# fudan-zvg/NeRF-LiDAR

Measured on AMD Instinct MI355X. Metric: LiDAR rays/sec @128 samples/ray, 8x256 MLP; depth L1 vs reference, higher is better.
Workload: dtype f32 (sampling, hash grid) + split-bf16 x3 MFMA (density/semantic/intensity) + bf16 MFMA (view MLP); 1 GPU; C2: nuScenes 32-beam sweep, 32x1024 rays per sweep, samples (64,64,128), 8x256 NerfMLP + semantic + intensity heads, full-size fp32 hash tables; azimuth_columns_total=1024, parallelism=azimuth-sector x1, hip_graph_replay=False, weights=seeded synthetic (white-noise tables, x1500 density gain), sweep_origins=moving: step i renders sweep i mod 64 (pre-uploaded ray batches), gather_bytes_per_ray=1347584

## Files before the change

### include/nerflidar_hip.h

```cpp
#ifndef NERFLIDAR_HIP_H
#define NERFLIDAR_HIP_H

#include <stddef.h>
#include <stdint.h>

#ifdef __cplusplus
extern "C" {
#endif

#define NLR_MAX_LEVELS 4
#define NLR_MAX_GRID_LEVELS 16
#define NLR_MAX_VIEW_DEPTH 16

enum {
    NLR_OK = 0,
    NLR_ERR_INVALID = -1,
    NLR_ERR_UNSUPPORTED = -2,
    NLR_ERR_HIP = -3,
    NLR_ERR_WORKSPACE = -4
};

enum {
    NLR_PREC_F32 = 0,
    NLR_PREC_MIXED = 1,
    NLR_PREC_FAST = 2
};

const char *nlr_last_error(void);
int nlr_version(void);

int nlr_grid_encode_forward(const float *inputs, const void *embeddings, int table_dtype,
                            const int32_t *offsets_host, float *outputs, uint32_t B, uint32_t D,
                            uint32_t C, uint32_t L, float S, uint32_t H, float *dy_dx,
                            uint32_t gridtype, int align_corners, uint32_t interp, int out_layout,
                            void *stream);

int nlr_grid_encode_backward(const float *grad, const float *inputs, const int32_t *offsets_host,
                             float *grad_embeddings, uint32_t B, uint32_t D, uint32_t C, uint32_t L,
                             float S, uint32_t H, const float *dy_dx, float *grad_inputs,
                             uint32_t gridtype, int align_corners, uint32_t interp, int grad_layout,
                             void *stream);

size_t nlr_grid_backward_workspace_bytes(uint32_t B, uint32_t C, uint32_t L, float S, uint32_t H, const int32_t *offsets_host,
                                         uint32_t gridtype, int align_corners);
int nlr_grid_encode_backward_ws(const float *grad, const float *inputs, const int32_t *offsets_host, float *grad_embeddings, uint32_t B,
                                uint32_t D, uint32_t C, uint32_t L, float S, uint32_t H, const float *dy_dx, float *grad_inputs,
                                uint32_t gridtype, int align_corners, uint32_t interp, int grad_layout, void *workspace,
                                size_t workspace_bytes, void *stream);

int nlr_grad_total_variation(const float *inputs, const float *embeddings, float *grad, const int32_t *offsets_host, float weight,
                             uint32_t B, uint32_t D, uint32_t C, uint32_t L, float S, uint32_t H, uint32_t gridtype,
                             int align_corners, void *stream);

void nlr_level_scale(uint32_t L, float S, uint32_t H, float *scale, uint32_t *resolution);

void nlr_sample_u(uint32_t n, int rand, float *u_host, float *max_jitter);

typedef struct NlrLinear {
    const float *weight;
    const float *bias;
    uint32_t out_features, in_features;
} NlrLinear;

typedef struct NlrGridDesc {
    const void *table;
    int32_t table_dtype;
    uint32_t num_levels, level_dim;
    uint32_t base_resolution;
    float log2_per_level_scale;
    const int32_t *offsets;
    uint32_t gridtype;
    uint32_t align_corners;
    uint32_t interp;
} NlrGridDesc;

typedef struct NlrMlpDesc {
    NlrGridDesc grid;
    NlrLinear density0, density2;
    uint32_t disable_rgb;
    uint32_t bottleneck_width;
    uint32_t net_depth_viewdirs, net_width_viewdirs, skip_layer_dir, deg_view;
    NlrLinear view[NLR_MAX_VIEW_DEPTH];
    NlrLinear rgb_layer;
    uint32_t use_semantic, no_sem_layer, class_num;
    NlrLinear sem0, sem2;
    uint32_t use_intensity;
    NlrLinear int0, int2;
    float density_bias, rgb_premultiplier, rgb_bias, rgb_padding;
    uint32_t re_weights;
} NlrMlpDesc;

typedef struct NlrModelDesc {
    uint32_t num_levels;
    uint32_t num_samples[NLR_MAX_LEVELS];
    const NlrMlpDesc *mlps[NLR_MAX_LEVELS];
    float dilation_multiplier, dilation_bias;
    float anneal_slope, resample_padding;
    float power_lambda, std_scale;
    float bg_intensity;
    uint32_t opaque_background;
    uint32_t mlp_precision;
} NlrModelDesc;

typedef struct NlrModel NlrModel;
int nlr_model_create(const NlrModelDesc *desc, NlrModel **out, void *stream);
void nlr_model_destroy(NlrModel *m);
int nlr_model_set_table(NlrModel *m, uint32_t level, const void *table_dev, int table_dtype);

typedef struct NlrRays {
    const float *origins, *directions, *viewdirs;
    const float *radii, *near, *far;
    const float *base_x, *base_y;
} NlrRays;

typedef struct NlrRenderCfg {
    float train_frac;
    uint32_t compute_extras;
    uint32_t sample_n, sample_m;
    const float *rand_jitter[NLR_MAX_LEVELS];
    const float *rand_deg[NLR_MAX_LEVELS];
    float scale_factor;
    uint32_t shuffled_rays;
} NlrRenderCfg;

typedef struct NlrLevelOut {
    float *sdist, *tdist;
    float *weights, *density;
    float *rgb;
    float *semantic;
    float *intensity;
    float *depth;
    float *r_rgb;
    float *r_acc, *r_distance_mean, *r_distance_median, *r_distance_percentile_5, *r_distance_percentile_95;
} NlrLevelOut;

typedef struct NlrOut {
    float *rgb;
    float *depth;
    float *semantic;
    float *intensity;
    float *acc, *distance_mean, *distance_median, *distance_percentile_5, *distance_percentile_95;
    int32_t *labels;
    float *points;
    float *packed;
    uint32_t packed_h, packed_w;
    NlrLevelOut history[NLR_MAX_LEVELS];
} NlrOut;

size_t nlr_workspace_bytes(const NlrModel *m, uint32_t N);
int nlr_render_rays(const NlrModel *m, const NlrRays *rays, uint32_t N, const NlrRenderCfg *cfg,
                    const NlrOut *out, void *workspace, size_t workspace_bytes, void *stream);
int nlr_render_lidar(const NlrModel *m, const NlrRays *rays, uint32_t N, const NlrRenderCfg *cfg,
                     const NlrOut *out, void *workspace, size_t workspace_bytes, void *stream);

const char *nlr_kernel_names(void);

const char *nlr_build_sha(void);

#define NLR_DBG_FORCE_GENERIC 0
#define NLR_DBG_MLP_WORKGROUPS 1
#define NLR_DBG_BINNED_C4 2
#define NLR_DBG_NO_XPAIR_SCATTER 3
#define NLR_DBG_SCATTER_LEVELS 4
#define NLR_DBG_NO_SCATTER_CACHE 5
#define NLR_DBG_RAY_GROUPS 6
#define NLR_DBG_LAST_ROUTE 7
#define NLR_DBG_TRAIN_ROUTE 8
#define NLR_DBG_TRAIN_TRUNK_ROW0 9
#define NLR_DBG_TRAIN_TRUNK_ROWS 10
int nlr_debug_set(uint32_t key, int value);
int nlr_debug_get(uint32_t key);
int nlr_grid_fast_path(const int32_t *offsets_host, uint32_t L, uint32_t C, float S, uint32_t H, int table_dtype, uint32_t gridtype,
                       int align_corners, uint32_t interp);

enum { NLR_K_RESAMPLE = 0, NLR_K_PROP = 1, NLR_K_ENCODE = 2, NLR_K_DIRBIAS = 3, NLR_K_MLP = 4, NLR_K_COMPOSITE = 5, NLR_K_COUNT = 6 };
int nlr_profile_begin(NlrModel *m);
int nlr_profile_begin_kinds(NlrModel *m, uint32_t kind_mask);
int nlr_profile_end(NlrModel *m, void *stream, float *total_ms, uint32_t *launches);

int nlr_resample_level(const float *prev_sdist, const float *prev_weights, uint32_t n_prev,
                       float dilation, float anneal, float resample_padding, uint32_t num_samples,
                       const float *rand_jitter, const float *near, const float *far,
                       float power_lambda, uint32_t N, float *sdist, float *tdist, void *stream);

int nlr_mlp_level(const NlrModel *m, uint32_t level, const NlrRays *rays, const float *tdist,
                  uint32_t N, uint32_t sample_n, uint32_t sample_m, const float *rand_deg,
                  float *features , float *density, float *rgb,
                  float *semantic, float *intensity, void *workspace, size_t workspace_bytes,
                  void *stream);

int nlr_composite_level(const float *density, const float *tdist, const float *directions,
                        const float *rgb, const float *semantic, const float *intensity,
                        const float *far, const float *origins, uint32_t N, uint32_t S,
                        uint32_t class_num, int opaque_background, float bg, int compute_extras,
                        float scale_factor, float *weights, const NlrOut *out, float *level_depth,
                        void *stream);

size_t nlr_range_workspace_bytes(uint32_t H, uint32_t W);
int nlr_range_project(const double *points, const float *semantic, const float *rgb, uint32_t N, uint32_t H, uint32_t W,
                      float fov_up_deg, float fov_down_deg, void *workspace, size_t workspace_bytes, float *proj_range,
                      float *proj_xyz, float *proj_semantic, float *proj_rgb, int32_t *proj_idx, float *proj_mask,
                      void *stream);

int nlr_composite_backward(const float *density, const float *tdist, const float *directions, const float *rgb,
                           const float *semantic, const float *intensity, uint32_t N, uint32_t S, uint32_t class_num,
                           int opaque_background, float bg, const float *g_rgb, const float *g_depth,
                           const float *g_semantic, const float *g_intensity, const float *g_acc, const float *g_weights,
                           float *d_density, float *d_rgb, float *d_semantic, float *d_intensity, void *stream);
int nlr_cast_contract(const NlrRays *rays, const float *tdist, uint32_t N, uint32_t S, uint32_t sample_n, uint32_t sample_m,
                      float std_scale, const float *rand_deg, float *means, float *stds, void *stream);
int nlr_hash_decay_forward(const float *embeddings, const int32_t *offsets_host, uint32_t L, uint32_t C, double *level_sumsq,
                           void *stream);
int nlr_hash_decay_backward(const float *embeddings, const int32_t *offsets_host, uint32_t L, uint32_t C, float upstream,
                            float *grad_embeddings, void *stream);

typedef struct NlrTrainPlan NlrTrainPlan;
int nlr_train_plan_create(uint32_t F, uint32_t W, uint32_t WB, uint32_t D, uint32_t deg_view, uint32_t class_num,
                          int use_semantic, int use_intensity, float density_bias, float rgb_premultiplier, float rgb_bias,
                          float rgb_padding, NlrTrainPlan **out, uint32_t *n_params);
void nlr_train_plan_destroy(NlrTrainPlan *p);
uint32_t nlr_train_act_width(const NlrTrainPlan *p);
int nlr_train_param_layout(const NlrTrainPlan *p, uint32_t *offsets, uint32_t capacity);
int nlr_train_linear_table(const NlrTrainPlan *p, uint32_t *rows, uint32_t capacity);
int nlr_train_pack(NlrTrainPlan *p, const float *params_dev, void *stream);
int nlr_mlp_train_forward(const NlrTrainPlan *p, const float *features, const float *enc, uint32_t M, uint32_t S, float *density,
                          float *rgb, float *semantic, float *intensity, void *acts, void *stream);
int nlr_mlp_train_backward(const NlrTrainPlan *p, uint32_t M, uint32_t S, const float *density, const float *rgb,
                           const float *semantic, const void *acts, const float *g_density, const float *g_rgb,
                           const float *g_semantic, const float *g_intensity, void *gacts, float *d_features, void *stream);
size_t nlr_mlp_train_wgrad_workspace_bytes(const NlrTrainPlan *p, uint32_t M);
int nlr_mlp_train_wgrad(const NlrTrainPlan *p, uint32_t M, uint32_t S, const float *features, const float *enc, const void *acts,
                        const void *gacts, float *d_params, void *workspace, size_t workspace_bytes, void *stream);
int nlr_mlp_train_forward_split(const NlrTrainPlan *p, const float *features, const float *enc, uint32_t M, uint32_t M_color,
                                uint32_t S, float *density, float *rgb, float *semantic, float *intensity, void *acts, void *stream);
int nlr_mlp_train_backward_split(const NlrTrainPlan *p, uint32_t M, uint32_t M_color, uint32_t S, const float *density,
                                 const float *rgb, const float *semantic, const void *acts, const float *g_density,
                                 const float *g_rgb, const float *g_semantic, const float *g_intensity, void *gacts,
                                 float *d_features, void *stream);
int nlr_mlp_train_wgrad_split(const NlrTrainPlan *p, uint32_t M, uint32_t M_color, uint32_t S, const float *features,
                              const float *enc, const void *acts, const void *gacts, float *d_params, void *workspace,
                              size_t workspace_bytes, void *stream);

int nlr_box_winner(const float *tdist, const float *origins, const float *directions, const float *box_params, uint32_t N,
                   uint32_t S, uint32_t n_obj, int32_t *winner, void *stream);

int nlr_track_box_params(const float *tracks, const float *timestamps, uint32_t N, uint32_t n_obj, uint32_t T, float *box_params,
                         void *stream);

size_t nlr_obj_frame_backward_workspace_bytes(uint32_t K, uint32_t n_obj, uint32_t T);
int nlr_obj_frame_backward(const float *tracks, const float *timestamps, const float *origins, const float *directions,
                           const float *viewdirs, const float *tdist, uint32_t N, uint32_t S, uint32_t n_obj, uint32_t T,
                           const int32_t *ray_idx, const int32_t *sample_idx, const int32_t *track_idx, uint32_t K, const float *g_pts,
                           const float *g_dirs, float *g_tracks, void *workspace, size_t workspace_bytes, void *stream);

typedef struct NlrObjClassDesc {
    NlrMlpDesc mlp;
    uint32_t latent_size, split_latent;
    int32_t class_type;
} NlrObjClassDesc;

typedef struct NlrObjectsDesc {
    uint32_t n_classes;
    const NlrObjClassDesc *classes;
    uint32_t n_tracks;
    const int32_t *track_class;
    const float *latents;
} NlrObjectsDesc;

typedef struct NlrObjects NlrObjects;
int nlr_objects_create(const NlrObjectsDesc *desc, NlrObjects **out, void *stream);
void nlr_objects_destroy(NlrObjects *o);
size_t nlr_objects_workspace_bytes(const NlrObjects *o, uint32_t N, uint32_t S);
int nlr_objects_apply(const NlrObjects *o, const NlrRays *rays, const float *tdist, const float *box_params, uint32_t N, uint32_t S,
                      uint32_t n_obj, float *density, float *rgb, float *semantic, uint32_t K, int32_t *winner_out, void *workspace,
                      size_t workspace_bytes, void *stream);
int nlr_render_rays_dynamic(const NlrModel *m, const NlrObjects *o, const NlrRays *rays, const float *box_params, uint32_t n_obj,
                            uint32_t N, const NlrRenderCfg *cfg, const NlrOut *out, int32_t *const *winner, void *workspace,
                            size_t workspace_bytes, void *stream);
int nlr_render_lidar_dynamic(const NlrModel *m, const NlrObjects *o, const NlrRays *rays, const float *box_params, uint32_t n_obj,
                             uint32_t N, const NlrRenderCfg *cfg, const NlrOut *out, int32_t *const *winner, void *workspace,
                             size_t workspace_bytes, void *stream);

int nlr_prop_mlp_forward(const float *feat, const float *w1, const float *b1, const float *w2, const float *b2, uint32_t M, uint32_t F,
                         float *raw, void *stream);
int nlr_prop_mlp_backward(const float *feat, const float *w1, const float *b1, const float *w2, const float *b2, const float *g_raw,
                          uint32_t M, uint32_t F, float *d_feat, float *d_w1, float *d_b1, float *d_w2, float *d_b2, void *stream);

int nlr_encode_features_forward(const NlrRays *rays, const float *tdist, uint32_t N, uint32_t S, uint32_t sample_n, uint32_t sample_m,
                                float std_scale, const float *rand_deg, const NlrGridDesc *grid, uint32_t re_weights, float *features,
                                void *stream);
int nlr_encode_features_backward(const NlrRays *rays, const float *tdist, uint32_t N, uint32_t S, uint32_t sample_n, uint32_t sample_m,
                                 float std_scale, const float *rand_deg, const NlrGridDesc *grid, uint32_t re_weights,
                                 const float *d_features, float *points_tmp ,
                                 float *grad_tmp , float *grad_table, void *stream);
int nlr_encode_features_backward_ws(const NlrRays *rays, const float *tdist, uint32_t N, uint32_t S, uint32_t sample_n, uint32_t sample_m,
                                    float std_scale, const float *rand_deg, const NlrGridDesc *grid, uint32_t re_weights,
                                    const float *d_features, float *points_tmp, float *grad_tmp, float *grad_table, void *workspace,
                                    size_t workspace_bytes, void *stream);
int nlr_encode_features_backward_rays(const NlrRays *rays, const float *tdist, uint32_t N, uint32_t S, uint32_t sample_n, uint32_t sample_m,
                                      float std_scale, const float *rand_deg, const NlrGridDesc *grid, uint32_t re_weights,
                                      const float *d_features , float *d_origins, float *d_directions, float *d_base_x,
                                      float *d_base_y , void *stream);

#ifdef __cplusplus
}
#endif
#endif
```

### nerf-lidar_amd/csrc/nlr_api.hip

```cpp
#include <stdarg.h>

#include <vector>

#include "nlr_kernels.h"

#include <stdlib.h>
#include "nlr_objects.h"


static thread_local char g_err[512] = "";
void nlr_set_error(const char *fmt, ...) {
    va_list ap;
    va_start(ap, fmt);
    vsnprintf(g_err, sizeof(g_err), fmt, ap);
    va_end(ap);
}
extern "C" const char *nlr_last_error(void) { return g_err; }
extern "C" int nlr_version(void) { return 100; }
extern "C" const char *nlr_kernel_names(void) {
    return "nlr_resample_kernel,nlr_prop8_kernel,nlr_encode8_kernel,nlr_direnc_kernel,nlr_mlp_kernel,nlr_composite_kernel";
}

struct Profile {
    bool armed = false;
    uint32_t mask = 0xffffffffu;
    std::vector<hipEvent_t> ev;
    std::vector<int> kind;
};
struct ProfScope {
    Profile *p;
    hipStream_t st;
    ProfScope(Profile *prof, int kind, hipStream_t s) : p(prof && prof->armed && ((prof->mask >> kind) & 1u) ? prof : nullptr), st(s) {
        if (!p) return;
        hipEvent_t a, b;
        if (hipEventCreate(&a) != hipSuccess || hipEventCreate(&b) != hipSuccess) { p = nullptr; return; }
        p->ev.push_back(a);
        p->ev.push_back(b);
        p->kind.push_back(kind);
        (void)hipEventRecord(a, st);
    }
    ~ProfScope() {
        if (p) (void)hipEventRecord(p->ev.back(), st);
    }
};

struct LevelModel {
    bool is_prop = false;
    GridParams gp;
    uint32_t F = 0, S = 0;
    int re_weights = 1;
    float density_bias = -1.0f;
    float *p_w1 = nullptr, *p_b1 = nullptr, *p_w2 = nullptr;
    float p_b2 = 0.0f;
    uint32_t W = 0, WB = 0, D = 0, HT = 0, K = 0, int_row = 0xffffffffu, deg = 0, E = 0;
    bool use_int = false;
    uint32_t prec = NLR_PREC_MIXED;
    void *tape = nullptr;
    uint32_t tape_chunks = 0;
    void *tape_lidar = nullptr;
    uint32_t tape_lidar_chunks = 0;
    float rgb_premul = 1.0f, rgb_bias = 0.0f, rgb_padding = 0.001f;
    float *bias_all = nullptr;
    uint32_t bias_count = 0;
    float *u_det = nullptr, *u_rand = nullptr;
    float max_jitter = 0.0f;
};

struct NlrModel {
    uint32_t num_levels = 0;
    LevelModel lv[NLR_MAX_LEVELS];
    float dilation_multiplier, dilation_bias, anneal_slope, resample_padding, power_lambda, std_scale, bg;
    uint32_t opaque, prec;
    int device = 0;
    uint32_t cus = 0;
    hipStream_t up = nullptr;
    std::vector<void *> allocs;
    mutable Profile prof;
};

static int dev_upload(NlrModel *m, const void *host, size_t bytes, void **out) {
    void *p = nullptr;
    NLR_HIP(hipMalloc(&p, bytes ? bytes : 16));
    m->allocs.push_back(p);
    if (bytes) {
        NLR_HIP(hipMemcpyAsync(p, host, bytes, hipMemcpyHostToDevice, m->up));
        NLR_HIP(hipStreamSynchronize(m->up));
    }
    *out = p;
    return NLR_OK;
}

static uint16_t f32_to_bf16(float f) {
    uint32_t u;
    memcpy(&u, &f, 4);
    if ((u & 0x7f800000u) == 0x7f800000u && (u & 0x007fffffu)) return (uint16_t)((u >> 16) | 0x40);
    u += 0x7fffu + ((u >> 16) & 1u);
    return (uint16_t)(u >> 16);
}

struct Mat {
    std::vector<float> a;
    uint32_t rows = 0, cols = 0;
    Mat() {}
    Mat(uint32_t r, uint32_t c) : a((size_t)r * c, 0.0f), rows(r), cols(c) {}
    float &at(uint32_t r, uint32_t c) { return a[(size_t)r * cols + c]; }
    float get(uint32_t r, uint32_t c) const { return (r < rows && c < cols) ? a[(size_t)r * cols + c] : 0.0f; }
};

static Mat fold_w2(const Mat &a, uint32_t col0, const NlrLinear &w2, std::vector<float> &bias) {
    const uint32_t WB = w2.out_features, H = w2.in_features;
    Mat out(a.rows, H);
    for (uint32_t r = 0; r < a.rows; ++r) {
        for (uint32_t k = 0; k < H; ++k) {
            double acc = 0.0;
            for (uint32_t c = 0; c < WB; ++c) acc += (double)a.get(r, col0 + c) * (double)w2.weight[(size_t)c * H + k];
            out.at(r, k) = (float)acc;
        }
        double acc = (double)bias[r];
        for (uint32_t c = 0; c < WB; ++c) acc += (double)a.get(r, col0 + c) * (double)w2.bias[c];
        bias[r] = (float)acc;
    }
    return out;
}

static Mat mat_from(const NlrLinear &l, uint32_t col0, uint32_t ncols) {
    Mat m(l.out_features, ncols);
    for (uint32_t r = 0; r < l.out_features; ++r)
        for (uint32_t c = 0; c < ncols; ++c) m.at(r, c) = l.weight[(size_t)r * l.in_features + col0 + c];
    return m;
}

enum { TAPE_F32 = 0, TAPE_BF16 = 1, TAPE_X3 = 2 };
#define NLR_TAPE_CHUNK 32768
struct TapeBuilder {
    std::vector<uint8_t> bytes;
    size_t frags() const { return bytes.size() / 1024; }
    void frag_bf16(const Mat &w, uint32_t R, uint32_t g, bool lo_part) {
        uint16_t f[64 * 8];
        for (uint32_t lane = 0; lane < 64; ++lane)
            for (uint32_t j = 0; j < 8; ++j) {
                const float v = w.get(16 * R + (lane & 15), 32 * g + 16 * (j >> 2) + 4 * (lane >> 4) + (j & 3));
                const uint16_t hi = f32_to_bf16(v);
                if (!lo_part) {
                    f[lane * 8 + j] = hi;
                } else {
                    uint32_t hb = (uint32_t)hi << 16;
                    float hf;
                    memcpy(&hf, &hb, 4);
                    f[lane * 8 + j] = f32_to_bf16(v - hf);
                }
            }
        bytes.insert(bytes.end(), (const uint8_t *)f, (const uint8_t *)f + sizeof(f));
    }
    void frag_f32(const Mat &w, uint32_t R, uint32_t J) {
        float f[64 * 4];
        for (uint32_t lane = 0; lane < 64; ++lane)
            for (uint32_t e = 0; e < 4; ++e) f[lane * 4 + e] = w.get(16 * R + (lane & 15), 16 * J + 4 * (lane >> 4) + e);
        bytes.insert(bytes.end(), (const uint8_t *)f, (const uint8_t *)f + sizeof(f));
    }
    void add(const Mat &w, uint32_t out_pad, uint32_t in_pad, int kind, uint32_t RH = 2) {
        const uint32_t OT = RH == 2 ? out_pad / 32 : 1;
        const uint32_t KG = kind == TAPE_F32 ? in_pad / 16 : in_pad / 32;
        for (uint32_t o = 0; o < OT; ++o)
            for (uint32_t g = 0; g < KG; ++g)
                for (uint32_t j = 0; j < RH; ++j) {
                    const uint32_t R = RH == 2 ? 2 * o + j : o;
                    if (kind == TAPE_F32) {
                        frag_f32(w, R, g);
                    } else {
                        frag_bf16(w, R, g, false);
                        if (kind == TAPE_X3) frag_bf16(w, R, g, true);
                    }
                }
    }
    void pad_to_chunk() { bytes.resize((bytes.size() + NLR_TAPE_CHUNK - 1) / NLR_TAPE_CHUNK * NLR_TAPE_CHUNK, 0); }
};

static int upload_bias(NlrModel *m, const float *b, uint32_t n, uint32_t pad, float **out) {
    std::vector<float> v(pad, 0.0f);
    for (uint32_t i = 0; i < n; ++i) v[i] = b[i];
    return dev_upload(m, v.data(), pad * sizeof(float), (void **)out);
}

static int check_linear(const NlrLinear &l, uint32_t out_f, uint32_t in_f, const char *name) {
    NLR_CHECK_ARG(l.weight && l.bias, "%s: weight/bias is NULL", name);
    NLR_CHECK_ARG(l.out_features == out_f && l.in_features == in_f, "%s: expected [%u,%u], got [%u,%u]", name, out_f, in_f,
                  l.out_features, l.in_features);
    return NLR_OK;
}

static int build_level(NlrModel *m, LevelModel &lv, const NlrMlpDesc &d, uint32_t S, uint32_t prec) {
    int rc = nlr_fill_grid_params(&lv.gp, d.grid.table, d.grid.table_dtype, d.grid.offsets, d.grid.num_levels,
                                  d.grid.level_dim, d.grid.log2_per_level_scale, d.grid.base_resolution, d.grid.gridtype,
                                  (int)d.grid.align_corners, d.grid.interp);
    if (rc) return rc;
    NLR_CHECK_ARG(d.grid.table != nullptr, "mlp: hash table pointer is NULL");
    lv.S = S;
    lv.F = d.grid.num_levels * d.grid.level_dim;
    lv.re_weights = d.re_weights ? 1 : 0;
    lv.density_bias = d.density_bias;
    lv.is_prop = d.disable_rgb != 0;
    {
        std::vector<float> u(S);
        float mj = 0.0f;
        nlr_sample_u(S, 0, u.data(), nullptr);
        if ((rc = dev_upload(m, u.data(), S * sizeof(float), (void **)&lv.u_det))) return rc;
        nlr_sample_u(S, 1, u.data(), &mj);
        lv.max_jitter = mj;
        if ((rc = dev_upload(m, u.data(), S * sizeof(float), (void **)&lv.u_rand))) return rc;
    }
    if ((rc = check_linear(d.density0, 64, lv.F, "density_layer.0"))) return rc;
    if (lv.is_prop) {
        if ((rc = check_linear(d.density2, 1, 64, "density_layer.2 (PropMLP)"))) return rc;
        if ((rc = dev_upload(m, d.density0.weight, (size_t)64 * lv.F * 4, (void **)&lv.p_w1))) return rc;
        if ((rc = dev_upload(m, d.density0.bias, 64 * 4, (void **)&lv.p_b1))) return rc;
        if ((rc = dev_upload(m, d.density2.weight, 64 * 4, (void **)&lv.p_w2))) return rc;
        lv.p_b2 = d.density2.bias[0];
        return NLR_OK;
    }
    lv.W = d.net_width_viewdirs;
    lv.WB = d.bottleneck_width;
    lv.D = d.net_depth_viewdirs;
    lv.deg = d.deg_view;
    lv.E = 3 + 6 * d.deg_view;
    lv.rgb_premul = d.rgb_premultiplier;
    lv.rgb_bias = d.rgb_bias;
    lv.rgb_padding = d.rgb_padding;
    if (lv.D < 2 || d.skip_layer_dir != 0 || lv.D > NLR_MAX_VIEW_DEPTH)
        NLR_FAIL(NLR_ERR_UNSUPPORTED, "view MLP: fused path needs net_depth_viewdirs in [2,%d] and skip_layer_dir = 0 (got %u, %u)",
                 NLR_MAX_VIEW_DEPTH, lv.D, d.skip_layer_dir);
    if (lv.W % 32 || lv.WB % 32) NLR_FAIL(NLR_ERR_UNSUPPORTED, "view MLP: widths must be multiples of 32");
    if (lv.F % 4) NLR_FAIL(NLR_ERR_UNSUPPORTED, "NerfMLP: L*C = %u must be a multiple of 4", lv.F);
    if ((rc = check_linear(d.density2, lv.WB, 64, "density_layer.2"))) return rc;
    const bool sem_layer = d.use_semantic && !d.no_sem_layer;
    const bool sem_pass = d.use_semantic && d.no_sem_layer;
    if (sem_pass) NLR_CHECK_ARG(d.class_num <= 32 && 1 + d.class_num <= d.bottleneck_width, "no_sem_layer: class_num %u does not fit", d.class_num);
    lv.K = d.use_semantic ? d.class_num : 0;
    lv.use_int = d.use_intensity != 0;
    lv.HT = (d.use_semantic ? 2 : 0) + (lv.use_int ? 2 : 0);
    NLR_CHECK_ARG(lv.K + (lv.use_int ? 1 : 0) <= 32, "class_num %u (+intensity) exceeds one 32-row output tile", lv.K);

    lv.prec = prec;
    const int crit = (prec == NLR_PREC_FAST) ? TAPE_X3 : TAPE_F32;
    const int view = (prec == NLR_PREC_F32) ? TAPE_F32 : TAPE_BF16;
    const bool fold = prec == NLR_PREC_FAST;
    std::vector<float> bias;
    auto push_bias = [&](const float *b, uint32_t n, uint32_t pad) {
        for (uint32_t i = 0; i < pad; ++i) bias.push_back(i < n ? b[i] : 0.0f);
    };
    const uint32_t Fp32 = lv.F <= 64 ? 64 : ((lv.F + 31) / 32) * 32;
    TapeBuilder trunk;
    trunk.add(mat_from(d.density0, 0, lv.F), 64, Fp32, crit);
    push_bias(d.density0.bias, 64, 64);
    trunk.add(mat_from(d.density2, 0, 64), fold ? 32 : lv.WB, 64, crit);
    push_bias(d.density2.bias, fold ? 32 : lv.WB, fold ? 32 : lv.WB);
    if (lv.HT) {
        const uint32_t HH = lv.HT * 32;
        Mat h1(HH, lv.WB), h2(32, HH);
        std::vector<float> b1(HH, 0.0f), b2(32, 0.0f);
        uint32_t r0 = 0;
        if (sem_layer) {
            if ((rc = check_linear(d.sem0, 64, lv.WB, "sem_layer.0"))) return rc;
            if ((rc = check_linear(d.sem2, d.class_num, 64, "sem_layer.2"))) return rc;
            for (uint32_t r = 0; r < 64; ++r) {
                for (uint32_t c = 0; c < lv.WB; ++c) h1.at(r0 + r, c) = d.sem0.weight[(size_t)r * lv.WB + c];
                b1[r0 + r] = d.sem0.bias[r];
            }
            for (uint32_t r = 0; r < d.class_num; ++r) {
                for (uint32_t c = 0; c < 64; ++c) h2.at(r, r0 + c) = d.sem2.weight[(size_t)r * 64 + c];
                b2[r] = d.sem2.bias[r];
            }
            r0 += 64;
        }
        if (sem_pass) {
            for (uint32_t c = 0; c < d.class_num; ++c) {
                h1.at(r0 + c, 1 + c) = 1.0f;
                h1.at(r0 + 32 + c, 1 + c) = -1.0f;
                h2.at(c, r0 + c) = 1.0f;
                h2.at(c, r0 + 32 + c) = -1.0f;
            }
            r0 += 64;
        }
        if (lv.use_int) {
            if ((rc = check_linear(d.int0, 64, lv.WB, "intensity_layer.0"))) return rc;
            if ((rc = check_linear(d.int2, 1, 64, "intensity_layer.2"))) return rc;
            lv.int_row = lv.K;
            for (uint32_t r = 0; r < 64; ++r) {
                for (uint32_t c = 0; c < lv.WB; ++c) h1.at(r0 + r, c) = d.int0.weight[(size_t)r * lv.WB + c];
                b1[r0 + r] = d.int0.bias[r];
            }
            for (uint32_t c = 0; c < 64; ++c) h2.at(lv.int_row, r0 + c) = d.int2.weight[c];
            b2[lv.int_row] = d.int2.bias[0];
        }
        if (fold) trunk.add(fold_w2(h1, 0, d.density2, b1), HH, 64, crit);
        else trunk.add(h1, HH, lv.WB, crit);
        push_bias(b1.data(), HH, HH);
        trunk.add(h2, 32, HH, crit);
        push_bias(b2.data(), 32, 32);
    } else {
        push_bias(nullptr, 0, 32);
    }
    const uint32_t in0 = lv.WB + lv.E, in1 = lv.W + in0;
    if ((rc = check_linear(d.view[0], lv.W, in0, "lin_second_stage_0"))) return rc;
    if ((rc = check_linear(d.view[1], lv.W, in1, "lin_second_stage_1"))) return rc;
    NLR_CHECK_ARG(lv.E <= 32, "deg_view %u gives %u > 32 direction features -- no fused path", lv.deg, lv.E);
    TapeBuilder v01;
    if (fold) {
        const Mat v0 = mat_from(d.view[0], 0, in0), v1 = mat_from(d.view[1], 0, in1);
        std::vector<float> c0(d.view[0].bias, d.view[0].bias + lv.W), c1(d.view[1].bias, d.view[1].bias + lv.W);
        const Mat a0 = fold_w2(v0, 0, d.density2, c0), a1 = fold_w2(v1, lv.W, d.density2, c1);
        Mat f0(lv.W, 64 + lv.E), f1(lv.W, lv.W + 64 + lv.E);
        for (uint32_t r = 0; r < lv.W; ++r) {
            for (uint32_t c = 0; c < 64; ++c) f0.at(r, c) = a0.get(r, c), f1.at(r, lv.W + c) = a1.get(r, c);
            for (uint32_t c = 0; c < lv.E; ++c) f0.at(r, 64 + c) = v0.get(r, lv.WB + c), f1.at(r, lv.W + 64 + c) = v1.get(r, lv.W + lv.WB + c);
            for (uint32_t c = 0; c < lv.W; ++c) f1.at(r, c) = v1.get(r, c);
        }
        v01.add(f0, lv.W, 64 + 32, view);
        push_bias(c0.data(), lv.W, lv.W);
        v01.add(f1, lv.W, lv.W + 64 + 32, view);
        push_bias(c1.data(), lv.W, lv.W);
    } else {
        v01.add(mat_from(d.view[0], 0, in0), lv.W, lv.WB + 32, view);
        push_bias(d.view[0].bias, lv.W, lv.W);
        v01.add(mat_from(d.view[1], 0, in1), lv.W, lv.W + lv.WB + 32, view);
        push_bias(d.view[1].bias, lv.W, lv.W);
    }
    TapeBuilder tb;
    auto append = [&](const TapeBuilder &x) { tb.bytes.insert(tb.bytes.end(), x.bytes.begin(), x.bytes.end()); };
    if (prec == NLR_PREC_F32) {
        append(trunk);
        append(v01);
    } else {
        append(trunk);
        append(v01);
        append(trunk);
        append(v01);
    }
    for (uint32_t l = 2; l < lv.D; ++l) {
        char nm[64];
        snprintf(nm, sizeof(nm), "lin_second_stage_%u", l);
        if ((rc = check_linear(d.view[l], lv.W, lv.W, nm))) return rc;
        tb.add(mat_from(d.view[l], 0, lv.W), lv.W, lv.W, view);
        push_bias(d.view[l].bias, lv.W, lv.W);
    }
    if ((rc = check_linear(d.rgb_layer, 3, lv.W, "rgb_layer"))) return rc;
    tb.add(mat_from(d.rgb_layer, 0, lv.W), 16, lv.W, view, 1);
    push_bias(d.rgb_layer.bias, 3, 32);
    tb.pad_to_chunk();
    lv.bias_count = (uint32_t)bias.size();
    NLR_CHECK_ARG(lv.bias_count <= 3072, "bias block of %u floats exceeds the 3072-float LDS reservation (view MLP too deep / wide)", lv.bias_count);
    if ((rc = dev_upload(m, bias.data(), bias.size() * 4, (void **)&lv.bias_all))) return rc;
    lv.tape_chunks = (uint32_t)(tb.bytes.size() / NLR_TAPE_CHUNK);
    tb.bytes.resize(tb.bytes.size() + 3 * NLR_TAPE_CHUNK, 0);
    if ((rc = dev_upload(m, tb.bytes.data(), tb.bytes.size(), &lv.tape))) return rc;
    if (prec == NLR_PREC_FAST) {
        TapeBuilder tl;
        tl.bytes.insert(tl.bytes.end(), trunk.bytes.begin(), trunk.bytes.end());
        tl.bytes.insert(tl.bytes.end(), trunk.bytes.begin(), trunk.bytes.end());
        tl.pad_to_chunk();
        lv.tape_lidar_chunks = (uint32_t)(tl.bytes.size() / NLR_TAPE_CHUNK);
        tl.bytes.resize(tl.bytes.size() + 3 * NLR_TAPE_CHUNK, 0);
        if ((rc = dev_upload(m, tl.bytes.data(), tl.bytes.size(), &lv.tape_lidar))) return rc;
    }
    return NLR_OK;
}

extern "C" int nlr_model_create(const NlrModelDesc *desc, NlrModel **out, void *stream) {
    NLR_CHECK_ARG(desc && out, "model_create: NULL argument");
    NLR_CHECK_ARG(desc->num_levels >= 1 && desc->num_levels <= NLR_MAX_LEVELS, "num_levels %u outside [1,%d]", desc->num_levels,
                  NLR_MAX_LEVELS);
    NLR_CHECK_ARG(desc->mlp_precision <= NLR_PREC_FAST, "unknown mlp_precision %u", desc->mlp_precision);
    NlrModel *m = new NlrModel();
    m->up = (hipStream_t)stream;
    {
        int n = 0;
        if (hipGetDevice(&m->device) != hipSuccess ||
            hipDeviceGetAttribute(&n, hipDeviceAttributeMultiprocessorCount, m->device) != hipSuccess || n <= 0) {
            delete m;
            NLR_FAIL(NLR_ERR_HIP, "model_create: cannot query the current device");
        }
        m->cus = (uint32_t)n;
        const int w = nlr_debug_get(NLR_DBG_MLP_WORKGROUPS);
        if (w > 0 && w < n) m->cus = (uint32_t)w;
    }
    m->num_levels = desc->num_levels;
    m->dilation_multiplier = desc->dilation_multiplier;
    m->dilation_bias = desc->dilation_bias;
    m->anneal_slope = desc->anneal_slope;
    m->resample_padding = desc->resample_padding;
    m->power_lambda = desc->power_lambda;
    m->std_scale = desc->std_scale;
    m->bg = desc->bg_intensity;
    m->opaque = desc->opaque_background;
    m->prec = desc->mlp_precision;
    for (uint32_t l = 0; l < desc->num_levels; ++l) {
        int rc = NLR_OK;
        if (!desc->mlps[l]) {
            nlr_set_error("model_create: mlps[%u] is NULL", l);
            rc = NLR_ERR_INVALID;
        } else if (desc->num_samples[l] < 2 || desc->num_samples[l] > 512) {
            nlr_set_error("num_samples must be in [2,512], is %u", desc->num_samples[l]);
            rc = NLR_ERR_INVALID;
        } else {
            rc = build_level(m, m->lv[l], *desc->mlps[l], desc->num_samples[l], desc->mlp_precision);
            const bool last = (l + 1 == desc->num_levels);
            if (!rc && last && m->lv[l].is_prop) {
                nlr_set_error("the last level must be a NerfMLP (disable_rgb = 0)");
                rc = NLR_ERR_INVALID;
            }
            if (!rc && !last && !m->lv[l].is_prop) {
                nlr_set_error("single_mlp / NerfMLP as proposal network has no fused path (level %u)", l);
                rc = NLR_ERR_UNSUPPORTED;
            }
        }
        if (rc) {
            nlr_model_destroy(m);
            return rc;
        }
    }
    if (hipStreamSynchronize(m->up) != hipSuccess) {
        nlr_model_destroy(m);
        NLR_FAIL(NLR_ERR_HIP, "model_create: weight upload failed");
    }
    *out = m;
    return NLR_OK;
}

extern "C" void nlr_model_destroy(NlrModel *m) {
    if (!m) return;
    for (void *p : m->allocs) (void)hipFree(p);
    delete m;
}

extern "C" int nlr_model_set_table(NlrModel *m, uint32_t level, const void *table_dev, int table_dtype) {
    NLR_CHECK_ARG(m && level < m->num_levels && table_dev, "model_set_table: bad argument");
    NLR_CHECK_ARG(table_dtype == 0 || table_dtype == 1, "model_set_table: table_dtype must be 0 or 1");
    m->lv[level].gp.table = table_dev;
    m->lv[level].gp.table_dtype = table_dtype;
    return NLR_OK;
}

extern "C" int nlr_profile_begin_kinds(NlrModel *m, uint32_t kind_mask) {
    NLR_CHECK_ARG(m != nullptr, "profile_begin: NULL model");
    for (hipEvent_t e : m->prof.ev) (void)hipEventDestroy(e);
    m->prof.ev.clear();
    m->prof.kind.clear();
    m->prof.mask = kind_mask;
    m->prof.armed = true;
    return NLR_OK;
}
extern "C" int nlr_profile_begin(NlrModel *m) { return nlr_profile_begin_kinds(m, 0xffffffffu); }

extern "C" int nlr_profile_end(NlrModel *m, void *stream, float *total_ms, uint32_t *launches) {
    NLR_CHECK_ARG(m && total_ms && launches, "profile_end: NULL argument");
    m->prof.armed = false;
    NLR_HIP(hipStreamSynchronize((hipStream_t)stream));
    for (int k = 0; k < NLR_K_COUNT; ++k) {
        total_ms[k] = 0.0f;
        launches[k] = 0;
    }
    for (size_t i = 0; i < m->prof.kind.size(); ++i) {
        float ms = 0.0f;
        NLR_HIP(hipEventElapsedTime(&ms, m->prof.ev[2 * i], m->prof.ev[2 * i + 1]));
        total_ms[m->prof.kind[i]] += ms;
        launches[m->prof.kind[i]] += 1;
    }
    for (hipEvent_t e : m->prof.ev) (void)hipEventDestroy(e);
    m->prof.ev.clear();
    m->prof.kind.clear();
    return NLR_OK;
}


struct Carve {
    char *base;
    size_t off = 0, cap;
    Carve(void *p, size_t c) : base((char *)p), cap(c) {}
    float *take(size_t nfloat) {
        size_t b = al(nfloat * sizeof(float));
        float *r = base ? (float *)(base + off) : nullptr;
        off += b;
        return r;
    }
};

static size_t level_ws(const LevelModel &lv, uint32_t N, bool last) {
    size_t S = lv.S, b = 0;
    b += 2 * al((size_t)N * (S + 1) * 4);
    b += 2 * al((size_t)N * S * 4);
    if (!lv.is_prop) {
        b += al((size_t)N * S * lv.F * 4 + 1024);
        b += al((size_t)N * S * 3 * 4);
        b += al((size_t)N * S * (lv.K ? lv.K : 1) * 4);
        b += al((size_t)N * S * 4);
        b += al((size_t)N * 32 * 4);
        b += al((size_t)N * 4);
        b += al((size_t)N * S * 4);
    }
    (void)last;
    return b;
}

extern "C" size_t nlr_workspace_bytes(const NlrModel *m, uint32_t N) {
    if (!m) return 0;
    size_t b = 256 + al(64 * sizeof(uint32_t));
    for (uint32_t l = 0; l < m->num_levels; ++l) b += level_ws(m->lv[l], N, l + 1 == m->num_levels);
    return b;
}

static int run_mlp_level(const NlrModel *m, const LevelModel &lv, const NlrRays *rays, const float *tdist, uint32_t N,
                         uint32_t n, uint32_t mloops, const float *rand_deg, float *feat, float *raybias, float *density,
                         float *rgb, float *sem, float *inten, float *prop_feat, hipStream_t st, bool internal_feat = false,
                         float *seg = nullptr, float *dnorm = nullptr, uint32_t ray_groups = 0, const uint32_t *votes = nullptr,
                         bool lidar = false) {
    const int piece_major = (internal_feat && !lv.is_prop && n <= 8 && lv.F % 4 == 0) ? 1 : 0;
    CastParams cp;
    int rc = nlr_fill_cast_params(&cp, rays, tdist, rand_deg, N, lv.S, n, mloops, m->std_scale);
    if (rc) return rc;
    cp.ray_groups = ray_groups;
    cp.votes = votes;
    cp.vote_min = (uint32_t)(((uint64_t)(N ? N - 1 : 0) * lv.S) / 2);
    if (lv.is_prop) {
        ProfScope ps(&m->prof, NLR_K_PROP, st);
        return nlr_launch_prop(cp, lv.gp, lv.p_w1, lv.p_b1, lv.p_w2, lv.p_b2, lv.density_bias, lv.re_weights, density, prop_feat, st);
    }
    {
        ProfScope ps(&m->prof, NLR_K_ENCODE, st);
        if ((rc = nlr_launch_encode(cp, lv.gp, lv.re_weights, feat, piece_major, st))) return rc;
    }
    if (seg && lidar) {
        NLR_CHECK_ARG(lv.tape_lidar != nullptr, "NerfMLP: no LiDAR-only tape at this precision");
        ProfScope ps(&m->prof, NLR_K_DIRBIAS, st);
        if ((rc = nlr_launch_dnorm(rays->directions, N, dnorm, st))) return rc;
    } else if (rgb || seg) {
        NLR_CHECK_ARG(rays->viewdirs != nullptr, "NerfMLP: viewdirs is NULL");
        DirEncParams dp;
        dp.viewdirs = rays->viewdirs;
        dp.dirs = seg ? rays->directions : nullptr;
        dp.dnorm = seg ? dnorm : nullptr;
        dp.N = N;
        dp.deg = lv.deg;
        dp.E = lv.E;
        dp.out = raybias;
        ProfScope ps(&m->prof, NLR_K_DIRBIAS, st);
        if ((rc = nlr_launch_direnc(dp, st))) return rc;
    }
    MlpParams P;
    memset(&P, 0, sizeof(P));
    P.feat = feat;
    P.feat_piece_major = piece_major;
    P.M = N * lv.S;
    P.S = lv.S;
    P.F = lv.F;
    P.tape = (const uint4 *)lv.tape;
    P.tape_chunks = lv.tape_chunks;
    P.bias_all = lv.bias_all;
    P.bias_count = lv.bias_count;
    P.enc = raybias;
    P.depth = lv.D;
    P.K = (sem || seg) ? lv.K : 0;
    P.int_row = lv.int_row;
    P.tdist = tdist;
    P.dnorm = dnorm;
    P.seg = seg;
    P.opaque = m->opaque;
    P.density_bias = lv.density_bias;
    P.rgb_premul = lv.rgb_premul;
    P.rgb_bias = lv.rgb_bias;
    P.rgb_padding = lv.rgb_padding;
    P.density = density;
    P.rgb = seg ? seg : rgb;
    P.sem = sem;
    P.inten = (lv.use_int && (inten || seg)) ? (seg ? seg : inten) : nullptr;
    if (seg && lidar) {
        P.lidar = 1;
        P.tape = (const uint4 *)lv.tape_lidar;
        P.tape_chunks = lv.tape_lidar_chunks;
        P.enc = nullptr;
        P.rgb = nullptr;
    }
    ProfScope ps(&m->prof, NLR_K_MLP, st);
    return nlr_launch_mlp(P, lv.W, lv.WB, lv.HT, lv.prec, m->cus, st);
}

extern "C" int nlr_mlp_level(const NlrModel *m, uint32_t level, const NlrRays *rays, const float *tdist, uint32_t N,
                             uint32_t sample_n, uint32_t sample_m, const float *rand_deg, float *features, float *density,
                             float *rgb, float *semantic, float *intensity, void *workspace, size_t workspace_bytes,
                             void *stream) {
    NLR_CHECK_ARG(m && level < m->num_levels && rays && tdist && density, "mlp_level: bad argument");
    if (N == 0) return NLR_OK;
    const LevelModel &lv = m->lv[level];
    hipStream_t st = (hipStream_t)stream;
    if (lv.is_prop)
        return run_mlp_level(m, lv, rays, tdist, N, sample_n, sample_m, rand_deg, nullptr, nullptr, density, nullptr, nullptr,
                             nullptr, features, st);
    Carve c(workspace, workspace_bytes);
    float *feat = features ? features : c.take((size_t)N * lv.S * lv.F + 256);
    float *rb = c.take((size_t)N * 32);
    float *sem = semantic ? semantic : (lv.K ? c.take((size_t)N * lv.S * lv.K) : nullptr);
    if (c.off > workspace_bytes || (!workspace && c.off))
        NLR_FAIL(NLR_ERR_WORKSPACE, "mlp_level: workspace %zu B < needed %zu B", workspace_bytes, c.off);
    return run_mlp_level(m, lv, rays, tdist, N, sample_n, sample_m, rand_deg, feat, rb, density, rgb, sem, intensity, nullptr, st,
                         features == nullptr);
}

struct DynScene {
    const NlrObjects *objs;
    const float *box_params;
    uint32_t n_obj;
    int32_t *const *winner;
};

static int render_impl(const NlrModel *m, const NlrRays *rays, uint32_t N, const NlrRenderCfg *cfg, const NlrOut *out, void *workspace,
                       size_t workspace_bytes, void *stream, const DynScene *dyn, bool lidar_only) {
    NLR_CHECK_ARG(m && rays && cfg && out, "render_rays: NULL argument");
    NLR_CHECK_ARG(rays->origins && rays->directions && rays->near && rays->far && rays->radii, "render_rays: ray batch has NULL tensors");
    if (lidar_only) {
        NLR_CHECK_ARG(out->rgb == nullptr, "render_lidar: out->rgb must be NULL (a LiDAR-only render computes no colour)");
        NLR_CHECK_ARG(out->history[m->num_levels - 1].rgb == nullptr,
                      "render_lidar: history[%u].rgb must be NULL (a LiDAR-only render computes no colour)", m->num_levels - 1);
    }
    if (N == 0) return NLR_OK;
    size_t need = nlr_workspace_bytes(m, N), obj_ws = 0;
    if (dyn) {
        uint32_t smax = 0;
        for (uint32_t l = 0; l < m->num_levels; ++l) smax = m->lv[l].S > smax ? m->lv[l].S : smax;
        obj_ws = nlr_objects_workspace_bytes(dyn->objs, N, smax);
        need += obj_ws;
    }
    if (!workspace || workspace_bytes < need)
        NLR_FAIL(NLR_ERR_WORKSPACE, "render_rays: workspace %zu B < %zu B (nlr_workspace_bytes%s)", workspace_bytes, need,
                 dyn ? " + nlr_objects_workspace_bytes" : "");
    hipStream_t st = (hipStream_t)stream;
    void *obj_space = dyn ? (char *)workspace + (workspace_bytes - obj_ws) : nullptr;
    Carve c(workspace, workspace_bytes - obj_ws);
    const uint32_t n = cfg->sample_n ? cfg->sample_n : 7, mloops = cfg->sample_m ? cfg->sample_m : 3;
    uint32_t *votes = (uint32_t *)c.take(64);
    if (int rc0 = nlr_launch_ray_vote(nullptr, 0, 0, votes, st)) return rc0;

    const float *prev_s = nullptr, *prev_w = nullptr;
    uint32_t n_prev = 0;
    double prod = 1.0;
    for (uint32_t l = 0; l < m->num_levels; ++l) {
        const LevelModel &lv = m->lv[l];
        const bool last = (l + 1 == m->num_levels);
        const uint32_t S = lv.S;
        const NlrLevelOut &ho = out->history[l];
        float *sdist = ho.sdist ? ho.sdist : c.take((size_t)N * (S + 1));
        float *tdist = ho.tdist ? ho.tdist : c.take((size_t)N * (S + 1));
        float *weights = ho.weights ? ho.weights : c.take((size_t)N * S);
        float *density = ho.density ? ho.density : c.take((size_t)N * S);
        const bool use_dil = m->dilation_bias > 0 || m->dilation_multiplier > 0;
        const float dilation = (l > 0 && use_dil) ? (float)(m->dilation_bias + m->dilation_multiplier * 1.0 / prod) : 0.0f;
        prod *= (double)S;
        const float tf = cfg->train_frac;
        const float anneal = m->anneal_slope > 0 ? (float)(((double)m->anneal_slope * tf) / (((double)m->anneal_slope - 1.0) * tf + 1.0)) : 1.0f;
        const float *jit = cfg->rand_jitter[l];
        int rc;
        {
            ProfScope ps(&m->prof, NLR_K_RESAMPLE, st);
            rc = nlr_launch_resample(prev_s, prev_w, n_prev, dilation, anneal, m->resample_padding, S, jit ? lv.u_rand : lv.u_det,
                                     jit, lv.max_jitter, rays->near, rays->far, m->power_lambda, N, sdist, tdist, st);
        }
        if (rc) return rc;
        float *feat = nullptr, *rb = nullptr, *rgb = nullptr, *sem = nullptr, *inten = nullptr, *seg = nullptr, *dnorm = nullptr;
        const bool lidar = lidar_only && last;
        const bool fuse = !dyn && last && !lv.is_prop && !ho.rgb && !ho.semantic && !ho.intensity && lv.gp.C == 4 && n <= 8 &&
                          nlr_mlp_can_composite(lv.W, lv.WB, lv.HT, lv.prec, lv.F, S, lv.K, lv.use_int, (uint64_t)N * S, lidar ? 2 : 1);
        if (last) (void)nlr_debug_set(NLR_DBG_LAST_ROUTE, (lidar ? 2 : 0) + (fuse ? 1 : 0) + 1);
        if (!lv.is_prop) {
            feat = c.take((size_t)N * S * lv.F + 256);
            rb = c.take((size_t)N * 32);
            if (fuse) {
                dnorm = c.take((size_t)N);
                seg = c.take((size_t)N * S);
            } else {
                rgb = lidar ? nullptr : (ho.rgb ? ho.rgb : c.take((size_t)N * S * 3));
                sem = lv.K ? (ho.semantic ? ho.semantic : c.take((size_t)N * S * lv.K)) : nullptr;
                inten = lv.use_int ? (ho.intensity ? ho.intensity : c.take((size_t)N * S)) : nullptr;
            }
        }
        uint32_t groups = cfg->shuffled_rays ? 0u : 2u;
        if (const int force = nlr_debug_get(NLR_DBG_RAY_GROUPS)) groups = force == 1 ? 1u : 0u;
        if (groups == 2u && n > 8) groups = 0u;
        if (groups == 2u && (rc = nlr_launch_ray_vote(tdist, N, S, votes + l, st))) return rc;
        rc = run_mlp_level(m, lv, rays, tdist, N, n, mloops, cfg->rand_deg[l], feat, rb, density, rgb, sem, inten, nullptr, st, true, seg,
                           dnorm, groups, votes + l, lidar);
        if (rc) return rc;
        if (dyn) {
            rc = nlr_objects_apply_impl(dyn->objs, rays, tdist, dyn->box_params, N, S, dyn->n_obj, density, rgb, sem, lv.K,
                                        dyn->winner ? dyn->winner[l] : nullptr, obj_space, obj_ws, st);
            if (rc) return rc;
        }
        {
            ProfScope ps(&m->prof, NLR_K_COMPOSITE, st);
            if (fuse)
                rc = nlr_composite_segments(density, tdist, rays->directions, seg, lv.K, lv.use_int ? 1 : 0, rays->far, rays->origins, N, S,
                                            (int)m->opaque, m->bg, (int)cfg->compute_extras, cfg->scale_factor, weights, out, ho.depth, st,
                                            lidar);
            else if (last)
                rc = nlr_composite_level_impl(density, tdist, rays->directions, rgb, sem, inten, rays->far, rays->origins, N, S, lv.K,
                                              (int)m->opaque, m->bg, (int)cfg->compute_extras, cfg->scale_factor, weights, out, ho.depth,
                                              st, lidar);
            else {
                NlrOut lo;
                memset(&lo, 0, sizeof(lo));
                lo.rgb = ho.r_rgb;
                lo.acc = ho.r_acc;
                lo.distance_mean = ho.r_distance_mean;
                lo.distance_median = ho.r_distance_median;
                lo.distance_percentile_5 = ho.r_distance_percentile_5;
                lo.distance_percentile_95 = ho.r_distance_percentile_95;
                const bool extras = cfg->compute_extras && (lo.distance_mean || lo.distance_median || lo.distance_percentile_5 || lo.distance_percentile_95);
                rc = nlr_composite_level(density, tdist, rays->directions, nullptr, nullptr, nullptr, rays->far, rays->origins, N, S, 0,
                                         (int)m->opaque, m->bg, extras ? 1 : 0, 0.0f, weights, &lo, ho.depth, st);
            }
        }
        if (rc) return rc;
        prev_s = sdist;
        prev_w = weights;
        n_prev = S;
    }
    if (c.off > workspace_bytes - obj_ws) NLR_FAIL(NLR_ERR_WORKSPACE, "render_rays: carved %zu B > workspace %zu B", c.off, workspace_bytes - obj_ws);
    return NLR_OK;
}

extern "C" int nlr_render_rays(const NlrModel *m, const NlrRays *rays, uint32_t N, const NlrRenderCfg *cfg, const NlrOut *out,
                               void *workspace, size_t workspace_bytes, void *stream) {
    return render_impl(m, rays, N, cfg, out, workspace, workspace_bytes, stream, nullptr, false);
}

extern "C" int nlr_render_lidar(const NlrModel *m, const NlrRays *rays, uint32_t N, const NlrRenderCfg *cfg, const NlrOut *out,
                                void *workspace, size_t workspace_bytes, void *stream) {
    return render_impl(m, rays, N, cfg, out, workspace, workspace_bytes, stream, nullptr, true);
}

static int render_dynamic(const NlrModel *m, const NlrObjects *o, const NlrRays *rays, const float *box_params, uint32_t n_obj, uint32_t N,
                          const NlrRenderCfg *cfg, const NlrOut *out, int32_t *const *winner, void *workspace, size_t workspace_bytes,
                          void *stream, bool lidar_only) {
    NLR_CHECK_ARG(m && o && (box_params || n_obj == 0), "render_rays_dynamic: NULL argument");
    for (uint32_t l = 0; l < m->num_levels; ++l)
        NLR_CHECK_ARG(!m->lv[l].use_int, "render_rays_dynamic: the object networks have no intensity head (ZI/models.py:469 assigns None)");
    DynScene d{o, box_params, n_obj, winner};
    return render_impl(m, rays, N, cfg, out, workspace, workspace_bytes, stream, &d, lidar_only);
}

extern "C" int nlr_render_rays_dynamic(const NlrModel *m, const NlrObjects *o, const NlrRays *rays, const float *box_params, uint32_t n_obj,
                                       uint32_t N, const NlrRenderCfg *cfg, const NlrOut *out, int32_t *const *winner, void *workspace,
                                       size_t workspace_bytes, void *stream) {
    return render_dynamic(m, o, rays, box_params, n_obj, N, cfg, out, winner, workspace, workspace_bytes, stream, false);
}

extern "C" int nlr_render_lidar_dynamic(const NlrModel *m, const NlrObjects *o, const NlrRays *rays, const float *box_params, uint32_t n_obj,
                                        uint32_t N, const NlrRenderCfg *cfg, const NlrOut *out, int32_t *const *winner, void *workspace,
                                        size_t workspace_bytes, void *stream) {
    return render_dynamic(m, o, rays, box_params, n_obj, N, cfg, out, winner, workspace, workspace_bytes, stream, true);
}
```

### nerf-lidar_amd/csrc/nlr_common.h

```cpp
#pragma once
#include <hip/hip_runtime.h>
#include <math.h>
#include <stdint.h>
#include <stdio.h>
#include <string.h>

#include "../../include/nerflidar_hip.h"

#define NLR_EPS 1.1920928955078125e-07f
#define NLR_WAVE 64

void nlr_set_error(const char *fmt, ...);
#define NLR_FAIL(code, ...)         \
    do {                            \
        nlr_set_error(__VA_ARGS__); \
        return (code);              \
    } while (0)
#define NLR_CHECK_ARG(cond, ...) \
    do {                         \
        if (!(cond)) NLR_FAIL(NLR_ERR_INVALID, __VA_ARGS__); \
    } while (0)
#define NLR_HIP(call)                                                                      \
    do {                                                                                   \
        hipError_t e_ = (call);                                                            \
        if (e_ != hipSuccess)                                                              \
            NLR_FAIL(NLR_ERR_HIP, "%s failed: %s (%s:%d)", #call, hipGetErrorString(e_), __FILE__, __LINE__); \
    } while (0)
#define NLR_LAUNCH_CHECK(name)                                                             \
    do {                                                                                   \
        hipError_t e_ = hipGetLastError();                                                 \
        if (e_ != hipSuccess)                                                              \
            NLR_FAIL(NLR_ERR_HIP, "launch of %s failed: %s", name, hipGetErrorString(e_)); \
    } while (0)

struct GridParams {
    const void *table;
    int32_t table_dtype;
    uint32_t L, C;
    uint32_t gridtype, align_corners, interp;
    uint32_t offset[NLR_MAX_GRID_LEVELS];
    uint32_t hsize[NLR_MAX_GRID_LEVELS];
    uint32_t res[NLR_MAX_GRID_LEVELS];
    float scale[NLR_MAX_GRID_LEVELS];
    float gsize[NLR_MAX_GRID_LEVELS];
    float inv_gsize[NLR_MAX_GRID_LEVELS];
    uint32_t dense[NLR_MAX_GRID_LEVELS];
    uint32_t mode[NLR_MAX_GRID_LEVELS];
    uint32_t step[NLR_MAX_GRID_LEVELS];
};

int nlr_fill_grid_params(GridParams *gp, const void *table, int table_dtype, const int32_t *offsets_host,
                         uint32_t L, uint32_t C, float S, uint32_t H, uint32_t gridtype, int align_corners,
                         uint32_t interp);

#ifdef __HIPCC__
__device__ __forceinline__ uint32_t nlr_grid_index(uint32_t gridtype, uint32_t align_corners, uint32_t hsize,
                                                   uint32_t res, uint32_t x, uint32_t y, uint32_t z) {
    uint32_t stride = 1, index = 0;
    const uint32_t step = align_corners ? res : res + 1;
    if (stride <= hsize) { index += x * stride; stride *= step; }
    if (stride <= hsize) { index += y * stride; stride *= step; }
    if (stride <= hsize) { index += z * stride; stride *= step; }
    if (gridtype == 0 && stride > hsize) index = x ^ (y * 2654435761u) ^ (z * 805459861u);
    return index % hsize;
}

template <int MODE>
__device__ __forceinline__ void nlr_corner_idx(const GridParams &gp, uint32_t level, const uint32_t (&pg)[3], uint32_t (&idx)[8]) {
    if (MODE == 0) {
        const uint32_t s = gp.step[level];
        const uint32_t y0 = pg[1] * s, z0 = pg[2] * s * s;
        const uint32_t y1 = y0 + s, z1 = z0 + s * s;
#pragma unroll
        for (int c8 = 0; c8 < 8; ++c8) idx[c8] = (pg[0] + (c8 & 1)) + ((c8 & 2) ? y1 : y0) + ((c8 & 4) ? z1 : z0);
    } else if (MODE == 1) {
        const uint32_t mask = gp.hsize[level] - 1u;
        const uint32_t y0 = pg[1] * 2654435761u, z0 = pg[2] * 805459861u;
        const uint32_t y1 = y0 + 2654435761u, z1 = z0 + 805459861u;
#pragma unroll
        for (int c8 = 0; c8 < 8; ++c8) idx[c8] = ((pg[0] + (c8 & 1)) ^ ((c8 & 2) ? y1 : y0) ^ ((c8 & 4) ? z1 : z0)) & mask;
    } else {
#pragma unroll
        for (int c8 = 0; c8 < 8; ++c8)
            idx[c8] = nlr_grid_index(gp.gridtype, gp.align_corners, gp.hsize[level], gp.res[level], pg[0] + (c8 & 1),
                                     pg[1] + ((c8 >> 1) & 1), pg[2] + ((c8 >> 2) & 1));
    }
}

__device__ __forceinline__ float nlr_wave_incl_scan_add(float v, int lane) {
#pragma unroll
    for (int d = 1; d < 64; d <<= 1) {
        float o = __shfl_up(v, d, 64);
        if (lane >= d) v += o;
    }
    return v;
}
__device__ __forceinline__ float nlr_wave_incl_scan_max(float v, int lane) {
#pragma unroll
    for (int d = 1; d < 64; d <<= 1) {
        float o = __shfl_up(v, d, 64);
        if (lane >= d) v = fmaxf(v, o);
    }
    return v;
}
__device__ __forceinline__ float nlr_wave_sum(float v) {
#pragma unroll
    for (int d = 32; d >= 1; d >>= 1) v += __shfl_xor(v, d, 64);
    return v;
}
__device__ __forceinline__ float nlr_wave_max(float v) {
#pragma unroll
    for (int d = 32; d >= 1; d >>= 1) v = fmaxf(v, __shfl_xor(v, d, 64));
    return v;
}
__device__ __forceinline__ float nlr_nan0_clip01(float x) {
    if (x != x) x = 0.0f;
    return fminf(fmaxf(x, 0.0f), 1.0f);
}
#endif
```

### nerf-lidar_amd/csrc/nlr_encode.hip

```cpp
#include "nlr_kernels.h"

#include <stdlib.h>

#include "nlr_cast.h"
#include "nlr_grid_level.h"
#include "nlr_level_fast.h"

template <typename T, int C>
__global__ void __launch_bounds__(256) nlr_encode_kernel(CastParams cp, GridParams gp, int re_weights, float *__restrict__ feat) {
    const uint32_t m = blockIdx.x * blockDim.x + threadIdx.x;
    const uint32_t M = cp.N * cp.S;
    if (m >= M) return;
    const uint32_t level = blockIdx.y;
    const uint32_t ray = m / cp.S, k = m - ray * cp.S;
    float o[3], d[3], bx[3], by[3];
#pragma unroll
    for (int c = 0; c < 3; ++c) {
        o[c] = cp.origins[(size_t)ray * 3 + c];
        d[c] = cp.directions[(size_t)ray * 3 + c];
        bx[c] = cp.base_x[(size_t)ray * 3 + c];
        by[c] = cp.base_y[(size_t)ray * 3 + c];
    }
    const float radius = cp.radii[ray];
    const float t0 = cp.tdist[(size_t)ray * (cp.S + 1) + k], t1 = cp.tdist[(size_t)ray * (cp.S + 1) + k + 1];
// ... 13 lines not shown

struct PropMlpParams {
    const float *w1, *b1;
    const float *w2;
    float b2, density_bias;
    uint32_t F;
};

template <typename T, int C, int LMAX>
__global__ void __launch_bounds__(256) nlr_prop_kernel(CastParams cp, GridParams gp, PropMlpParams mp, int re_weights,
                                                       float *__restrict__ density, float *__restrict__ feat_out) {
    const uint32_t m = blockIdx.x * blockDim.x + threadIdx.x;
    const uint32_t M = cp.N * cp.S;
    if (m >= M) return;
    const uint32_t ray = m / cp.S, k = m - ray * cp.S;
    float o[3], d[3], bx[3], by[3];
#pragma unroll
    for (int c = 0; c < 3; ++c) {
        o[c] = cp.origins[(size_t)ray * 3 + c];
        d[c] = cp.directions[(size_t)ray * 3 + c];
        bx[c] = cp.base_x[(size_t)ray * 3 + c];
        by[c] = cp.base_y[(size_t)ray * 3 + c];
    }
    const float radius = cp.radii[ray];
    const float t0 = cp.tdist[(size_t)ray * (cp.S + 1) + k], t1 = cp.tdist[(size_t)ray * (cp.S + 1) + k + 1];
    float feat[LMAX * C];
#pragma unroll
    for (int i = 0; i < LMAX * C; ++i) feat[i] = 0.0f;
    for (uint32_t j = 0; j < cp.n; ++j) {
        const Gauss g = nlr_cast_one(cp, ray, k, j, t0, t1, o, d, bx, by, radius);
#pragma unroll
        for (int l = 0; l < LMAX; ++l) {
            if (l < (int)gp.L) {
                const float werf = re_weights ? nlr_erf_weight(g.zs, gp.gsize[l]) : 1.0f;
                float a[C];
#pragma unroll
                for (int c = 0; c < C; ++c) a[c] = 0.0f;
                nlr_level_accum<T, C>(gp, l, g, werf, a);
#pragma unroll
                for (int c = 0; c < C; ++c) feat[l * C + c] += a[c];
            }
        }
    }
#pragma unroll
    for (int i = 0; i < LMAX * C; ++i) feat[i] = feat[i] / (float)cp.n;
    if (feat_out)
        for (uint32_t i = 0; i < mp.F; ++i) feat_out[(size_t)m * mp.F + i] = feat[i];
    float raw = mp.b2;
    for (int h = 0; h < 64; ++h) {
        float a = mp.b1[h];
#pragma unroll
        for (int i = 0; i < LMAX * C; ++i)
            if (i < (int)mp.F) a = fmaf(mp.w1[h * mp.F + i], feat[i], a);
        raw = fmaf(mp.w2[h], fmaxf(a, 0.0f), raw);
    }
    const float x = raw + mp.density_bias;
    density[m] = x > 20.0f ? x : log1pf(expf(x));
}

__device__ __forceinline__ bool nlr_slot_sample(const CastParams &cp, uint32_t slot, uint32_t &ray, uint32_t &k) {
    const bool groups = cp.ray_groups == 1u || (cp.ray_groups == 2u && cp.votes[0] > cp.vote_min);
    if (groups) {
        const uint32_t G = 8u * cp.S, gi = slot / G, w = slot - gi * G;
        ray = gi * 8u + (w & 7u);
        k = w >> 3;
    } else {
        ray = slot / cp.S;
        k = slot - ray * cp.S;
    }
    const bool in = ray < cp.N;
    if (!in) ray = cp.N - 1, k = cp.S - 1;
    return in;
}
__global__ void __launch_bounds__(256) nlr_ray_vote_kernel(const float *__restrict__ tdist, uint32_t N, uint32_t S, uint32_t *__restrict__ votes) {
    __shared__ uint32_t part[4];
    const uint32_t total = (N - 1) * S;
    uint32_t mine = 0;
    for (uint32_t i = blockIdx.x * 256u + threadIdx.x; i < total; i += gridDim.x * 256u) {
        const uint32_t r = i / S, k = i - r * S;
        const float *a = tdist + (size_t)r * (S + 1) + k;
        mine += fabsf(a[S + 1] - a[0]) < (a[1] - a[0]) ? 1u : 0u;
    }
#pragma unroll
    for (int o = 32; o; o >>= 1) mine += __shfl_down(mine, o);
    if ((threadIdx.x & 63u) == 0) part[threadIdx.x >> 6] = mine;
    __syncthreads();
    if (threadIdx.x == 0) {
        const uint32_t c = part[0] + part[1] + part[2] + part[3];
        if (c) atomicAdd(votes, c);
    }
}
__global__ void nlr_ray_vote_zero_kernel(uint32_t *votes) { votes[threadIdx.x] = 0u; }
int nlr_launch_ray_vote(const float *tdist, uint32_t N, uint32_t S, uint32_t *votes, hipStream_t st) {
    if (!tdist) {
        hipLaunchKernelGGL(nlr_ray_vote_zero_kernel, dim3(1), dim3(64), 0, st, votes);
        NLR_LAUNCH_CHECK("nlr_ray_vote_zero_kernel");
        return NLR_OK;
    }
    if (N < 2 || S == 0) return NLR_OK;
    NLR_CHECK_ARG((uint64_t)N * S < (1ull << 32), "ray vote: N * S = %llu does not fit 32 bits", (unsigned long long)N * S);
    const uint32_t nb = ((N - 1) * S + 255) / 256;
    hipLaunchKernelGGL(nlr_ray_vote_kernel, dim3(nb < 512u ? nb : 512u), dim3(256), 0, st, tdist, N, S, votes);
    NLR_LAUNCH_CHECK("nlr_ray_vote_kernel");
    return NLR_OK;
}
__host__ __forceinline__ uint64_t nlr_slot_count(const CastParams &cp) {
    return (uint64_t)(cp.ray_groups ? (cp.N + 7u) / 8u * 8u : cp.N) * cp.S;
}

template <int CTRL>
__device__ __forceinline__ float nlr_dpp_mov(float v) {
    return __builtin_bit_cast(float, __builtin_amdgcn_update_dpp(0, __builtin_bit_cast(int, v), CTRL, 0xf, 0xf, false));
}
__device__ __forceinline__ float nlr_group8_sum(float v) {
    v += nlr_dpp_mov<0xB1>(v);
    v += nlr_dpp_mov<0x4E>(v);
    v += nlr_dpp_mov<0x141>(v);
    return v;
}

template <int C>
__device__ __forceinline__ float *nlr_feat_ptr(float *feat, int piece_major, uint32_t M, uint32_t m, uint32_t l, uint32_t L) {
    if (piece_major) {
        const uint32_t f = l * C;
        return feat + ((size_t)(f >> 2) * M + m) * 4 + (f & 3u);
    }
    return feat + (size_t)m * L * C + l * C;
}

template <typename T, int C>
__global__ void __launch_bounds__(256) nlr_encode8g_kernel(CastParams cp, GridParams gp, int re_weights, float *__restrict__ feat,
                                                          int piece_major) {
    const uint32_t gt = blockIdx.x * blockDim.x + threadIdx.x;
    const uint32_t M = cp.N * cp.S;
    const uint32_t j = gt & 7;
    uint32_t ray, k;
    const bool in = nlr_slot_sample(cp, gt >> 3, ray, k);
    const uint32_t m = ray * cp.S + k;
    const bool active = in && j < cp.n;
    float o[3], d[3], bx[3], by[3];
#pragma unroll
    for (int c = 0; c < 3; ++c) {
        o[c] = cp.origins[(size_t)ray * 3 + c];
        d[c] = cp.directions[(size_t)ray * 3 + c];
        bx[c] = cp.base_x[(size_t)ray * 3 + c];
        by[c] = cp.base_y[(size_t)ray * 3 + c];
    }
    const float radius = cp.radii[ray];
    const float t0 = cp.tdist[(size_t)ray * (cp.S + 1) + k], t1 = cp.tdist[(size_t)ray * (cp.S + 1) + k + 1];
    Gauss g = nlr_cast_one(cp, ray, k, active ? j : 0, t0, t1, o, d, bx, by, radius);
    if (!active) g.x0 = -1.0f;
    const float inv_s8 = __frsqrt_rn(8.0f * (g.zs * g.zs));
    const float inv_n = 1.0f / (float)cp.n;
    for (uint32_t l = 0; l < gp.L; ++l) {
        const float werf = re_weights ? nlr_erf_weight_fast(inv_s8, gp.inv_gsize[l]) : 1.0f;
        float a[C];
#pragma unroll
        for (int c = 0; c < C; ++c) a[c] = 0.0f;
        nlr_level_accum<T, C>(gp, l, g, werf, a);
#pragma unroll
        for (int c = 0; c < C; ++c) a[c] = nlr_group8_sum(a[c]);
        if (in && j == (l & 7)) {
            if constexpr (C == 8) {
                float *f0 = nlr_feat_ptr<4>(feat, piece_major, M, m, 2 * l, 2 * gp.L), *f1 = nlr_feat_ptr<4>(feat, piece_major, M, m, 2 * l + 1, 2 * gp.L);
#pragma unroll
                for (int c = 0; c < 4; ++c) f0[c] = a[c] * inv_n, f1[c] = a[4 + c] * inv_n;
            } else {
                float *f = nlr_feat_ptr<C>(feat, piece_major, M, m, l, gp.L);
#pragma unroll
                for (int c = 0; c < C; ++c) f[c] = a[c] * inv_n;
            }
        }
    }
}

template <typename T, int C, int LMAX>
__global__ void __launch_bounds__(256) nlr_prop8g_kernel(CastParams cp, GridParams gp, PropMlpParams mp, int re_weights,
                                                        float *__restrict__ density, float *__restrict__ feat_out) {
    __shared__ float sw[64 * 16 + 128];
    for (uint32_t i = threadIdx.x; i < 64 * mp.F; i += 256) sw[i] = mp.w1[i];
    if (threadIdx.x < 64) {
        sw[64 * mp.F + threadIdx.x] = mp.b1[threadIdx.x];
        sw[64 * mp.F + 64 + threadIdx.x] = mp.w2[threadIdx.x];
    }
    __syncthreads();
    const uint32_t gt = blockIdx.x * blockDim.x + threadIdx.x;
    const uint32_t j = gt & 7;
    uint32_t ray, k;
    const bool in = nlr_slot_sample(cp, gt >> 3, ray, k);
    const uint32_t m = ray * cp.S + k;
    const bool active = in && j < cp.n;
    float o[3], d[3], bx[3], by[3];
#pragma unroll
    for (int c = 0; c < 3; ++c) {
        o[c] = cp.origins[(size_t)ray * 3 + c];
        d[c] = cp.directions[(size_t)ray * 3 + c];
        bx[c] = cp.base_x[(size_t)ray * 3 + c];
        by[c] = cp.base_y[(size_t)ray * 3 + c];
    }
    const float radius = cp.radii[ray];
    const float t0 = cp.tdist[(size_t)ray * (cp.S + 1) + k], t1 = cp.tdist[(size_t)ray * (cp.S + 1) + k + 1];
    Gauss g = nlr_cast_one(cp, ray, k, active ? j : 0, t0, t1, o, d, bx, by, radius);
    if (!active) g.x0 = -1.0f;
    const float inv_s8 = __frsqrt_rn(8.0f * (g.zs * g.zs));
    const float inv_n = 1.0f / (float)cp.n;
    float feat[LMAX * C];
#pragma unroll
    for (int l = 0; l < LMAX; ++l) {
        float a[C];
#pragma unroll
        for (int c = 0; c < C; ++c) a[c] = 0.0f;
        if (l < (int)gp.L) {
            const float werf = re_weights ? nlr_erf_weight_fast(inv_s8, gp.inv_gsize[l]) : 1.0f;
            nlr_level_accum<T, C>(gp, l, g, werf, a);
        }
#pragma unroll
        for (int c = 0; c < C; ++c) feat[l * C + c] = nlr_group8_sum(a[c]) * inv_n;
    }
    if (feat_out && in && j == 0)
        for (uint32_t i = 0; i < mp.F; ++i) feat_out[(size_t)m * mp.F + i] = feat[i];
    float part = 0.0f;
#pragma unroll
    for (int hh = 0; hh < 8; ++hh) {
        const uint32_t hu = hh * 8 + j;
        float a = sw[64 * mp.F + hu];
#pragma unroll
        for (int i = 0; i < LMAX * C; ++i)
            if (i < (int)mp.F) a = fmaf(sw[hu * mp.F + i], feat[i], a);
        part = fmaf(sw[64 * mp.F + 64 + hu], fmaxf(a, 0.0f), part);
    }
    const float raw = nlr_group8_sum(part) + mp.b2;
    if (in && j == 0) {
        const float x = raw + mp.density_bias;
        density[m] = x > 20.0f ? x : log1pf(expf(x));
    }
}

__device__ __forceinline__ uint32_t nlr_xcd_block(uint32_t b, uint32_t nblocks, uint32_t chunk) {
    const uint32_t per = 8u * chunk, full = (nblocks / per) * per;
    if (b >= full) return b;
    const uint32_t x = b & 7u, q = b >> 3;
    return ((q / chunk) * 8u + x) * chunk + (q % chunk);
}

#define NLR_XCD_CHUNK 32u

#ifdef NLR_DBG_ENV
#define NLR_DBG_LO nlr_dbg[0]
#define NLR_DBG_HI nlr_dbg[1]
__device__ __forceinline__ uint32_t nlr_dbg_ray(uint32_t po) {
    const uint32_t W = (uint32_t)nlr_dbg[2], tb = (uint32_t)nlr_dbg[5], ta = (uint32_t)nlr_dbg[6];
    if (!W || !tb || !ta) return po;
    const uint32_t per = tb * ta, tile = po / per, within = po - tile * per, tiles_row = W / ta;
    const uint32_t trow = tile / tiles_row, tcol = tile - trow * tiles_row;
    return (trow * tb + within / ta) * W + tcol * ta + within % ta;
}
#define NLR_DBG_RAY(r) nlr_dbg_ray(r)
#else
#define NLR_DBG_LO 0
#define NLR_DBG_HI 99
#define NLR_DBG_RAY(r) (r)
#endif

struct RayRegs {
    float o[3], d[3], bx[3], by[3], radius, t0, t1;
};
__device__ __forceinline__ RayRegs nlr_load_ray(const CastParams &cp, uint32_t ray, uint32_t k) {
    RayRegs r;
#pragma unroll
    for (int c = 0; c < 3; ++c) {
        r.o[c] = cp.origins[(size_t)ray * 3 + c];
        r.d[c] = cp.directions[(size_t)ray * 3 + c];
        r.bx[c] = cp.base_x[(size_t)ray * 3 + c];
        r.by[c] = cp.base_y[(size_t)ray * 3 + c];
    }
    r.radius = cp.radii[ray];
    r.t0 = cp.tdist[(size_t)ray * (cp.S + 1) + k];
    r.t1 = cp.tdist[(size_t)ray * (cp.S + 1) + k + 1];
    return r;
}

template <typename T, int C>
__device__ __forceinline__ void nlr_encode8_block(const CastParams &cp, const GridParams &gp, int re_weights, float *__restrict__ feat,
                                                  int piece_major, uint32_t block) {
    const uint32_t gt = block * 256u + threadIdx.x;
    const uint32_t M = cp.N * cp.S;
    const uint32_t j = gt & 7;
    uint32_t pray, k;
    const bool in = nlr_slot_sample(cp, gt >> 3, pray, k);
    const uint32_t ray = NLR_DBG_RAY(pray);
    const uint32_t m = ray * cp.S + k;
    const bool active = in && j < cp.n;
    const RayRegs rr = nlr_load_ray(cp, ray, k);
    const Gauss g = nlr_cast_one(cp, ray, k, active ? j : 0, rr.t0, rr.t1, rr.o, rr.d, rr.bx, rr.by, rr.radius);
    const bool valid = active && !((g.x0 < 0 || g.x0 > 1) || (g.x1 < 0 || g.x1 > 1) || (g.x2 < 0 || g.x2 > 1));
    const float inv_s8 = __frsqrt_rn(8.0f * (g.zs * g.zs));
    const float inv_n = 1.0f / (float)cp.n;
    float r[C];
#pragma unroll
    for (int c = 0; c < C; ++c) r[c] = 0.0f;
    for (uint32_t l = NLR_DBG_LO; l < gp.L && l < (uint32_t)NLR_DBG_HI; ++l) {
        if (valid) {
            const float werf = re_weights ? nlr_erf_weight_fast(inv_s8, gp.inv_gsize[l]) : 1.0f;
            if (gp.mode[l] == 0) nlr_level_fast<T, C, 0>(gp, l, g.x0, g.x1, g.x2, werf, r);
            else nlr_level_fast<T, C, 1>(gp, l, g.x0, g.x1, g.x2, werf, r);
        }
        float a[C];
        nlr_group8_sum_to(r, a);
        if (in && j == (l & 7)) {
            if constexpr (C == 8) {
                float *f0 = nlr_feat_ptr<4>(feat, piece_major, M, m, 2 * l, 2 * gp.L), *f1 = nlr_feat_ptr<4>(feat, piece_major, M, m, 2 * l + 1, 2 * gp.L);
#pragma unroll
                for (int c = 0; c < 4; ++c) f0[c] = a[c] * inv_n, f1[c] = a[4 + c] * inv_n;
                continue;
            }
            float *f = nlr_feat_ptr<C>(feat, piece_major, M, m, l, gp.L);
            if constexpr (C == 4) {
                const nlr_f4 q = {a[0] * inv_n, a[1] * inv_n, a[2] * inv_n, a[3] * inv_n};
                __builtin_nontemporal_store(q, (nlr_f4 *)f);
            } else {
#pragma unroll
                for (int c = 0; c < C; ++c) f[c] = a[c] * inv_n;
            }
        }
    }
}

template <typename T, int C>
__global__ void __launch_bounds__(256) nlr_encode8_kernel(CastParams cp, GridParams gp, int re_weights, float *__restrict__ feat,
                                                          int piece_major, uint32_t nblocks, uint32_t chunk) {
    for (uint32_t b = blockIdx.x; b < nblocks; b += gridDim.x)
        nlr_encode8_block<T, C>(cp, gp, re_weights, feat, piece_major, chunk ? nlr_xcd_block(b, nblocks, chunk) : b);
}

template <typename T, int C, int LMAX>
__global__ void __launch_bounds__(256) nlr_prop8_kernel(CastParams cp, GridParams gp, PropMlpParams mp, int re_weights,
                                                        float *__restrict__ density, float *__restrict__ feat_out, uint32_t nblocks, uint32_t chunk) {
    __shared__ float sw[64 * 16 + 128];
    for (uint32_t i = threadIdx.x; i < 64 * mp.F; i += 256) sw[i] = mp.w1[i];
    if (threadIdx.x < 64) {
        sw[64 * mp.F + threadIdx.x] = mp.b1[threadIdx.x];
        sw[64 * mp.F + 64 + threadIdx.x] = mp.w2[threadIdx.x];
    }
    __syncthreads();
  for (uint32_t lb = blockIdx.x; lb < nblocks; lb += gridDim.x) {
    const uint32_t gt = (chunk ? nlr_xcd_block(lb, nblocks, chunk) : lb) * 256u + threadIdx.x;
    const uint32_t j = gt & 7;
    uint32_t pray, k;
    const bool in = nlr_slot_sample(cp, gt >> 3, pray, k);
    const uint32_t ray = NLR_DBG_RAY(pray);
    const uint32_t m = ray * cp.S + k;
    const bool active = in && j < cp.n;
    const RayRegs rr = nlr_load_ray(cp, ray, k);
    const Gauss g = nlr_cast_one(cp, ray, k, active ? j : 0, rr.t0, rr.t1, rr.o, rr.d, rr.bx, rr.by, rr.radius);
    const bool valid = active && !((g.x0 < 0 || g.x0 > 1) || (g.x1 < 0 || g.x1 > 1) || (g.x2 < 0 || g.x2 > 1));
    const float inv_s8 = __frsqrt_rn(8.0f * (g.zs * g.zs));
    const float inv_n = 1.0f / (float)cp.n;
    float feat[LMAX * C];
#pragma unroll
    for (int i = 0; i < LMAX * C; ++i) feat[i] = 0.0f;
    if (valid) {
#pragma unroll
        for (int l = 0; l < LMAX; ++l) {
            if (l < (int)gp.L) {
                const float werf = re_weights ? nlr_erf_weight_fast(inv_s8, gp.inv_gsize[l]) : 1.0f;
                float a[C];
                if (gp.mode[l] == 0) nlr_level_fast<T, C, 0>(gp, l, g.x0, g.x1, g.x2, werf, a);
                else nlr_level_fast<T, C, 1>(gp, l, g.x0, g.x1, g.x2, werf, a);
#pragma unroll
                for (int c = 0; c < C; ++c) feat[l * C + c] = a[c];
            }
        }
    }
    static_assert((LMAX * C) % 4 == 0, "feature count of the proposal kernel must be a multiple of 4");
#pragma unroll
    for (int i = 0; i < LMAX * C; i += 4) {
        float q[4] = {feat[i], feat[i + 1], feat[i + 2], feat[i + 3]};
        nlr_group8_sum_n(q);
#pragma unroll
        for (int u = 0; u < 4; ++u) feat[i + u] = q[u] * inv_n;
    }
    if (feat_out && in && j == 0)
        for (uint32_t i = 0; i < mp.F; ++i) feat_out[(size_t)m * mp.F + i] = feat[i];
    float part = 0.0f;
#pragma unroll
    for (int hh = 0; hh < 8; ++hh) {
        const uint32_t hu = hh * 8 + j;
        float a = sw[64 * mp.F + hu];
#pragma unroll
        for (int i = 0; i < LMAX * C; ++i)
            if (i < (int)mp.F) a = fmaf(sw[hu * mp.F + i], feat[i], a);
        part = fmaf(sw[64 * mp.F + 64 + hu], fmaxf(a, 0.0f), part);
    }
    float praw[1] = {part};
    nlr_group8_sum_n(praw);
    if (in && j == 0) {
        const float x = (praw[0] + mp.b2) + mp.density_bias;
        density[m] = x > 20.0f ? x : log1pf(expf(x));
    }
  }
}

int nlr_fill_cast_params(CastParams *cp, const NlrRays *rays, const float *tdist, const float *rand_deg, uint32_t N,
                         uint32_t S, uint32_t n, uint32_t mloops, float std_scale);
int nlr_launch_encode(const CastParams &cp, const GridParams &gp, int re_weights, float *feat, int piece_major, hipStream_t st);

__global__ void __launch_bounds__(256) nlr_encode_expand_kernel(CastParams cp, GridParams gp, int re_weights, const float *__restrict__ d_feat,
                                                               float *__restrict__ x01, float *__restrict__ g_pts) {
    const size_t t = (size_t)blockIdx.x * blockDim.x + threadIdx.x;
    const size_t M = (size_t)cp.N * cp.S;
    if (t >= M * cp.n) return;
    const uint32_t m = (uint32_t)(t / cp.n), j = (uint32_t)(t - (size_t)m * cp.n);
    const uint32_t ray = m / cp.S, k = m - ray * cp.S;
    float o[3], d[3], bx[3], by[3];
#pragma unroll
    for (int c = 0; c < 3; ++c) {
        o[c] = cp.origins[(size_t)ray * 3 + c];
        d[c] = cp.directions[(size_t)ray * 3 + c];
        bx[c] = cp.base_x[(size_t)ray * 3 + c];
        by[c] = cp.base_y[(size_t)ray * 3 + c];
    }
    const float t0 = cp.tdist[(size_t)ray * (cp.S + 1) + k], t1 = cp.tdist[(size_t)ray * (cp.S + 1) + k + 1];
    const Gauss g = nlr_cast_one(cp, ray, k, j, t0, t1, o, d, bx, by, cp.radii[ray]);
    x01[t * 3 + 0] = g.x0;
    x01[t * 3 + 1] = g.x1;
    x01[t * 3 + 2] = g.x2;
    const float inv_s8 = __frsqrt_rn(8.0f * (g.zs * g.zs));
    const float inv_n = 1.0f / (float)cp.n;
    const uint32_t LC = gp.L * gp.C;
    const float *gf = d_feat + (size_t)m * LC;
    float *out = g_pts + t * LC;
    for (uint32_t l = 0; l < gp.L; ++l) {
        const float w = (re_weights ? nlr_erf_weight_fast(inv_s8, gp.inv_gsize[l]) : 1.0f) * inv_n;
        for (uint32_t c = 0; c < gp.C; ++c) out[l * gp.C + c] = gf[l * gp.C + c] * w;
    }
}

static int encode_features_args(CastParams *cp, GridParams *gp, const NlrRays *rays, const float *tdist, uint32_t N, uint32_t S, uint32_t sample_n,
                                uint32_t sample_m, float std_scale, const float *rand_deg, const NlrGridDesc *grid) {
    NLR_CHECK_ARG(grid && grid->table && grid->offsets && tdist, "encode_features: NULL argument");
    int rc = nlr_fill_cast_params(cp, rays, tdist, rand_deg, N, S, sample_n, sample_m, std_scale);
    if (rc) return rc;
    return nlr_fill_grid_params(gp, grid->table, grid->table_dtype, grid->offsets, grid->num_levels, grid->level_dim, grid->log2_per_level_scale,
                                grid->base_resolution, grid->gridtype, (int)grid->align_corners, grid->interp);
}

extern "C" int nlr_encode_features_forward(const NlrRays *rays, const float *tdist, uint32_t N, uint32_t S, uint32_t sample_n, uint32_t sample_m,
                                           float std_scale, const float *rand_deg, const NlrGridDesc *grid, uint32_t re_weights, float *features,
                                           void *stream) {
    if (N == 0 || S == 0) return NLR_OK;
    NLR_CHECK_ARG(features, "encode_features_forward: NULL output");
    CastParams cp;
    GridParams gp;
    int rc = encode_features_args(&cp, &gp, rays, tdist, N, S, sample_n, sample_m, std_scale, rand_deg, grid);
    if (rc) return rc;
    return nlr_launch_encode(cp, gp, (int)re_weights, features, 0, (hipStream_t)stream);
}

extern "C" int nlr_encode_features_backward_ws(const NlrRays *rays, const float *tdist, uint32_t N, uint32_t S, uint32_t sample_n, uint32_t sample_m,
                                               float std_scale, const float *rand_deg, const NlrGridDesc *grid, uint32_t re_weights,
                                               const float *d_features, float *points_tmp, float *grad_tmp, float *grad_table, void *workspace,
                                               size_t workspace_bytes, void *stream);

extern "C" int nlr_encode_features_backward(const NlrRays *rays, const float *tdist, uint32_t N, uint32_t S, uint32_t sample_n, uint32_t sample_m,
                                            float std_scale, const float *rand_deg, const NlrGridDesc *grid, uint32_t re_weights,
                                            const float *d_features, float *points_tmp, float *grad_tmp, float *grad_table, void *stream) {
    return nlr_encode_features_backward_ws(rays, tdist, N, S, sample_n, sample_m, std_scale, rand_deg, grid, re_weights, d_features, points_tmp,
                                           grad_tmp, grad_table, nullptr, 0, stream);
}

extern "C" int nlr_encode_features_backward_ws(const NlrRays *rays, const float *tdist, uint32_t N, uint32_t S, uint32_t sample_n, uint32_t sample_m,
                                               float std_scale, const float *rand_deg, const NlrGridDesc *grid, uint32_t re_weights,
                                               const float *d_features, float *points_tmp, float *grad_tmp, float *grad_table, void *workspace,
                                               size_t workspace_bytes, void *stream) {
    if (N == 0 || S == 0) return NLR_OK;
    NLR_CHECK_ARG(d_features && grad_table && points_tmp && grad_tmp, "encode_features_backward: NULL tensor");
    CastParams cp;
    GridParams gp;
    int rc = encode_features_args(&cp, &gp, rays, tdist, N, S, sample_n, sample_m, std_scale, rand_deg, grid);
    if (rc) return rc;
    const size_t B = (size_t)N * S * sample_n;
    NLR_CHECK_ARG(B < (1ull << 32), "encode_features_backward: %zu multisample points do not fit the 32-bit point index", B);
    hipStream_t st = (hipStream_t)stream;
    hipLaunchKernelGGL(nlr_encode_expand_kernel, dim3((unsigned)((B + 255) / 256)), dim3(256), 0, st, cp, gp, (int)re_weights, d_features, points_tmp,
                       grad_tmp);
    NLR_LAUNCH_CHECK("nlr_encode_expand_kernel");
    return nlr_grid_encode_backward_ws(grad_tmp, points_tmp, grid->offsets, grad_table, (uint32_t)B, 3, grid->level_dim, grid->num_levels,
                                       grid->log2_per_level_scale, grid->base_resolution, nullptr, nullptr, grid->gridtype, (int)grid->align_corners,
                                       grid->interp, 1, workspace, workspace_bytes, stream);
}

__global__ void __launch_bounds__(256) nlr_cast_contract_kernel(CastParams cp, float *__restrict__ means, float *__restrict__ stds) {
    const size_t t = (size_t)blockIdx.x * blockDim.x + threadIdx.x;
    const size_t M = (size_t)cp.N * cp.S;
    if (t >= M * cp.n) return;
    const uint32_t m = (uint32_t)(t / cp.n), j = (uint32_t)(t - (size_t)m * cp.n);
    const uint32_t ray = m / cp.S, k = m - ray * cp.S;
    float o[3], d[3], bx[3], by[3];
#pragma unroll
    for (int c = 0; c < 3; ++c) {
        o[c] = cp.origins[(size_t)ray * 3 + c];
        d[c] = cp.directions[(size_t)ray * 3 + c];
        bx[c] = cp.base_x[(size_t)ray * 3 + c];
        by[c] = cp.base_y[(size_t)ray * 3 + c];
    }
    const float t0 = cp.tdist[(size_t)ray * (cp.S + 1) + k], t1 = cp.tdist[(size_t)ray * (cp.S + 1) + k + 1];
    float raw[3];
    const Gauss g = nlr_cast_one(cp, ray, k, j, t0, t1, o, d, bx, by, cp.radii[ray], raw);
    means[t * 3 + 0] = raw[0];
    means[t * 3 + 1] = raw[1];
    means[t * 3 + 2] = raw[2];
    stds[t] = g.zs;
}

int nlr_fill_cast_params(CastParams *cp, const NlrRays *rays, const float *tdist, const float *rand_deg, uint32_t N,
                         uint32_t S, uint32_t n, uint32_t mloops, float std_scale);

extern "C" int nlr_cast_contract(const NlrRays *rays, const float *tdist, uint32_t N, uint32_t S, uint32_t sample_n,
                                 uint32_t sample_m, float std_scale, const float *rand_deg, float *means, float *stds, void *stream) {
    NLR_CHECK_ARG(tdist && means && stds, "cast_contract: NULL tensor");
    if (N == 0 || S == 0) return NLR_OK;
    CastParams cp;
    int rc = nlr_fill_cast_params(&cp, rays, tdist, rand_deg, N, S, sample_n, sample_m, std_scale);
    if (rc) return rc;
    const size_t total = (size_t)N * S * sample_n;
    hipLaunchKernelGGL(nlr_cast_contract_kernel, dim3((unsigned)((total + 255) / 256)), dim3(256), 0, (hipStream_t)stream, cp, means, stds);
    NLR_LAUNCH_CHECK("nlr_cast_contract_kernel");
    return NLR_OK;
}

int nlr_fill_cast_params(CastParams *cp, const NlrRays *rays, const float *tdist, const float *rand_deg, uint32_t N,
                         uint32_t S, uint32_t n, uint32_t mloops, float std_scale) {
    NLR_CHECK_ARG(n >= 1 && n <= NLR_MAX_MULTI, "cast: sample_n=%u outside [1,%d]", n, NLR_MAX_MULTI);
    NLR_CHECK_ARG(rays && rays->origins && rays->directions && rays->radii && rays->base_x && rays->base_y,
                  "cast: ray batch has NULL origins/directions/radii/base_x/base_y");
    memset(cp, 0, sizeof(*cp));
    cp->origins = rays->origins;
    cp->directions = rays->directions;
    cp->base_x = rays->base_x;
    cp->base_y = rays->base_y;
    cp->radii = rays->radii;
    cp->tdist = tdist;
    cp->rand_deg = rand_deg;
    cp->N = N;
    cp->S = S;
    cp->n = n;
    cp->std_scale = std_scale;
    for (uint32_t j = 0; j < n; ++j) {
        const float deg = ((float)(2.0 * M_PI * (double)mloops) * (float)j) / (float)n;
        cp->degj[j] = deg;
        cp->cosd[j] = cosf(deg);
        cp->sind[j] = sinf(deg);
    }
    return NLR_OK;
}

#include <atomic>
#define NLR_DBG_KEYS 11
static std::atomic<int> nlr_debug_switch[NLR_DBG_KEYS] = {{0}, {0}, {0}, {0}, {0}, {0}, {0}, {0}, {0}, {0}, {0}};
extern "C" int nlr_debug_set(uint32_t key, int value) {
    NLR_CHECK_ARG(key < NLR_DBG_KEYS, "debug_set: unknown key %u", key);
    nlr_debug_switch[key].store(value);
    return NLR_OK;
}
extern "C" int nlr_debug_get(uint32_t key) { return key < NLR_DBG_KEYS ? nlr_debug_switch[key].load() : 0; }
static bool nlr_force_generic() { return nlr_debug_switch[NLR_DBG_FORCE_GENERIC].load() != 0; }

extern "C" int nlr_grid_fast_path(const int32_t *offsets_host, uint32_t L, uint32_t C, float S, uint32_t H, int table_dtype, uint32_t gridtype,
                                  int align_corners, uint32_t interp) {
    GridParams gp;
    if (!offsets_host || nlr_fill_grid_params(&gp, offsets_host, table_dtype, offsets_host, L, C, S, H, gridtype, align_corners, interp)) return 0;
    return nlr_level_fast_ok(gp) ? 1 : 0;
}

#ifdef NLR_DBG_ENV
static void nlr_dbg_upload(hipStream_t st) {
    int v[8] = {0, 99, 0, 0, 0, 0, 0, 0};
    if (const char *e = getenv("NLR_ENC_LO")) v[0] = atoi(e);
    if (const char *e = getenv("NLR_ENC_HI")) v[1] = atoi(e);
    if (const char *e = getenv("NLR_ENC_NOSCALAR")) v[3] = atoi(e);
    if (const char *e = getenv("NLR_ENC_NT")) v[4] = (int)strtol(e, nullptr, 0);
    if (const char *e = getenv("NLR_ENC_SWEEPW")) v[2] = atoi(e);
    if (const char *e = getenv("NLR_ENC_TILEB")) v[5] = atoi(e);
    if (const char *e = getenv("NLR_ENC_TILEA")) v[6] = atoi(e);
    (void)hipMemcpyToSymbolAsync(HIP_SYMBOL(nlr_dbg), v, sizeof(v), 0, hipMemcpyHostToDevice, st);
}
#endif

int nlr_launch_encode(const CastParams &cp, const GridParams &gp, int re_weights, float *feat, int piece_major, hipStream_t st) {
#ifdef NLR_DBG_ENV
    nlr_dbg_upload(st);
#endif
    NLR_CHECK_ARG(nlr_slot_count(cp) * 8 < (1ull << 32), "encode: N * S = %llu samples do not fit the 32-bit lane index (chunk the rays)",
                  (unsigned long long)cp.N * cp.S);
    const uint32_t M = cp.N * cp.S;
    if (cp.n <= 8) {
        dim3 grid8((uint32_t)((nlr_slot_count(cp) * 8 + 255) / 256)), block8(256);
        const bool fast = nlr_level_fast_ok(gp) && !nlr_force_generic();
        uint32_t chunk = NLR_XCD_CHUNK;
        dim3 gridp = grid8;
#ifdef NLR_DBG_ENV
        if (const char *e = getenv("NLR_ENC_CHUNK")) chunk = (uint32_t)atoi(e);
        if (const char *e = getenv("NLR_ENC_PERSIST")) gridp.x = (uint32_t)atoi(e) * 256u < grid8.x ? (uint32_t)atoi(e) * 256u : grid8.x;
#endif
#define NLR_ENC8(T, C)                                                                                                               \
    do {                                                                                                                             \
        if (fast) hipLaunchKernelGGL((nlr_encode8_kernel<T, C>), gridp, block8, 0, st, cp, gp, re_weights, feat, piece_major, grid8.x, chunk); \
        else hipLaunchKernelGGL((nlr_encode8g_kernel<T, C>), grid8, block8, 0, st, cp, gp, re_weights, feat, piece_major);           \
    } while (0)
        if (gp.table_dtype == 0) {
            switch (gp.C) {
                case 1: NLR_ENC8(float, 1); break;
                case 2: NLR_ENC8(float, 2); break;
                case 4: NLR_ENC8(float, 4); break;
                default: NLR_ENC8(float, 8); break;
            }
        } else {
            switch (gp.C) {
                case 1: NLR_ENC8(__half, 1); break;
                case 2: NLR_ENC8(__half, 2); break;
                case 4: NLR_ENC8(__half, 4); break;
                default: NLR_ENC8(__half, 8); break;
            }
        }
#undef NLR_ENC8
        NLR_LAUNCH_CHECK("nlr_encode8_kernel");
        return NLR_OK;
    }
    dim3 grid((M + 255) / 256, gp.L), block(256);
#define NLR_ENC(T, C) hipLaunchKernelGGL((nlr_encode_kernel<T, C>), grid, block, 0, st, cp, gp, re_weights, feat)
    if (gp.table_dtype == 0) {
        switch (gp.C) {
            case 1: NLR_ENC(float, 1); break;
            case 2: NLR_ENC(float, 2); break;
            case 4: NLR_ENC(float, 4); break;
            default: NLR_ENC(float, 8); break;
        }
    } else {
        switch (gp.C) {
            case 1: NLR_ENC(__half, 1); break;
            case 2: NLR_ENC(__half, 2); break;
            case 4: NLR_ENC(__half, 4); break;
            default: NLR_ENC(__half, 8); break;
        }
    }
#undef NLR_ENC
    NLR_LAUNCH_CHECK("nlr_encode_kernel");
    return NLR_OK;
}

int nlr_launch_prop(const CastParams &cp, const GridParams &gp, const float *w1, const float *b1, const float *w2, float b2,
                    float density_bias, int re_weights, float *density, float *feat_out, hipStream_t st) {
    NLR_CHECK_ARG(nlr_slot_count(cp) * 8 < (1ull << 32), "proposal level: N * S = %llu samples do not fit the 32-bit lane index (chunk the rays)",
                  (unsigned long long)cp.N * cp.S);
    const uint32_t M = cp.N * cp.S;
#ifdef NLR_DBG_ENV
    nlr_dbg_upload(st);
#endif
    PropMlpParams mp;
    mp.w1 = w1;
    mp.b1 = b1;
    mp.w2 = w2;
    mp.b2 = b2;
    mp.density_bias = density_bias;
    mp.F = gp.L * gp.C;
    NLR_CHECK_ARG(mp.F <= 16, "proposal MLP: L*C = %u > 16 features is outside the fused proposal kernel", mp.F);
    if (cp.n <= 8) {
        dim3 grid8((uint32_t)((nlr_slot_count(cp) * 8 + 255) / 256)), block8(256);
        const bool fast = nlr_level_fast_ok(gp) && !nlr_force_generic();
        uint32_t chunk = NLR_XCD_CHUNK;
        dim3 gridp = grid8;
#ifdef NLR_DBG_ENV
        if (const char *e = getenv("NLR_ENC_CHUNK")) chunk = (uint32_t)atoi(e);
        if (const char *e = getenv("NLR_ENC_PERSIST")) gridp.x = (uint32_t)atoi(e) * 256u < grid8.x ? (uint32_t)atoi(e) * 256u : grid8.x;
#endif
#define NLR_PROP8(T, C, LM)                                                                                                                    \
    do {                                                                                                                                       \
        if (fast) hipLaunchKernelGGL((nlr_prop8_kernel<T, C, LM>), gridp, block8, 0, st, cp, gp, mp, re_weights, density, feat_out, grid8.x, chunk); \
        else hipLaunchKernelGGL((nlr_prop8g_kernel<T, C, LM>), grid8, block8, 0, st, cp, gp, mp, re_weights, density, feat_out);               \
    } while (0)
        const bool f32t = gp.table_dtype == 0;
        if (gp.C == 1 && gp.L <= 8) { if (f32t) NLR_PROP8(float, 1, 8); else NLR_PROP8(__half, 1, 8); }
        else if (gp.C == 1) { if (f32t) NLR_PROP8(float, 1, 16); else NLR_PROP8(__half, 1, 16); }
        else if (gp.C == 2) { if (f32t) NLR_PROP8(float, 2, 8); else NLR_PROP8(__half, 2, 8); }
        else if (gp.C == 4 && gp.L <= 4) { if (f32t) NLR_PROP8(float, 4, 4); else NLR_PROP8(__half, 4, 4); }
        else NLR_FAIL(NLR_ERR_UNSUPPORTED, "proposal MLP: grid L=%u C=%u not supported by the fused proposal kernel", gp.L, gp.C);
#undef NLR_PROP8
        NLR_LAUNCH_CHECK("nlr_prop8_kernel");
        return NLR_OK;
    }
    dim3 grid((M + 255) / 256), block(256);
#define NLR_PROP(T, C, LM) hipLaunchKernelGGL((nlr_prop_kernel<T, C, LM>), grid, block, 0, st, cp, gp, mp, re_weights, density, feat_out)
    const bool f32 = gp.table_dtype == 0;
    if (gp.C == 1 && gp.L <= 8) { if (f32) NLR_PROP(float, 1, 8); else NLR_PROP(__half, 1, 8); }
    else if (gp.C == 1) { if (f32) NLR_PROP(float, 1, 16); else NLR_PROP(__half, 1, 16); }
    else if (gp.C == 2) { if (f32) NLR_PROP(float, 2, 8); else NLR_PROP(__half, 2, 8); }
    else if (gp.C == 4 && gp.L <= 4) { if (f32) NLR_PROP(float, 4, 4); else NLR_PROP(__half, 4, 4); }
    else NLR_FAIL(NLR_ERR_UNSUPPORTED, "proposal MLP: grid L=%u C=%u not supported by the fused proposal kernel", gp.L, gp.C);
#undef NLR_PROP
    NLR_LAUNCH_CHECK("nlr_prop_kernel");
    return NLR_OK;
}
```

### nerf-lidar_amd/csrc/nlr_grid.hip

```cpp
#include "nlr_common.h"
#include "nlr_grid_level.h"

#include <hip/hip_fp16.h>

void nlr_level_scale(uint32_t L, float S, uint32_t H, float *scale, uint32_t *resolution) {
    for (uint32_t l = 0; l < L; ++l) {
        float sc = exp2f((float)l * S) * (float)H - 1.0f;
        scale[l] = sc;
        resolution[l] = (uint32_t)ceilf(sc) + 1u;
    }
}

int nlr_fill_grid_params(GridParams *gp, const void *table, int table_dtype, const int32_t *offsets_host,
                         uint32_t L, uint32_t C, float S, uint32_t H, uint32_t gridtype, int align_corners,
                         uint32_t interp) {
    NLR_CHECK_ARG(L >= 1 && L <= NLR_MAX_GRID_LEVELS, "grid: num_levels %u outside [1,%d]", L, NLR_MAX_GRID_LEVELS);
    NLR_CHECK_ARG(C == 1 || C == 2 || C == 4 || C == 8, "GridEncoding: C must be 1, 2, 4, or 8 (got %u)", C);
    NLR_CHECK_ARG(table_dtype == 0 || table_dtype == 1, "grid: table_dtype must be 0 (f32) or 1 (f16)");
    NLR_CHECK_ARG(offsets_host != nullptr, "grid: offsets (host) is NULL");
    memset(gp, 0, sizeof(*gp));
    gp->table = table;
    gp->table_dtype = table_dtype;
    gp->L = L;
    gp->C = C;
    gp->gridtype = gridtype;
    gp->align_corners = align_corners ? 1u : 0u;
    gp->interp = interp;
    nlr_level_scale(L, S, H, gp->scale, gp->res);
    for (uint32_t l = 0; l < L; ++l) {
        NLR_CHECK_ARG(offsets_host[l + 1] > offsets_host[l], "grid: offsets must be increasing (level %u)", l);
        gp->offset[l] = (uint32_t)offsets_host[l];
        gp->hsize[l] = (uint32_t)(offsets_host[l + 1] - offsets_host[l]);
        double r = ceil((double)H * exp2((double)l * (double)S));
        gp->gsize[l] = (float)((int)r + (align_corners ? 0 : 1));
        gp->inv_gsize[l] = 1.0f / gp->gsize[l];
        uint64_t step = align_corners ? gp->res[l] : gp->res[l] + 1, stride = 1;
        int dense = 1;
        for (int d = 0; d < 3; ++d) {
            if (stride > gp->hsize[l]) break;
            stride *= step;
        }
        if (gridtype == 0 && stride > gp->hsize[l]) dense = 0;
        gp->dense[l] = dense;
        gp->step[l] = (uint32_t)step;
        const uint32_t hs = gp->hsize[l];
        const bool all3 = (step <= hs) && (step * step <= hs);
        if (all3 && step * step * step <= hs) gp->mode[l] = 0;
        else if (gridtype == 0 && (hs & (hs - 1)) == 0) gp->mode[l] = 1;
        else gp->mode[l] = 2;
    }
    return NLR_OK;
}

template <typename T>
__device__ __forceinline__ float ld(const T *p);
template <>
__device__ __forceinline__ float ld<float>(const float *p) { return *p; }
template <>
__device__ __forceinline__ float ld<__half>(const __half *p) { return __half2float(*p); }

template <typename T, int C, bool DYDX>
__global__ void __launch_bounds__(256) nlr_grid_fwd_kernel(const float *__restrict__ x, GridParams gp, float *__restrict__ out,
                                                           float *__restrict__ dy_dx, uint32_t B, int out_layout) {
    const uint32_t b = blockIdx.x * blockDim.x + threadIdx.x;
    if (b >= B) return;
    const uint32_t level = blockIdx.y;
    const uint32_t L = gp.L;
    const T *grid = (const T *)gp.table + (size_t)gp.offset[level] * C;
    float *o = out_layout == 0 ? out + ((size_t)level * B + b) * C : out + (size_t)b * L * C + level * C;
    float *dd = DYDX ? dy_dx + (size_t)b * 3 * L * C + (size_t)level * 3 * C : nullptr;

    const float x0 = x[(size_t)b * 3 + 0], x1 = x[(size_t)b * 3 + 1], x2 = x[(size_t)b * 3 + 2];
    const bool oob = (x0 < 0 || x0 > 1) || (x1 < 0 || x1 > 1) || (x2 < 0 || x2 > 1);
    if (oob) {
#pragma unroll
        for (int c = 0; c < C; ++c) o[c] = 0.0f;
        if (DYDX)
            for (int i = 0; i < 3 * C; ++i) dd[i] = 0.0f;
        return;
    }
    const uint32_t hsize = gp.hsize[level], res = gp.res[level];
    const float scale = gp.scale[level];
    const float half = gp.align_corners ? 0.0f : 0.5f;
    float pos[3] = {fmaf(x0, scale, half), fmaf(x1, scale, half), fmaf(x2, scale, half)};
    uint32_t pg[3];
    float pd[3];
#pragma unroll
    for (int d = 0; d < 3; ++d) {
        pg[d] = (uint32_t)floorf(pos[d]);
        pos[d] -= (float)pg[d];
        if (gp.interp == 1) {
            pd[d] = 6 * pos[d] * (1.0f - pos[d]);
            pos[d] = pos[d] * pos[d] * (3.0f - 2.0f * pos[d]);
        } else {
            pd[d] = 1.0f;
        }
    }
    uint32_t idx[8];
    float w[8];
#pragma unroll
    for (int c8 = 0; c8 < 8; ++c8) {
        float ww = 1.0f;
        uint32_t pl[3];
#pragma unroll
        for (int d = 0; d < 3; ++d) {
            if ((c8 >> d) & 1) {
                ww *= pos[d];
                pl[d] = pg[d] + 1;
            } else {
                ww *= 1 - pos[d];
                pl[d] = pg[d];
            }
        }
        w[c8] = ww;
        idx[c8] = nlr_grid_index(gp.gridtype, gp.align_corners, hsize, res, pl[0], pl[1], pl[2]) * C;
    }
    float g[8][C];
#pragma unroll
    for (int c8 = 0; c8 < 8; ++c8)
#pragma unroll
        for (int c = 0; c < C; ++c) g[c8][c] = ld<T>(grid + idx[c8] + c);
    float r[C];
#pragma unroll
    for (int c = 0; c < C; ++c) r[c] = 0.0f;
#pragma unroll
    for (int c8 = 0; c8 < 8; ++c8)
#pragma unroll
        for (int c = 0; c < C; ++c) r[c] = fmaf(w[c8], g[c8][c], r[c]);
#pragma unroll
    for (int c = 0; c < C; ++c) o[c] = r[c];

    if (DYDX) {
#pragma unroll
        for (int gd = 0; gd < 3; ++gd) {
            float rg[C];
#pragma unroll
            for (int c = 0; c < C; ++c) rg[c] = 0.0f;
#pragma unroll
            for (int i4 = 0; i4 < 4; ++i4) {
                float ww = scale;
                uint32_t pl[3];
#pragma unroll
                for (int nd = 0; nd < 2; ++nd) {
                    const int d = (nd >= gd) ? nd + 1 : nd;
                    if ((i4 >> nd) & 1) {
                        ww *= pos[d];
                        pl[d] = pg[d] + 1;
                    } else {
                        ww *= 1 - pos[d];
                        pl[d] = pg[d];
                    }
                }
                pl[gd] = pg[gd];
                const uint32_t il = nlr_grid_index(gp.gridtype, gp.align_corners, hsize, res, pl[0], pl[1], pl[2]) * C;
                pl[gd] = pg[gd] + 1;
                const uint32_t ir = nlr_grid_index(gp.gridtype, gp.align_corners, hsize, res, pl[0], pl[1], pl[2]) * C;
#pragma unroll
                for (int c = 0; c < C; ++c) rg[c] += ww * (ld<T>(grid + ir + c) - ld<T>(grid + il + c)) * pd[gd];
            }
#pragma unroll
            for (int c = 0; c < C; ++c) dd[gd * C + c] = rg[c];
        }
    }
}

template <typename T, int C>
static int launch_fwd(const float *x, const GridParams &gp, float *out, float *dy_dx, uint32_t B, int out_layout,
                      hipStream_t st) {
    dim3 grid((B + 255) / 256, gp.L), block(256);
    if (dy_dx)
        hipLaunchKernelGGL((nlr_grid_fwd_kernel<T, C, true>), grid, block, 0, st, x, gp, out, dy_dx, B, out_layout);
    else
        hipLaunchKernelGGL((nlr_grid_fwd_kernel<T, C, false>), grid, block, 0, st, x, gp, out, dy_dx, B, out_layout);
    NLR_LAUNCH_CHECK("nlr_grid_fwd_kernel");
    return NLR_OK;
}

extern "C" int nlr_grid_encode_forward(const float *inputs, const void *embeddings, int table_dtype,
                                       const int32_t *offsets_host, float *outputs, uint32_t B, uint32_t D,
                                       uint32_t C, uint32_t L, float S, uint32_t H, float *dy_dx, uint32_t gridtype,
                                       int align_corners, uint32_t interp, int out_layout, void *stream) {
    NLR_CHECK_ARG(D == 3, "GridEncoding: this build supports input_dim D = 3 only (got %u)", D);
    NLR_CHECK_ARG(inputs && embeddings && outputs, "grid_encode_forward: NULL tensor");
    NLR_CHECK_ARG(out_layout == 0 || out_layout == 1, "grid_encode_forward: out_layout must be 0 or 1");
    NLR_CHECK_ARG(gridtype <= 1 && interp <= 1, "grid_encode_forward: gridtype/interp out of range");
    if (B == 0) return NLR_OK;
    GridParams gp;
    int rc = nlr_fill_grid_params(&gp, embeddings, table_dtype, offsets_host, L, C, S, H, gridtype, align_corners, interp);
    if (rc) return rc;
    hipStream_t st = (hipStream_t)stream;
#define NLR_DISPATCH_C(T)                                                          \
    switch (C) {                                                                   \
        case 1: return launch_fwd<T, 1>(inputs, gp, outputs, dy_dx, B, out_layout, st); \
        case 2: return launch_fwd<T, 2>(inputs, gp, outputs, dy_dx, B, out_layout, st); \
        case 4: return launch_fwd<T, 4>(inputs, gp, outputs, dy_dx, B, out_layout, st); \
        default: return launch_fwd<T, 8>(inputs, gp, outputs, dy_dx, B, out_layout, st); \
    }
    if (table_dtype == 0) { NLR_DISPATCH_C(float) } else { NLR_DISPATCH_C(__half) }
#undef NLR_DISPATCH_C
}

#define NLR_LDS_TABLE_FLOATS 36864
#define NLR_LDS_CACHE_MAX_STEP 129u
__host__ __device__ __forceinline__ int nlr_level_lds_kind(const GridParams &gp, uint32_t level, uint32_t C, int no_cache) {
    if (gp.mode[level] == 0 && gp.hsize[level] * C <= NLR_LDS_TABLE_FLOATS) return 1;
    if (!no_cache && C <= 4 && gp.mode[level] <= 1 && gp.step[level] <= NLR_LDS_CACHE_MAX_STEP) return 2;
    return 0;
}
__device__ __forceinline__ void nlr_corner_idx_any(const GridParams &gp, uint32_t level, const uint32_t (&pg)[3], uint32_t (&idx)[8]) {
    const uint32_t mode = gp.mode[level];
    if (mode == 0) nlr_corner_idx<0>(gp, level, pg, idx);
    else if (mode == 1) nlr_corner_idx<1>(gp, level, pg, idx);
    else nlr_corner_idx<2>(gp, level, pg, idx);
}
template <int C>
__global__ void __launch_bounds__(256) nlr_grid_bwd_kernel(const float *__restrict__ grad, const float *__restrict__ x,
                                                           GridParams gp, float *__restrict__ grad_table, uint32_t B,
                                                           int grad_layout, uint64_t level_list) {
    const uint32_t t = blockIdx.x * blockDim.x + threadIdx.x;
    const int lane = threadIdx.x & 63;
    constexpr uint32_t P = 64 / C;
    const uint32_t b0 = (t >> 6) * P + ((uint32_t)lane % P), ch = (uint32_t)lane / P;
    const uint32_t level = (uint32_t)(level_list >> (4 * blockIdx.y)) & 15u;
    const bool inb = b0 < B;
    const uint32_t b = inb ? b0 : B - 1;
    const float x0 = x[(size_t)b * 3 + 0], x1 = x[(size_t)b * 3 + 1], x2 = x[(size_t)b * 3 + 2];
    const bool valid = inb && !((x0 < 0 || x0 > 1) || (x1 < 0 || x1 > 1) || (x2 < 0 || x2 > 1));
    if (__ballot(valid) == 0ull) return;
    const float gc = grad_layout == 0 ? grad[((size_t)level * B + b) * C + ch] : grad[(size_t)b * gp.L * C + level * C + ch];
    float *gt = grad_table + (size_t)gp.offset[level] * C;
    const uint32_t hsize = gp.hsize[level], res = gp.res[level];
    const float scale = gp.scale[level];
    const float half = gp.align_corners ? 0.0f : 0.5f;
    float pos[3] = {fmaf(valid ? x0 : 0.5f, scale, half), fmaf(valid ? x1 : 0.5f, scale, half), fmaf(valid ? x2 : 0.5f, scale, half)};
    uint32_t pg[3];
#pragma unroll
    for (int d = 0; d < 3; ++d) {
        pg[d] = (uint32_t)floorf(pos[d]);
        pos[d] -= (float)pg[d];
        if (gp.interp == 1) pos[d] = pos[d] * pos[d] * (3.0f - 2.0f * pos[d]);
    }
#pragma unroll
    for (int c8 = 0; c8 < 8; ++c8) {
        float ww = 1.0f;
        uint32_t pl[3];
#pragma unroll
        for (int d = 0; d < 3; ++d) {
            if ((c8 >> d) & 1) {
                ww *= pos[d];
                pl[d] = pg[d] + 1;
            } else {
                ww *= 1 - pos[d];
                pl[d] = pg[d];
            }
        }
        const uint32_t addr = nlr_grid_index(gp.gridtype, gp.align_corners, hsize, res, pl[0], pl[1], pl[2]) * C + ch;
        nlr_run_atomic<1>(gt, addr, ww * gc, valid, lane);
    }
}

template <int C>
__global__ void __launch_bounds__(256) nlr_grid_bwd_xpair_kernel(const float *__restrict__ grad, const float *__restrict__ x,
                                                                 GridParams gp, float *__restrict__ grad_table, uint32_t B,
                                                                 int grad_layout, uint64_t level_list, uint32_t level_mask) {
    static_assert(C == 1 || C == 2 || C == 4, "x-pair scatter: C in {1, 2, 4}");
    const uint32_t level = (uint32_t)(level_list >> (4 * blockIdx.y)) & 15u;
    if (level_mask && !((level_mask >> level) & 1u)) return;
    constexpr uint32_t P = 32 / C;
    const uint32_t w = (blockIdx.x * blockDim.x + threadIdx.x) >> 6;
    const int lane = threadIdx.x & 63;
    const uint32_t ch = (uint32_t)lane / (2 * P), xc = ((uint32_t)lane / P) & 1u, b0 = w * P + (uint32_t)lane % P;
    const bool inb = b0 < B;
    const uint32_t b = inb ? b0 : B - 1;
    const float x0 = x[(size_t)b * 3 + 0], x1 = x[(size_t)b * 3 + 1], x2 = x[(size_t)b * 3 + 2];
    const bool valid = inb && !((x0 < 0 || x0 > 1) || (x1 < 0 || x1 > 1) || (x2 < 0 || x2 > 1));
    if (__ballot(valid) == 0ull) return;
    const float gc = grad_layout == 0 ? grad[((size_t)level * B + b) * C + ch] : grad[(size_t)b * gp.L * C + level * C + ch];
    float *gt = grad_table + (size_t)gp.offset[level] * C;
    const uint32_t hsize = gp.hsize[level], res = gp.res[level];
    const float scale = gp.scale[level];
    const float half = gp.align_corners ? 0.0f : 0.5f;
    float pos[3] = {fmaf(valid ? x0 : 0.5f, scale, half), fmaf(valid ? x1 : 0.5f, scale, half), fmaf(valid ? x2 : 0.5f, scale, half)};
    uint32_t pg[3];
#pragma unroll
    for (int d = 0; d < 3; ++d) {
        pg[d] = (uint32_t)floorf(pos[d]);
        pos[d] -= (float)pg[d];
        if (gp.interp == 1) pos[d] = pos[d] * pos[d] * (3.0f - 2.0f * pos[d]);
    }
    const float wx = xc ? pos[0] : 1 - pos[0];
    const uint32_t px = pg[0] + xc;
#pragma unroll
    for (int c4 = 0; c4 < 4; ++c4) {
        const float wy = (c4 & 1) ? pos[1] : 1 - pos[1], wz = (c4 & 2) ? pos[2] : 1 - pos[2];
        const uint32_t addr = nlr_grid_index(gp.gridtype, gp.align_corners, hsize, res, px, pg[1] + (c4 & 1), pg[2] + (c4 >> 1)) * C + ch;
        nlr_run_atomic<1>(gt, addr, ((1.0f * wx) * wy) * wz * gc, valid, lane);
    }
}

template <int C>
__global__ void __launch_bounds__(1024) nlr_grid_bwd_lds_kernel(const float *__restrict__ grad, const float *__restrict__ x, GridParams gp,
                                                               float *__restrict__ grad_table, uint32_t B, int grad_layout, uint32_t direct_mask,
                                                               uint32_t cache_mask) {
    __shared__ float acc[NLR_LDS_TABLE_FLOATS];
    const uint32_t level = blockIdx.y;
    const bool direct = (direct_mask >> level) & 1u;
    if (!direct && !((cache_mask >> level) & 1u)) return;
    constexpr uint32_t NS = NLR_LDS_TABLE_FLOATS / (C + 1);
    uint32_t *tags = (uint32_t *)(acc + NS * C);
    const uint32_t cells = direct ? gp.hsize[level] * C : NS * C;
    for (uint32_t i = threadIdx.x; i < cells; i += blockDim.x) acc[i] = 0.0f;
    if (!direct)
        for (uint32_t i = threadIdx.x; i < NS; i += blockDim.x) tags[i] = 0xffffffffu;
    __syncthreads();
    float *gt = grad_table + (size_t)gp.offset[level] * C;

    const float scale = gp.scale[level];
    const float half = gp.align_corners ? 0.0f : 0.5f;
    constexpr uint32_t P = 64 / C;
    const int lane = threadIdx.x & 63;
    const uint32_t ch = (uint32_t)lane / P, pl0 = (uint32_t)lane % P;
    const uint32_t nwaves = gridDim.x * (blockDim.x >> 6), groups = (B + P - 1) / P;
    const uint32_t g0 = (uint32_t)__builtin_amdgcn_readfirstlane((int)(blockIdx.x * (blockDim.x >> 6) + (threadIdx.x >> 6)));
    float nx0 = 0, nx1 = 0, nx2 = 0, ngc = 0;
    auto fetch = [&](uint32_t g) {
        const uint32_t bb = g * P + pl0 < B ? g * P + pl0 : B - 1;
        nx0 = x[(size_t)bb * 3 + 0], nx1 = x[(size_t)bb * 3 + 1], nx2 = x[(size_t)bb * 3 + 2];
        ngc = grad_layout == 0 ? grad[((size_t)level * B + bb) * C + ch] : grad[(size_t)bb * gp.L * C + level * C + ch];
    };
    if (g0 < groups) fetch(g0);
    for (uint32_t g = g0; g < groups; g += nwaves) {
        const bool inb = g * P + pl0 < B;
        const float x0 = nx0, x1 = nx1, x2 = nx2, gc = ngc;
        if (g + nwaves < groups) fetch(g + nwaves);
        const bool valid = inb && !((x0 < 0 || x0 > 1) || (x1 < 0 || x1 > 1) || (x2 < 0 || x2 > 1));
        float pos[3] = {fmaf(valid ? x0 : 0.5f, scale, half), fmaf(valid ? x1 : 0.5f, scale, half), fmaf(valid ? x2 : 0.5f, scale, half)};
        uint32_t pg[3];
#pragma unroll
        for (int d = 0; d < 3; ++d) {
            pg[d] = (uint32_t)floorf(pos[d]);
            pos[d] -= (float)pg[d];
            if (gp.interp == 1) pos[d] = pos[d] * pos[d] * (3.0f - 2.0f * pos[d]);
        }
        uint32_t cidx[8];
        nlr_corner_idx_any(gp, level, pg, cidx);
        const NlrRuns runs = nlr_cell_runs(pg, valid, lane);
        float vv[8];
        bool tail[8];
#pragma unroll
        for (int c8 = 0; c8 < 8; ++c8) {
            float ww = 1.0f;
#pragma unroll
            for (int d = 0; d < 3; ++d) ww *= ((c8 >> d) & 1) ? pos[d] : 1 - pos[d];
            vv[c8] = nlr_runs_sum(runs, ww * gc);
            tail[c8] = runs.tail;
        }
        if (direct) {
#pragma unroll
            for (int c8 = 0; c8 < 8; ++c8)
                if (tail[c8]) atomicAdd(&acc[cidx[c8] * C + ch], vv[c8]);
        } else {
            uint32_t slot[8], was[8];
#pragma unroll
            for (int c8 = 0; c8 < 8; ++c8) {
                slot[c8] = __umulhi(cidx[c8] * 2654435761u, NS);
                was[c8] = tail[c8] ? atomicCAS(&tags[slot[c8]], 0xffffffffu, cidx[c8]) : 0u;
            }
#pragma unroll
            for (int c8 = 0; c8 < 8; ++c8)
                if (tail[c8]) {
                    if (was[c8] == 0xffffffffu || was[c8] == cidx[c8]) atomicAdd(&acc[slot[c8] * C + ch], vv[c8]);
                    else atomicAdd(gt + (size_t)cidx[c8] * C + ch, vv[c8]);
                }
        }
    }
    __syncthreads();
    if (direct) {
        for (uint32_t i = threadIdx.x; i < cells; i += blockDim.x) {
            const float v = acc[i];
            if (v != 0.0f) atomicAdd(gt + i, v);
        }
    } else {
        for (uint32_t i = threadIdx.x; i < cells; i += blockDim.x) {
            const uint32_t tag = tags[i / C];
            const float v = acc[i];
            if (tag != 0xffffffffu && v != 0.0f) atomicAdd(gt + (size_t)tag * C + i % C, v);
        }
    }
}

#define NLR_BIN_FLOATS 32768u
#define NLR_BIN_CHUNK 8192u
#define NLR_BIN_SPLIT 16u
#define NLR_BIN_MAXB 256u

struct BinArgs {
    uint32_t nlev;
    uint32_t level[NLR_MAX_GRID_LEVELS];
    uint32_t nb[NLR_MAX_GRID_LEVELS];
    uint32_t nchunks, shift;
    uint32_t split;
    uint32_t *counts, *starts;
    uint32_t *item_idx;
    float *item_val;
};

template <int C>
__global__ void __launch_bounds__(256) nlr_grid_bwd_bin_kernel(const float *__restrict__ grad, const float *__restrict__ x, GridParams gp,
                                                               uint32_t B, int grad_layout, BinArgs a) {
    __shared__ uint32_t cnt[NLR_BIN_MAXB], cur[NLR_BIN_MAXB];
    const uint32_t chunk = blockIdx.x, li = blockIdx.y, level = a.level[li], nb = a.nb[li];
    const int lane = threadIdx.x & 63;
    for (uint32_t i = threadIdx.x; i < NLR_BIN_MAXB; i += 256) cnt[i] = 0;
    __syncthreads();

    const float scale = gp.scale[level];
    const float half = gp.align_corners ? 0.0f : 0.5f;
    const size_t region = ((size_t)li * a.nchunks + chunk) * (NLR_BIN_CHUNK * 8);
    const uint32_t emask = (1u << a.shift) - 1u;
    for (int pass = 0; pass < 2; ++pass) {
        for (uint32_t it = 0; it < NLR_BIN_CHUNK; it += 256) {
            const uint32_t b0 = chunk * NLR_BIN_CHUNK + it + threadIdx.x;
            const bool inb = b0 < B;
            const uint32_t b = inb ? b0 : B - 1;
            const float x0 = x[(size_t)b * 3 + 0], x1 = x[(size_t)b * 3 + 1], x2 = x[(size_t)b * 3 + 2];
            const bool valid = inb && !((x0 < 0 || x0 > 1) || (x1 < 0 || x1 > 1) || (x2 < 0 || x2 > 1));
            float g[C];
#pragma unroll
            for (int c = 0; c < C; ++c)
                g[c] = grad_layout == 0 ? grad[((size_t)level * B + b) * C + c] : grad[(size_t)b * gp.L * C + level * C + c];
            float pos[3] = {fmaf(valid ? x0 : 0.5f, scale, half), fmaf(valid ? x1 : 0.5f, scale, half), fmaf(valid ? x2 : 0.5f, scale, half)};
            uint32_t pg[3];
#pragma unroll
            for (int d = 0; d < 3; ++d) {
                pg[d] = (uint32_t)floorf(pos[d]);
                pos[d] -= (float)pg[d];
                if (gp.interp == 1) pos[d] = pos[d] * pos[d] * (3.0f - 2.0f * pos[d]);
            }
            uint32_t cidx[8];
            nlr_corner_idx_any(gp, level, pg, cidx);
            const NlrRuns runs = nlr_cell_runs(pg, valid, lane);
#pragma unroll
            for (int c8 = 0; c8 < 8; ++c8) {
                float ww = 1.0f;
#pragma unroll
                for (int d = 0; d < 3; ++d) ww *= ((c8 >> d) & 1) ? pos[d] : 1 - pos[d];
                const uint32_t idx = cidx[c8];
                float v[C];
#pragma unroll
                for (int c = 0; c < C; ++c) v[c] = nlr_runs_sum(runs, ww * g[c]);
                if (runs.tail) {
                    const uint32_t bucket = idx >> a.shift;
                    if (pass == 0) {
                        atomicAdd(&cnt[bucket], 1u);
                    } else {
                        const size_t p = region + atomicAdd(&cur[bucket], 1u);
                        a.item_idx[p] = idx & emask;
#pragma unroll
                        for (int c = 0; c < C; ++c) a.item_val[p * C + c] = v[c];
                    }
                }
            }
        }
        __syncthreads();
        if (pass == 0) {
            if (threadIdx.x == 0) {
                uint32_t run = 0;
                for (uint32_t i = 0; i < nb; ++i) {
                    cur[i] = run;
                    run += cnt[i];
                }
            }
            __syncthreads();
            for (uint32_t i = threadIdx.x; i < nb; i += 256) {
                const size_t o = ((size_t)li * NLR_BIN_MAXB + i) * a.nchunks + chunk;
                a.counts[o] = cnt[i];
                a.starts[o] = cur[i];
            }
            __syncthreads();
        }
    }
}

template <int C>
__global__ void __launch_bounds__(1024) nlr_grid_bwd_acc_kernel(GridParams gp, float *__restrict__ grad_table, BinArgs a) {
    extern __shared__ float acc[];
    const uint32_t bucket = blockIdx.x, li = blockIdx.y, split = blockIdx.z;
    if (bucket >= a.nb[li]) return;
    const uint32_t level = a.level[li];
    for (uint32_t i = threadIdx.x; i < NLR_BIN_FLOATS; i += 1024) acc[i] = 0.0f;
    __syncthreads();
    const int lane = threadIdx.x & 63;
    const uint32_t wave = split * 16 + (threadIdx.x >> 6), nwaves = a.split * 16;
    const uint32_t *cn = a.counts + ((size_t)li * NLR_BIN_MAXB + bucket) * a.nchunks;
    const uint32_t *st = a.starts + ((size_t)li * NLR_BIN_MAXB + bucket) * a.nchunks;
    for (uint32_t c0 = wave * 8; c0 < a.nchunks; c0 += nwaves * 8) {
        const uint32_t mine = c0 + (lane & 7) < a.nchunks ? c0 + (lane & 7) : a.nchunks - 1;
        const uint32_t my_n = c0 + (lane & 7) < a.nchunks ? cn[mine] : 0u, my_s = st[mine];
        const uint32_t lim = a.nchunks - c0 < 8 ? a.nchunks - c0 : 8;
        for (uint32_t j = 0; j < lim; ++j) {
            const uint32_t n = __builtin_amdgcn_readlane(my_n, j), s0 = __builtin_amdgcn_readlane(my_s, j);
            const size_t base = ((size_t)li * a.nchunks + (c0 + j)) * (NLR_BIN_CHUNK * 8) + s0;
            for (uint32_t i = lane; i < n; i += 256) {
                uint32_t e[4];
                float v[4][C];
#pragma unroll
                for (int u = 0; u < 4; ++u) {
                    const uint32_t k = i + u * 64 < n ? i + u * 64 : i;
                    e[u] = a.item_idx[base + k];
#pragma unroll
                    for (int c = 0; c < C; ++c) v[u][c] = a.item_val[(base + k) * C + c];
                }
#pragma unroll
                for (int u = 0; u < 4; ++u)
                    if (i + u * 64 < n) {
#pragma unroll
                        for (int c = 0; c < C; ++c) atomicAdd(&acc[e[u] * C + c], v[u][c]);
// ... 250 lines not shown
```

### nerf-lidar_amd/csrc/nlr_kernels.h

```cpp
#pragma once
#include "nlr_common.h"

#define NLR_MAX_MULTI 16

struct CastParams {
    const float *origins, *directions, *base_x, *base_y, *radii;
    const float *tdist;
    const float *rand_deg;
    uint32_t N, S, n;
    uint32_t ray_groups, vote_min;
    const uint32_t *votes;
    float std_scale;
    float cosd[NLR_MAX_MULTI], sind[NLR_MAX_MULTI];
    float degj[NLR_MAX_MULTI];
};

struct CompositeParams {
    const float *density, *tdist, *dirs, *rgb, *sem, *inten, *far, *origins;
    uint32_t N, S, K;
    int opaque, extras;
    float bg, scale_factor;
    float *weights;
    float *o_rgb, *o_depth, *o_sem, *o_int, *o_acc, *o_dmean, *o_dmed, *o_p5, *o_p95, *o_points, *level_depth;
    int32_t *o_labels;
    const float *seg;
    uint32_t no_rgb;
    uint32_t seg_int;
    float *o_packed;
    uint32_t pk_h, pk_w;
};

typedef float f32x16 __attribute__((ext_vector_type(16)));
typedef float f32x4 __attribute__((ext_vector_type(4)));
typedef __bf16 bf16x8 __attribute__((ext_vector_type(8)));

struct TileH {
    bf16x8 f[2];
};

struct MlpParams {
    const float *feat;
    int feat_piece_major;
    uint32_t M, S, F;
    const uint4 *tape;
    uint32_t tape_chunks;
    const float *bias_all;
    uint32_t bias_count;
    const float *enc;
    uint32_t depth;
    uint32_t K, int_row;
    float density_bias, rgb_premul, rgb_bias, rgb_padding;
    float *density, *rgb, *sem, *inten;
    const float *tdist;
    const float *dnorm;
    float *seg;
    uint32_t opaque;
    uint32_t lidar;
};

struct DirEncParams {
    const float *viewdirs;
    const float *dirs;
    uint32_t N, deg, E;
    float *out;
    float *dnorm;
};
int nlr_launch_dnorm(const float *dirs, uint32_t N, float *dnorm, hipStream_t st);

int nlr_launch_resample(const float *prev_sdist, const float *prev_weights, uint32_t n_prev, float dilation, float anneal,
                        float pad, uint32_t S, const float *u_dev, const float *jitter, float max_jitter, const float *near,
                        const float *far, float lam, uint32_t N, float *sdist, float *tdist, hipStream_t st);
int nlr_fill_cast_params(CastParams *cp, const NlrRays *rays, const float *tdist, const float *rand_deg, uint32_t N,
                         uint32_t S, uint32_t n, uint32_t mloops, float std_scale);
int nlr_launch_encode(const CastParams &cp, const GridParams &gp, int re_weights, float *feat, int piece_major, hipStream_t st);
int nlr_launch_ray_vote(const float *tdist, uint32_t N, uint32_t S, uint32_t *votes, hipStream_t st);
int nlr_launch_prop(const CastParams &cp, const GridParams &gp, const float *w1, const float *b1, const float *w2, float b2,
                    float density_bias, int re_weights, float *density, float *feat_out, hipStream_t st);
int nlr_launch_direnc(const DirEncParams &P, hipStream_t st);
int nlr_launch_mlp(const MlpParams &P, uint32_t W, uint32_t WB, uint32_t HT, uint32_t prec, uint32_t cus, hipStream_t st);
bool nlr_mlp_can_composite(uint32_t W, uint32_t WB, uint32_t HT, uint32_t prec, uint32_t F, uint32_t S, uint32_t K, bool use_int, uint64_t M,
                           uint32_t mode = 1);
int nlr_launch_composite(const CompositeParams &P, hipStream_t st);
int nlr_composite_segments(const float *density, const float *tdist, const float *directions, const float *seg, uint32_t class_num,
                           int has_intensity, const float *far, const float *origins, uint32_t N, uint32_t S, int opaque_background,
                           float bg, int compute_extras, float scale_factor, float *weights, const NlrOut *out, float *level_depth,
                           hipStream_t st, bool no_rgb = false);
int nlr_composite_level_impl(const float *density, const float *tdist, const float *directions, const float *rgb, const float *semantic,
                             const float *intensity, const float *far, const float *origins, uint32_t N, uint32_t S, uint32_t class_num,
                             int opaque_background, float bg, int compute_extras, float scale_factor, float *weights, const NlrOut *out,
                             float *level_depth, hipStream_t st, bool no_rgb);
```

### nerf-lidar_amd/csrc/nlr_level_fast.h

```cpp
#pragma once
#include "nlr_grid_level.h"

typedef float nlr_f2 __attribute__((ext_vector_type(2)));
#ifdef NLR_DBG_ENV
__device__ int nlr_dbg[8] = {0, 99, 0, 0, 0, 0, 0, 0};
#endif

template <typename T, int C>
struct NlrEntry;
template <>
struct NlrEntry<float, 1> {
    static constexpr int E = 2;
    static __device__ __forceinline__ void ld(const char *base, uint32_t off, float (&v)[1]) { v[0] = *(const float *)(base + off); }
};
template <>
struct NlrEntry<float, 2> {
    static constexpr int E = 3;
    static __device__ __forceinline__ void ld(const char *base, uint32_t off, float (&v)[2]) {
        const float2 t = *(const float2 *)(base + off);
        v[0] = t.x, v[1] = t.y;
    }
};
typedef float nlr_f4 __attribute__((ext_vector_type(4)));
template <>
struct NlrEntry<float, 4> {
    static constexpr int E = 4;
    static __device__ __forceinline__ void ld(const char *base, uint32_t off, float (&v)[4]) {
        const float4 t = *(const float4 *)(base + off);
        v[0] = t.x, v[1] = t.y, v[2] = t.z, v[3] = t.w;
    }
    static __device__ __forceinline__ void ld_nt(const char *base, uint32_t off, float (&v)[4]) {
        const nlr_f4 t = __builtin_nontemporal_load((const nlr_f4 *)(base + off));
        v[0] = t.x, v[1] = t.y, v[2] = t.z, v[3] = t.w;
    }
};
template <>
struct NlrEntry<float, 8> {
    static constexpr int E = 5;
    static __device__ __forceinline__ void ld(const char *base, uint32_t off, float (&v)[8]) {
        const float4 t = *(const float4 *)(base + off), u = *(const float4 *)(base + off + 16);
        v[0] = t.x, v[1] = t.y, v[2] = t.z, v[3] = t.w, v[4] = u.x, v[5] = u.y, v[6] = u.z, v[7] = u.w;
    }
};
template <>
struct NlrEntry<__half, 1> {
    static constexpr int E = 1;
    static __device__ __forceinline__ void ld(const char *base, uint32_t off, float (&v)[1]) { v[0] = __half2float(*(const __half *)(base + off)); }
};
template <>
struct NlrEntry<__half, 2> {
    static constexpr int E = 2;
    static __device__ __forceinline__ void ld(const char *base, uint32_t off, float (&v)[2]) {
        const __half2 t = *(const __half2 *)(base + off);
        v[0] = __low2float(t), v[1] = __high2float(t);
    }
};
template <>
struct NlrEntry<__half, 4> {
    static constexpr int E = 3;
    static __device__ __forceinline__ void ld(const char *base, uint32_t off, float (&v)[4]) {
        const uint2 t = *(const uint2 *)(base + off);
        const uint32_t tx = t.x, ty = t.y;
        const __half2 a = __builtin_bit_cast(__half2, tx), b = __builtin_bit_cast(__half2, ty);
        v[0] = __low2float(a), v[1] = __high2float(a), v[2] = __low2float(b), v[3] = __high2float(b);
    }
};
template <>
struct NlrEntry<__half, 8> {
    static constexpr int E = 4;
    static __device__ __forceinline__ void ld(const char *base, uint32_t off, float (&v)[8]) {
        const uint4 t = *(const uint4 *)(base + off);
        const uint32_t w[4] = {t.x, t.y, t.z, t.w};
#pragma unroll
        for (int i = 0; i < 4; ++i) {
            const __half2 a = __builtin_bit_cast(__half2, w[i]);
            v[2 * i] = __low2float(a), v[2 * i + 1] = __high2float(a);
        }
    }
};

template <typename T, int C>
struct NlrPair {
    static constexpr bool ok = false;
    static __device__ __forceinline__ void ld(const char *, uint32_t, float (&)[C], float (&)[C]) {}
};
typedef float nlr_float2_a4 __attribute__((ext_vector_type(2), aligned(4)));
typedef float nlr_float4_a8 __attribute__((ext_vector_type(4), aligned(8)));
typedef uint32_t __attribute__((aligned(2))) nlr_u32_a2;
typedef uint32_t nlr_uint2_a4 __attribute__((ext_vector_type(2), aligned(4)));
typedef uint32_t nlr_uint4_a8 __attribute__((ext_vector_type(4), aligned(8)));
template <>
struct NlrPair<float, 1> {
    static constexpr bool ok = true;
    static __device__ __forceinline__ void ld(const char *base, uint32_t off, float (&a)[1], float (&b)[1]) {
        const nlr_float2_a4 t = *(const nlr_float2_a4 *)(base + off);
        a[0] = t.x, b[0] = t.y;
    }
};
template <>
struct NlrPair<float, 2> {
    static constexpr bool ok = true;
    static __device__ __forceinline__ void ld(const char *base, uint32_t off, float (&a)[2], float (&b)[2]) {
        const nlr_float4_a8 t = *(const nlr_float4_a8 *)(base + off);
        a[0] = t.x, a[1] = t.y, b[0] = t.z, b[1] = t.w;
    }
};
template <>
struct NlrPair<__half, 1> {
    static constexpr bool ok = true;
    static __device__ __forceinline__ void ld(const char *base, uint32_t off, float (&a)[1], float (&b)[1]) {
        const __half2 t = __builtin_bit_cast(__half2, (uint32_t) * (const nlr_u32_a2 *)(base + off));
        a[0] = __low2float(t), b[0] = __high2float(t);
    }
};
template <>
struct NlrPair<__half, 2> {
    static constexpr bool ok = true;
    static __device__ __forceinline__ void ld(const char *base, uint32_t off, float (&a)[2], float (&b)[2]) {
        const nlr_uint2_a4 t = *(const nlr_uint2_a4 *)(base + off);
        const uint32_t tx = t.x, ty = t.y;
        const __half2 p = __builtin_bit_cast(__half2, tx), q = __builtin_bit_cast(__half2, ty);
        a[0] = __low2float(p), a[1] = __high2float(p), b[0] = __low2float(q), b[1] = __high2float(q);
    }
};
template <>
struct NlrPair<__half, 4> {
    static constexpr bool ok = true;
    static __device__ __forceinline__ void ld(const char *base, uint32_t off, float (&a)[4], float (&b)[4]) {
        const nlr_uint4_a8 t = *(const nlr_uint4_a8 *)(base + off);
        const uint32_t w[4] = {t.x, t.y, t.z, t.w};
#pragma unroll
        for (int i = 0; i < 2; ++i) {
            const __half2 p = __builtin_bit_cast(__half2, w[i]), q = __builtin_bit_cast(__half2, w[2 + i]);
            a[2 * i] = __low2float(p), a[2 * i + 1] = __high2float(p), b[2 * i] = __low2float(q), b[2 * i + 1] = __high2float(q);
        }
    }
};

static inline bool nlr_level_fast_ok(const GridParams &gp) {
    if (gp.interp != 0 || gp.align_corners != 0) return false;
    const uint64_t entry = (uint64_t)gp.C * (gp.table_dtype == 0 ? 4 : 2);
    for (uint32_t l = 0; l < gp.L; ++l) {
        if (gp.mode[l] > 1) return false;
        if ((uint64_t)gp.hsize[l] * entry > (1ull << 32)) return false;
        if (gp.res[l] >= (1u << 30)) return false;
    }
    return true;
}

typedef uint32_t nlr_u2 __attribute__((ext_vector_type(2)));
typedef uint32_t nlr_u4 __attribute__((ext_vector_type(4)));
typedef uint32_t nlr_u8 __attribute__((ext_vector_type(8)));
template <int DW>
struct NlrSLoad8;
#define NLR_SLOAD8(DW, VT, OP)                                                                                                        \
    template <>                                                                                                                       \
    struct NlrSLoad8<DW> {                                                                                                            \
        typedef VT vt;                                                                                                                \
        static __device__ __forceinline__ void ld(const char *base, const uint32_t (&o)[8], VT (&q)[8]) {                             \
            asm volatile(OP " %0, %8, %9\n" OP " %1, %8, %10\n" OP " %2, %8, %11\n" OP " %3, %8, %12\n" OP " %4, %8, %13\n"      \
                         OP " %5, %8, %14\n" OP " %6, %8, %15\n" OP " %7, %8, %16\ns_waitcnt lgkmcnt(0)"                            \
                         : "=&s"(q[0]), "=&s"(q[1]), "=&s"(q[2]), "=&s"(q[3]), "=&s"(q[4]), "=&s"(q[5]), "=&s"(q[6]), "=&s"(q[7])      \
                         : "s"(base), "s"(o[0]), "s"(o[1]), "s"(o[2]), "s"(o[3]), "s"(o[4]), "s"(o[5]), "s"(o[6]), "s"(o[7])           \
                         : "memory");                                                                                                 \
        }                                                                                                                             \
    };
NLR_SLOAD8(1, uint32_t, "s_load_dword")
NLR_SLOAD8(2, nlr_u2, "s_load_dwordx2")
NLR_SLOAD8(4, nlr_u4, "s_load_dwordx4")
NLR_SLOAD8(8, nlr_u8, "s_load_dwordx8")
#undef NLR_SLOAD8
template <int DW>
__device__ __forceinline__ uint32_t nlr_dw(const typename NlrSLoad8<DW>::vt &q, int i) {
    if constexpr (DW == 1) return q;
    else return q[i];
}
template <typename T, int DW>
__device__ __forceinline__ float nlr_entry_ch(const typename NlrSLoad8<DW>::vt &q, int c) {
    if constexpr (sizeof(T) == 4) return __builtin_bit_cast(float, nlr_dw<DW>(q, c));
    else {
        const __half2 h = __builtin_bit_cast(__half2, nlr_dw<DW>(q, c >> 1));
        return (c & 1) ? __high2float(h) : __low2float(h);
    }
}

__device__ __forceinline__ uint32_t nlr_add_su(uint32_t v, uint32_t s) {
    uint32_t r;
    asm("v_add_u32 %0, %1, %2" : "=v"(r) : "s"(s), "v"(v));
    return r;
}

template <typename T, int C, int MODE>
__device__ __forceinline__ void nlr_level_fast(const GridParams &gp, uint32_t level, float x0, float x1, float x2, float werf, float (&a)[C]) {
    constexpr int E = NlrEntry<T, C>::E;
    constexpr int DW = (1 << E) / 4;
    const float scale = gp.scale[level];
    const char *base = (const char *)gp.table + ((size_t)gp.offset[level] << E);
    const float p0 = fmaf(x0, scale, 0.5f), p1 = fmaf(x1, scale, 0.5f), p2 = fmaf(x2, scale, 0.5f);
    const uint32_t g0 = (uint32_t)p0, g1 = (uint32_t)p1, g2 = (uint32_t)p2;
    const float f0 = __builtin_amdgcn_fractf(p0), f1 = __builtin_amdgcn_fractf(p1), f2 = __builtin_amdgcn_fractf(p2);
    const nlr_f2 wx = {1.0f - f0, f0};
    const float wy0 = 1.0f - f1, wz0 = 1.0f - f2;
    const nlr_f2 wxy0 = wx * wy0, wxy1 = wx * f1;
    const nlr_f2 w2[4] = {wxy0 * wz0, wxy1 * wz0, wxy0 * f2, wxy1 * f2};
    float r[C];
#pragma unroll
    for (int c = 0; c < C; ++c) r[c] = 0.0f;
    const uint32_t step = gp.step[level], sy = step << E, sz = (step * step) << E;
    const uint32_t hm = gp.hsize[level] - 1u, pa = 2654435761u & hm, pb = 805459861u & hm;
    const uint32_t mask = hm << E;
    bool uniform = false;
    uint32_t u0 = 0, u1 = 0, u2 = 0;
    if constexpr (DW >= 1) {
        u0 = __builtin_amdgcn_readfirstlane(g0), u1 = __builtin_amdgcn_readfirstlane(g1), u2 = __builtin_amdgcn_readfirstlane(g2);
        uniform = __builtin_amdgcn_ballot_w64((g0 != u0) | (g1 != u1) | (g2 != u2)) == 0ull;
#ifdef NLR_DBG_ENV
        if (nlr_dbg[3]) uniform = false;
#endif
    }
    if (uniform) {
        if constexpr (DW >= 1) {
            uint32_t so[8];
            if (MODE == 0) {
                const uint32_t ox = u0 << E, oy = u1 * sy, oz = u2 * sz;
#pragma unroll
                for (int c8 = 0; c8 < 8; ++c8) so[c8] = (ox + ((c8 & 1) << E)) + (oy + ((c8 & 2) ? sy : 0u)) + (oz + ((c8 & 4) ? sz : 0u));
            } else {
                const uint32_t hx = u0 << E, hy = (u1 << E) * pa, hz = (u2 << E) * pb;
#pragma unroll
                for (int c8 = 0; c8 < 8; ++c8)
                    so[c8] = ((hx + ((c8 & 1) << E)) ^ (hy + ((c8 & 2) ? (pa << E) : 0u)) ^ (hz + ((c8 & 4) ? (pb << E) : 0u))) & mask;
            }
            typename NlrSLoad8<DW>::vt q[8];
            NlrSLoad8<DW>::ld(base, so, q);
#pragma unroll
            for (int c8 = 0; c8 < 8; ++c8) {
                const float w = (c8 & 1) ? w2[c8 >> 1].y : w2[c8 >> 1].x;
#pragma unroll
                for (int c = 0; c < C; ++c) r[c] = fmaf(w, nlr_entry_ch<T, DW>(q[c8], c), r[c]);
            }
        }
    } else {
        uint32_t off[8];
        if (MODE == 0) {
            const uint32_t ox0 = g0 << E, ox1 = ox0 + (1u << E);
            const uint32_t oy0 = g1 * sy, oy1 = nlr_add_su(oy0, sy);
            const uint32_t oz0 = g2 * sz, oz1 = nlr_add_su(oz0, sz);
#pragma unroll
            for (int c8 = 0; c8 < 8; ++c8) off[c8] = ((c8 & 1) ? ox1 : ox0) + ((c8 & 2) ? oy1 : oy0) + ((c8 & 4) ? oz1 : oz0);
        } else {
            const uint32_t hx0 = g0 << E, hx1 = hx0 + (1u << E);
            const uint32_t hy0 = (g1 << E) * pa, hy1 = nlr_add_su(hy0, pa << E);
            const uint32_t hz0 = (g2 << E) * pb, hz1 = nlr_add_su(hz0, pb << E);
            const uint32_t yz[4] = {hy0 ^ hz0, hy1 ^ hz0, hy0 ^ hz1, hy1 ^ hz1};
#pragma unroll
            for (int c8 = 0; c8 < 8; ++c8) off[c8] = (((c8 & 1) ? hx1 : hx0) ^ yz[c8 >> 1]) & mask;
        }
        float v[8][C];
        if constexpr (MODE == 0 && NlrPair<T, C>::ok) {
#pragma unroll
            for (int c8 = 0; c8 < 8; c8 += 2) NlrPair<T, C>::ld(base, off[c8], v[c8], v[c8 + 1]);
        } else {
#ifdef NLR_DBG_ENV
            if constexpr (sizeof(T) == 4 && C == 4) {
                if ((nlr_dbg[4] >> level) & 1) {
#pragma unroll
                    for (int c8 = 0; c8 < 8; ++c8) NlrEntry<T, C>::ld_nt(base, off[c8], v[c8]);
                } else {
#pragma unroll
                    for (int c8 = 0; c8 < 8; ++c8) NlrEntry<T, C>::ld(base, off[c8], v[c8]);
                }
            } else
#endif
            {
#pragma unroll
                for (int c8 = 0; c8 < 8; ++c8) NlrEntry<T, C>::ld(base, off[c8], v[c8]);
            }
        }
#pragma unroll
        for (int c8 = 0; c8 < 8; ++c8) {
            const float w = (c8 & 1) ? w2[c8 >> 1].y : w2[c8 >> 1].x;
#pragma unroll
            for (int c = 0; c < C; ++c) r[c] = fmaf(w, v[c8][c], r[c]);
        }
    }
#pragma unroll
    for (int c = 0; c < C; ++c) a[c] = r[c] * werf;
}

#define NLR_DPP_ADD(R, CTRL) "v_add_f32_dpp " R ", " R ", " R " " CTRL " row_mask:0xf bank_mask:0xf\n"
#define NLR_Q1 "quad_perm:[1,0,3,2]"
#define NLR_Q2 "quad_perm:[2,3,0,1]"
#define NLR_HM "row_half_mirror"
__device__ __forceinline__ void nlr_group8_sum_n(float (&a)[1]) {
    asm volatile("s_nop 1\n" NLR_DPP_ADD("%0", NLR_Q1) "s_nop 1\n" NLR_DPP_ADD("%0", NLR_Q2) "s_nop 1\n" NLR_DPP_ADD("%0", NLR_HM) : "+v"(a[0]));
}
__device__ __forceinline__ void nlr_group8_sum_n(float (&a)[2]) {
    asm volatile("s_nop 1\n" NLR_DPP_ADD("%0", NLR_Q1) NLR_DPP_ADD("%1", NLR_Q1) "s_nop 0\n" NLR_DPP_ADD("%0", NLR_Q2) NLR_DPP_ADD("%1", NLR_Q2)
                 "s_nop 0\n" NLR_DPP_ADD("%0", NLR_HM) NLR_DPP_ADD("%1", NLR_HM)
                 : "+v"(a[0]), "+v"(a[1]));
}
__device__ __forceinline__ void nlr_group8_sum_n(float (&a)[4]) {
    asm volatile("s_nop 1\n" NLR_DPP_ADD("%0", NLR_Q1) NLR_DPP_ADD("%1", NLR_Q1) NLR_DPP_ADD("%2", NLR_Q1) NLR_DPP_ADD("%3", NLR_Q1)
                 NLR_DPP_ADD("%0", NLR_Q2) NLR_DPP_ADD("%1", NLR_Q2) NLR_DPP_ADD("%2", NLR_Q2) NLR_DPP_ADD("%3", NLR_Q2)
                 NLR_DPP_ADD("%0", NLR_HM) NLR_DPP_ADD("%1", NLR_HM) NLR_DPP_ADD("%2", NLR_HM) NLR_DPP_ADD("%3", NLR_HM)
                 : "+v"(a[0]), "+v"(a[1]), "+v"(a[2]), "+v"(a[3]));
}
#define NLR_DPP_ADD3(D, R, CTRL) "v_add_f32_dpp " D ", " R ", " R " " CTRL " row_mask:0xf bank_mask:0xf\n"
__device__ __forceinline__ void nlr_group8_sum_to(const float (&r)[4], float (&t)[4]) {
    asm volatile("s_nop 1\n" NLR_DPP_ADD3("%0", "%4", NLR_Q1) NLR_DPP_ADD3("%1", "%5", NLR_Q1) NLR_DPP_ADD3("%2", "%6", NLR_Q1) NLR_DPP_ADD3("%3", "%7", NLR_Q1)
                 NLR_DPP_ADD("%0", NLR_Q2) NLR_DPP_ADD("%1", NLR_Q2) NLR_DPP_ADD("%2", NLR_Q2) NLR_DPP_ADD("%3", NLR_Q2)
                 NLR_DPP_ADD("%0", NLR_HM) NLR_DPP_ADD("%1", NLR_HM) NLR_DPP_ADD("%2", NLR_HM) NLR_DPP_ADD("%3", NLR_HM)
                 : "=&v"(t[0]), "=&v"(t[1]), "=&v"(t[2]), "=&v"(t[3])
                 : "v"(r[0]), "v"(r[1]), "v"(r[2]), "v"(r[3]));
}
__device__ __forceinline__ void nlr_group8_sum_n(float (&a)[8]) {
    float lo[4] = {a[0], a[1], a[2], a[3]}, hi[4] = {a[4], a[5], a[6], a[7]};
    nlr_group8_sum_n(lo);
    nlr_group8_sum_n(hi);
#pragma unroll
    for (int i = 0; i < 4; ++i) a[i] = lo[i], a[4 + i] = hi[i];
}
template <int C>
__device__ __forceinline__ void nlr_group8_sum_to(const float (&r)[C], float (&t)[C]) {
#pragma unroll
    for (int c = 0; c < C; ++c) t[c] = r[c];
    nlr_group8_sum_n(t);
}
```

### nerf-lidar_amd/nerflidar_hip/_lib.py

```python
from __future__ import annotations

import ctypes as C
import os

_HERE = os.path.dirname(os.path.abspath(__file__))
LIB_PATH = os.environ.get("NLR_LIB_PATH") or os.path.join(_HERE, "libnerflidar_hip.so")

NLR_MAX_LEVELS = 4
NLR_MAX_VIEW_DEPTH = 16
PREC_F32, PREC_MIXED, PREC_FAST = 0, 1, 2

c_fp = C.c_void_p


class NlrLinear(C.Structure):
    _fields_ = [("weight", c_fp), ("bias", c_fp), ("out_features", C.c_uint32), ("in_features", C.c_uint32)]


class NlrGridDesc(C.Structure):
    _fields_ = [("table", c_fp), ("table_dtype", C.c_int32), ("num_levels", C.c_uint32), ("level_dim", C.c_uint32),
                ("base_resolution", C.c_uint32), ("log2_per_level_scale", C.c_float), ("offsets", c_fp),
                ("gridtype", C.c_uint32), ("align_corners", C.c_uint32), ("interp", C.c_uint32)]


class NlrMlpDesc(C.Structure):
    _fields_ = [("grid", NlrGridDesc), ("density0", NlrLinear), ("density2", NlrLinear), ("disable_rgb", C.c_uint32),
                ("bottleneck_width", C.c_uint32), ("net_depth_viewdirs", C.c_uint32), ("net_width_viewdirs", C.c_uint32),
                ("skip_layer_dir", C.c_uint32), ("deg_view", C.c_uint32), ("view", NlrLinear * NLR_MAX_VIEW_DEPTH),
                ("rgb_layer", NlrLinear), ("use_semantic", C.c_uint32), ("no_sem_layer", C.c_uint32),
                ("class_num", C.c_uint32), ("sem0", NlrLinear), ("sem2", NlrLinear), ("use_intensity", C.c_uint32),
                ("int0", NlrLinear), ("int2", NlrLinear), ("density_bias", C.c_float), ("rgb_premultiplier", C.c_float),
                ("rgb_bias", C.c_float), ("rgb_padding", C.c_float), ("re_weights", C.c_uint32)]


class NlrObjClassDesc(C.Structure):
    _fields_ = [("mlp", NlrMlpDesc), ("latent_size", C.c_uint32), ("split_latent", C.c_uint32), ("class_type", C.c_int32)]


class NlrObjectsDesc(C.Structure):
    _fields_ = [("n_classes", C.c_uint32), ("classes", C.POINTER(NlrObjClassDesc)), ("n_tracks", C.c_uint32), ("track_class", c_fp),
                ("latents", c_fp)]


class NlrModelDesc(C.Structure):
    _fields_ = [("num_levels", C.c_uint32), ("num_samples", C.c_uint32 * NLR_MAX_LEVELS),
                ("mlps", C.POINTER(NlrMlpDesc) * NLR_MAX_LEVELS), ("dilation_multiplier", C.c_float),
                ("dilation_bias", C.c_float), ("anneal_slope", C.c_float), ("resample_padding", C.c_float),
                ("power_lambda", C.c_float), ("std_scale", C.c_float), ("bg_intensity", C.c_float),
                ("opaque_background", C.c_uint32), ("mlp_precision", C.c_uint32)]


class NlrRays(C.Structure):
    _fields_ = [(k, c_fp) for k in ("origins", "directions", "viewdirs", "radii", "near", "far", "base_x", "base_y")]


class NlrRenderCfg(C.Structure):
    _fields_ = [("train_frac", C.c_float), ("compute_extras", C.c_uint32), ("sample_n", C.c_uint32),
                ("sample_m", C.c_uint32), ("rand_jitter", c_fp * NLR_MAX_LEVELS), ("rand_deg", c_fp * NLR_MAX_LEVELS),
                ("scale_factor", C.c_float), ("shuffled_rays", C.c_uint32)]


class NlrLevelOut(C.Structure):
    _fields_ = [(k, c_fp) for k in ("sdist", "tdist", "weights", "density", "rgb", "semantic", "intensity", "depth", "r_rgb", "r_acc",
                                    "r_distance_mean", "r_distance_median", "r_distance_percentile_5", "r_distance_percentile_95")]


class NlrOut(C.Structure):
    _fields_ = [(k, c_fp) for k in ("rgb", "depth", "semantic", "intensity", "acc", "distance_mean", "distance_median",
                                    "distance_percentile_5", "distance_percentile_95", "labels", "points", "packed")] + \
               [("packed_h", C.c_uint32), ("packed_w", C.c_uint32), ("history", NlrLevelOut * NLR_MAX_LEVELS)]


_lib = None

EXPORTS = ["nlr_last_error", "nlr_version", "nlr_build_sha", "nlr_debug_set", "nlr_debug_get", "nlr_grid_fast_path", "nlr_grid_encode_forward", "nlr_grid_encode_backward", "nlr_grad_total_variation", "nlr_level_scale",
           "nlr_sample_u", "nlr_model_create", "nlr_model_destroy", "nlr_model_set_table", "nlr_workspace_bytes",
           "nlr_render_rays", "nlr_kernel_names", "nlr_resample_level", "nlr_mlp_level", "nlr_composite_level",
           "nlr_profile_begin", "nlr_profile_begin_kinds", "nlr_profile_end", "nlr_range_workspace_bytes", "nlr_range_project",
           "nlr_composite_backward", "nlr_hash_decay_forward", "nlr_hash_decay_backward", "nlr_box_winner", "nlr_cast_contract",
           "nlr_track_box_params", "nlr_objects_create", "nlr_objects_destroy", "nlr_objects_workspace_bytes", "nlr_objects_apply",
           "nlr_render_rays_dynamic", "nlr_prop_mlp_forward", "nlr_prop_mlp_backward", "nlr_encode_features_forward",
           "nlr_encode_features_backward", "nlr_encode_features_backward_ws", "nlr_encode_features_backward_rays", "nlr_grid_encode_backward_ws", "nlr_grid_backward_workspace_bytes",
           "nlr_train_plan_create", "nlr_train_plan_destroy", "nlr_train_act_width", "nlr_train_param_layout", "nlr_train_linear_table",
           "nlr_train_pack",
           "nlr_mlp_train_forward", "nlr_mlp_train_backward", "nlr_mlp_train_wgrad_workspace_bytes", "nlr_mlp_train_wgrad",
           "nlr_mlp_train_forward_split", "nlr_mlp_train_backward_split", "nlr_mlp_train_wgrad_split",
           "nlr_render_lidar", "nlr_render_lidar_dynamic", "nlr_obj_frame_backward_workspace_bytes", "nlr_obj_frame_backward"]
NLR_K_COUNT = 6
DBG_FORCE_GENERIC, DBG_MLP_WORKGROUPS, DBG_BINNED_C4, DBG_NO_XPAIR_SCATTER, DBG_SCATTER_LEVELS, DBG_NO_SCATTER_CACHE, DBG_RAY_GROUPS = 0, 1, 2, 3, 4, 5, 6
DBG_LAST_ROUTE = 7
ROUTE_FULL, ROUTE_FULL_FUSED, ROUTE_LIDAR, ROUTE_LIDAR_FUSED = 1, 2, 3, 4
DBG_TRAIN_ROUTE, DBG_TRAIN_TRUNK_ROW0, DBG_TRAIN_TRUNK_ROWS = 8, 9, 10
TRAIN_FULL, TRAIN_TRUNK, TRAIN_BWD = 1, 2, 4


def lib():
    global _lib
    if _lib is None:
        if not os.path.exists(LIB_PATH):
            raise RuntimeError(f"{LIB_PATH} is missing: the HIP extension has not been built (make -C nerf-lidar_amd). "
                               "There is no CPU fallback for the render path.")
        L = C.CDLL(LIB_PATH)
        L.nlr_last_error.restype = C.c_char_p
        L.nlr_kernel_names.restype = C.c_char_p
        L.nlr_build_sha.restype = C.c_char_p
        L.nlr_version.restype = C.c_int
        L.nlr_workspace_bytes.restype = C.c_size_t
        L.nlr_workspace_bytes.argtypes = [c_fp, C.c_uint32]
        L.nlr_model_destroy.restype = None
        L.nlr_model_destroy.argtypes = [c_fp]
        L.nlr_model_create.argtypes = [C.POINTER(NlrModelDesc), C.POINTER(c_fp), c_fp]
        L.nlr_model_set_table.argtypes = [c_fp, C.c_uint32, c_fp, C.c_int]
        L.nlr_level_scale.restype = None
        L.nlr_level_scale.argtypes = [C.c_uint32, C.c_float, C.c_uint32, c_fp, c_fp]
        L.nlr_sample_u.restype = None
        L.nlr_sample_u.argtypes = [C.c_uint32, C.c_int, c_fp, c_fp]
        L.nlr_grid_encode_forward.argtypes = [c_fp, c_fp, C.c_int, c_fp, c_fp, C.c_uint32, C.c_uint32, C.c_uint32,
                                              C.c_uint32, C.c_float, C.c_uint32, c_fp, C.c_uint32, C.c_int, C.c_uint32,
                                              C.c_int, c_fp]
        L.nlr_grid_encode_backward.argtypes = [c_fp, c_fp, c_fp, c_fp, C.c_uint32, C.c_uint32, C.c_uint32, C.c_uint32,
                                               C.c_float, C.c_uint32, c_fp, c_fp, C.c_uint32, C.c_int, C.c_uint32,
                                               C.c_int, c_fp]
        L.nlr_grid_encode_backward_ws.argtypes = L.nlr_grid_encode_backward.argtypes[:-1] + [c_fp, C.c_size_t, c_fp]
        L.nlr_grid_backward_workspace_bytes.restype = C.c_size_t
        L.nlr_grid_backward_workspace_bytes.argtypes = [C.c_uint32, C.c_uint32, C.c_uint32, C.c_float, C.c_uint32, c_fp, C.c_uint32, C.c_int]
        L.nlr_debug_set.argtypes = [C.c_uint32, C.c_int]
        L.nlr_debug_get.argtypes = [C.c_uint32]
        L.nlr_grid_fast_path.argtypes = [c_fp, C.c_uint32, C.c_uint32, C.c_float, C.c_uint32, C.c_int, C.c_uint32, C.c_int, C.c_uint32]
        L.nlr_grad_total_variation.argtypes = [c_fp, c_fp, c_fp, c_fp, C.c_float, C.c_uint32, C.c_uint32, C.c_uint32, C.c_uint32, C.c_float,
                                               C.c_uint32, C.c_uint32, C.c_int, c_fp]
        L.nlr_render_rays.argtypes = [c_fp, C.POINTER(NlrRays), C.c_uint32, C.POINTER(NlrRenderCfg), C.POINTER(NlrOut),
                                      c_fp, C.c_size_t, c_fp]
        L.nlr_render_lidar.argtypes = L.nlr_render_rays.argtypes
        L.nlr_resample_level.argtypes = [c_fp, c_fp, C.c_uint32, C.c_float, C.c_float, C.c_float, C.c_uint32, c_fp, c_fp,
                                         c_fp, C.c_float, C.c_uint32, c_fp, c_fp, c_fp]
        L.nlr_mlp_level.argtypes = [c_fp, C.c_uint32, C.POINTER(NlrRays), c_fp, C.c_uint32, C.c_uint32, C.c_uint32, c_fp,
                                    c_fp, c_fp, c_fp, c_fp, c_fp, c_fp, C.c_size_t, c_fp]
        L.nlr_composite_level.argtypes = [c_fp, c_fp, c_fp, c_fp, c_fp, c_fp, c_fp, c_fp, C.c_uint32, C.c_uint32,
                                          C.c_uint32, C.c_int, C.c_float, C.c_int, C.c_float, c_fp, C.POINTER(NlrOut),
                                          c_fp, c_fp]
        L.nlr_range_workspace_bytes.restype = C.c_size_t
        L.nlr_range_workspace_bytes.argtypes = [C.c_uint32, C.c_uint32]
        L.nlr_range_project.argtypes = [c_fp, c_fp, c_fp, C.c_uint32, C.c_uint32, C.c_uint32, C.c_float, C.c_float, c_fp,
                                        C.c_size_t, c_fp, c_fp, c_fp, c_fp, c_fp, c_fp, c_fp]
        L.nlr_composite_backward.argtypes = [c_fp, c_fp, c_fp, c_fp, c_fp, c_fp, C.c_uint32, C.c_uint32, C.c_uint32, C.c_int,
                                             C.c_float, c_fp, c_fp, c_fp, c_fp, c_fp, c_fp, c_fp, c_fp, c_fp, c_fp, c_fp]
        L.nlr_hash_decay_forward.argtypes = [c_fp, c_fp, C.c_uint32, C.c_uint32, c_fp, c_fp]
        L.nlr_hash_decay_backward.argtypes = [c_fp, c_fp, C.c_uint32, C.c_uint32, C.c_float, c_fp, c_fp]
        L.nlr_cast_contract.argtypes = [C.POINTER(NlrRays), c_fp, C.c_uint32, C.c_uint32, C.c_uint32, C.c_uint32, C.c_float, c_fp, c_fp, c_fp,
                                        c_fp]
        L.nlr_box_winner.argtypes = [c_fp, c_fp, c_fp, c_fp, C.c_uint32, C.c_uint32, C.c_uint32, c_fp, c_fp]
        L.nlr_track_box_params.argtypes = [c_fp, c_fp, C.c_uint32, C.c_uint32, C.c_uint32, c_fp, c_fp]
        L.nlr_obj_frame_backward_workspace_bytes.restype = C.c_size_t
        L.nlr_obj_frame_backward_workspace_bytes.argtypes = [C.c_uint32, C.c_uint32, C.c_uint32]
        L.nlr_obj_frame_backward.argtypes = [c_fp] * 6 + [C.c_uint32] * 4 + [c_fp] * 3 + [C.c_uint32] + [c_fp] * 4 + [C.c_size_t, c_fp]
        L.nlr_objects_create.argtypes = [C.POINTER(NlrObjectsDesc), C.POINTER(c_fp), c_fp]
        L.nlr_objects_destroy.restype = None
        L.nlr_objects_destroy.argtypes = [c_fp]
        L.nlr_objects_workspace_bytes.restype = C.c_size_t
        L.nlr_objects_workspace_bytes.argtypes = [c_fp, C.c_uint32, C.c_uint32]
        L.nlr_objects_apply.argtypes = [c_fp, C.POINTER(NlrRays), c_fp, c_fp, C.c_uint32, C.c_uint32, C.c_uint32, c_fp, c_fp, c_fp,
                                        C.c_uint32, c_fp, c_fp, C.c_size_t, c_fp]
        L.nlr_render_rays_dynamic.argtypes = [c_fp, c_fp, C.POINTER(NlrRays), c_fp, C.c_uint32, C.c_uint32, C.POINTER(NlrRenderCfg),
                                              C.POINTER(NlrOut), C.POINTER(c_fp), c_fp, C.c_size_t, c_fp]
        L.nlr_render_lidar_dynamic.argtypes = L.nlr_render_rays_dynamic.argtypes
        L.nlr_prop_mlp_forward.argtypes = [c_fp] * 5 + [C.c_uint32, C.c_uint32, c_fp, c_fp]
        L.nlr_prop_mlp_backward.argtypes = [c_fp] * 6 + [C.c_uint32, C.c_uint32] + [c_fp] * 6
        L.nlr_encode_features_forward.argtypes = [C.POINTER(NlrRays), c_fp, C.c_uint32, C.c_uint32, C.c_uint32, C.c_uint32, C.c_float, c_fp,
                                                  C.POINTER(NlrGridDesc), C.c_uint32, c_fp, c_fp]
        L.nlr_encode_features_backward.argtypes = [C.POINTER(NlrRays), c_fp, C.c_uint32, C.c_uint32, C.c_uint32, C.c_uint32, C.c_float, c_fp,
                                                   C.POINTER(NlrGridDesc), C.c_uint32, c_fp, c_fp, c_fp, c_fp, c_fp]
        L.nlr_encode_features_backward_ws.argtypes = L.nlr_encode_features_backward.argtypes[:-1] + [c_fp, C.c_size_t, c_fp]
        L.nlr_encode_features_backward_rays.argtypes = L.nlr_encode_features_forward.argtypes[:10] + [c_fp] * 6
        L.nlr_train_plan_create.argtypes = [C.c_uint32] * 6 + [C.c_int, C.c_int] + [C.c_float] * 4 + [C.POINTER(c_fp), C.POINTER(C.c_uint32)]
        L.nlr_train_plan_destroy.restype = None
        L.nlr_train_plan_destroy.argtypes = [c_fp]
        L.nlr_train_act_width.restype = C.c_uint32
        L.nlr_train_act_width.argtypes = [c_fp]
        L.nlr_train_param_layout.argtypes = [c_fp, c_fp, C.c_uint32]
        L.nlr_train_linear_table.argtypes = [c_fp, c_fp, C.c_uint32]
        L.nlr_train_pack.argtypes = [c_fp, c_fp, c_fp]
        L.nlr_mlp_train_forward.argtypes = [c_fp, c_fp, c_fp, C.c_uint32, C.c_uint32, c_fp, c_fp, c_fp, c_fp, c_fp, c_fp]
        L.nlr_mlp_train_backward.argtypes = [c_fp, C.c_uint32, C.c_uint32] + [c_fp] * 11
        L.nlr_mlp_train_wgrad_workspace_bytes.restype = C.c_size_t
        L.nlr_mlp_train_wgrad_workspace_bytes.argtypes = [c_fp, C.c_uint32]
        L.nlr_mlp_train_wgrad.argtypes = [c_fp, C.c_uint32, C.c_uint32] + [c_fp] * 6 + [C.c_size_t, c_fp]
        L.nlr_mlp_train_forward_split.argtypes = [c_fp, c_fp, c_fp, C.c_uint32, C.c_uint32, C.c_uint32, c_fp, c_fp, c_fp, c_fp, c_fp, c_fp]
        L.nlr_mlp_train_backward_split.argtypes = [c_fp, C.c_uint32, C.c_uint32, C.c_uint32] + [c_fp] * 11
        L.nlr_mlp_train_wgrad_split.argtypes = [c_fp, C.c_uint32, C.c_uint32, C.c_uint32] + [c_fp] * 6 + [C.c_size_t, c_fp]
        L.nlr_profile_begin.argtypes = [c_fp]
        L.nlr_profile_begin_kinds.argtypes = [c_fp, C.c_uint32]
        L.nlr_profile_end.argtypes = [c_fp, c_fp, c_fp, c_fp]
        _lib = L
    return _lib


def check(rc: int, what: str = ""):
    if rc != 0:
        msg = lib().nlr_last_error().decode(errors="replace")
        raise RuntimeError(f"{what or 'libnerflidar_hip'} failed ({rc}): {msg}")


def ptr(t):
    return None if t is None else C.c_void_p(t.data_ptr())


def current_stream():
    import torch
    return C.c_void_p(torch.cuda.current_stream().cuda_stream)
```

### nerf-lidar_amd/nerflidar_hip/models.py

```python
from __future__ import annotations

import ctypes as C
from typing import Dict, List, Optional

import numpy as np
import torch

from . import _lib
from .config import MLPConfig, ModelConfig
from .weights import grid_layout, mlp_names, mlp_param_shapes

_RAY_KEYS = ("origins", "directions", "viewdirs", "radii", "near", "far", "base_x", "base_y")


def _f32c(a) -> np.ndarray:
    return np.ascontiguousarray(np.asarray(a, dtype=np.float32))


class Model:

    def __init__(self, mc: ModelConfig, state_dict: Dict[str, object], device="cuda:0",
                 precision: int = _lib.PREC_FAST, table_dtype=torch.float32):
        if mc.config.instance_obj:
            raise NotImplementedError("instance_obj=True (dynamic-object branch, ZI/models.py:306-315,401-477) "
                                      "is outside the fused path (SURVEY section 8f-1)")
        if mc.raydist_fn != "power_transformation":
            raise NotImplementedError("only raydist_fn='power_transformation' (the gin value) is supported")
        self.mc = mc
        self.config = mc.config
        self.device = torch.device(device)
        self.precision = precision
        self.training = False
        self.shuffled_rays = False
        self.num_levels = mc.num_levels
        self.tables: Dict[str, torch.Tensor] = {}
        self._keep = []
        self._handle = C.c_void_p(None)
        self._ws: Optional[torch.Tensor] = None
        sd = {k: (v.detach().cpu().numpy() if isinstance(v, torch.Tensor) else np.asarray(v)) for k, v in state_dict.items()}
        desc = _lib.NlrModelDesc()
        desc.num_levels = mc.num_levels
        samples = mc.level_samples()
        mlp_descs = []
        for li, (prefix, cfg) in enumerate(mlp_names(mc)):
            desc.num_samples[li] = samples[li]
            md = self._mlp_desc(prefix, cfg, sd, table_dtype)
            mlp_descs.append(md)
            desc.mlps[li] = C.pointer(md)
        desc.dilation_multiplier = mc.dilation_multiplier
        desc.dilation_bias = mc.dilation_bias
        desc.anneal_slope = mc.anneal_slope
        desc.resample_padding = mc.resample_padding
        desc.power_lambda = mc.power_lambda
        desc.std_scale = mc.std_scale
        lo, hi = mc.bg_intensity_range
        desc.bg_intensity = lo if lo == hi else (lo + hi) / 2
        desc.opaque_background = int(mc.opaque_background)
        desc.mlp_precision = precision
        with torch.cuda.device(self.device):
            rc = _lib.lib().nlr_model_create(C.byref(desc), C.byref(self._handle), _lib.current_stream())
        _lib.check(rc, "nlr_model_create")
        self._keep.clear()

    def _linear(self, sd, name) -> _lib.NlrLinear:
        w, b = _f32c(sd[name + ".weight"]), _f32c(sd[name + ".bias"])
        self._keep += [w, b]
        l = _lib.NlrLinear()
        l.weight = w.ctypes.data
        l.bias = b.ctypes.data
        l.out_features, l.in_features = w.shape
        return l

    def _mlp_desc(self, prefix: str, cfg: MLPConfig, sd, table_dtype) -> _lib.NlrMlpDesc:
        md = _lib.NlrMlpDesc()
        offsets, _, pls = grid_layout(cfg)
        emb = sd[f"{prefix}.encoder.embeddings"]
        if emb.shape != (int(offsets[-1]), cfg.grid_level_dim):
            raise RuntimeError(f"{prefix}.encoder.embeddings has shape {emb.shape}, expected "
                               f"{(int(offsets[-1]), cfg.grid_level_dim)}")
        table = torch.from_numpy(_f32c(emb)).to(self.device, table_dtype).contiguous()
        self.tables[prefix] = table
        off = np.ascontiguousarray(offsets, np.int32)
        self._keep.append(off)
        g = md.grid
        g.table = table.data_ptr()
        g.table_dtype = 0 if table_dtype == torch.float32 else 1
        g.num_levels, g.level_dim = cfg.grid_num_levels, cfg.grid_level_dim
        g.base_resolution = cfg.grid_base_resolution
        g.log2_per_level_scale = float(np.log2(pls))
        g.offsets = off.ctypes.data
        g.gridtype, g.align_corners, g.interp = 0, 0, 0
        md.density0 = self._linear(sd, f"{prefix}.density_layer.0")
        md.density2 = self._linear(sd, f"{prefix}.density_layer.2")
        md.disable_rgb = int(cfg.disable_rgb)
        md.bottleneck_width = cfg.bottleneck_width
        md.net_depth_viewdirs, md.net_width_viewdirs = cfg.net_depth_viewdirs, cfg.net_width_viewdirs
        md.skip_layer_dir, md.deg_view = cfg.skip_layer_dir, cfg.deg_view
        md.density_bias, md.rgb_premultiplier = cfg.density_bias, cfg.rgb_premultiplier
        md.rgb_bias, md.rgb_padding = cfg.rgb_bias, cfg.rgb_padding
        md.re_weights = int(cfg.re_weights)
        md.class_num = cfg.class_num
        if not cfg.disable_rgb:
            if cfg.net_depth_viewdirs > _lib.NLR_MAX_VIEW_DEPTH:
                raise RuntimeError("net_depth_viewdirs too large")
            for i in range(cfg.net_depth_viewdirs):
                md.view[i] = self._linear(sd, f"{prefix}.lin_second_stage_{i}")
            md.rgb_layer = self._linear(sd, f"{prefix}.rgb_layer")
            md.use_semantic, md.no_sem_layer = int(cfg.use_semantic), int(cfg.no_sem_layer)
            if cfg.use_semantic and not cfg.no_sem_layer:
                md.sem0 = self._linear(sd, f"{prefix}.sem_layer.0")
                md.sem2 = self._linear(sd, f"{prefix}.sem_layer.2")
            md.use_intensity = int(cfg.use_intensity)
            if cfg.use_intensity:
                md.int0 = self._linear(sd, f"{prefix}.intensity_layer.0")
                md.int2 = self._linear(sd, f"{prefix}.intensity_layer.2")
        return md

    def __del__(self):
        try:
            if self._handle:
                _lib.lib().nlr_model_destroy(self._handle)
                self._handle = C.c_void_p(None)
        except Exception:
            pass

    def eval(self):
        self.training = False
        return self

    def train(self, mode=True):
        self.training = mode
        return self

    def _workspace(self, n: int) -> torch.Tensor:
        need = _lib.lib().nlr_workspace_bytes(self._handle, n)
        if self._ws is None or self._ws.numel() < need:
            self._ws = torch.empty(need, dtype=torch.uint8, device=self.device)
        return self._ws

    def _render_call(self, rays, n: int, cfg, out, lidar_only: bool = False) -> None:
        ws = self._workspace(n)
        name = "nlr_render_lidar" if lidar_only else "nlr_render_rays"
        rc = getattr(_lib.lib(), name)(self._handle, C.byref(rays), n, C.byref(cfg), C.byref(out), _lib.ptr(ws), ws.numel(),
                                       _lib.current_stream())
        _lib.check(rc, name)

    def render_rays(self, batch: Dict[str, torch.Tensor], train_frac: float = 1.0, compute_extras: bool = True,
                    sample_n: int = 7, sample_m: int = 3, want_history: bool = False, scale_factor: float = 0.0,
                    rand_jitter: Optional[List[torch.Tensor]] = None, rand_deg: Optional[List[torch.Tensor]] = None,
                    packed: Optional[torch.Tensor] = None, lidar_only: bool = False):
        rays = _lib.NlrRays()
        n = batch["origins"].shape[0]
        keep = []
        for k in _RAY_KEYS:
            t = batch.get(k)
            if t is None and lidar_only and k == "viewdirs":
                continue
            if t is None:
                raise RuntimeError(f"batch['{k}'] is missing")
            if not t.is_cuda:
                raise RuntimeError(f"batch['{k}'] must be a CUDA tensor (no CPU fallback)")
            t = t.reshape(n, -1).contiguous().float()
            keep.append(t)
            setattr(rays, k, t.data_ptr())
        dev, f32 = self.device, torch.float32
        K = self.mc.nerf_mlp.class_num if self.config.use_semantic else 0
        new = lambda *shape, dtype=f32: torch.empty(*shape, device=dev, dtype=dtype)
        out = _lib.NlrOut()
        r: Dict[str, torch.Tensor] = {"depth": new(n)} if lidar_only else {"rgb": new(n, 3), "depth": new(n)}
        if K:
            r["semantic"] = new(n, K)
        if self.config.use_intensity:
            r["intensity"] = new(n)
        if compute_extras:
            for k in ("acc", "distance_mean", "distance_median", "distance_percentile_5", "distance_percentile_95"):
                r[k] = new(n)
        if scale_factor > 0:
            r["points"] = new(n, 3)
            if K:
                r["labels"] = new(n, dtype=torch.int32)
        for k, t in r.items():
            setattr(out, k, t.data_ptr())
        if packed is not None:
            if not (packed.is_cuda and packed.dtype == f32 and packed.is_contiguous() and packed.numel() == n * 7):
                raise RuntimeError("packed must be a contiguous float32 CUDA tensor with 7 values per ray")
            out.packed = packed.data_ptr()
            if packed.dim() == 3:
                out.packed_w, out.packed_h = int(packed.shape[0]), int(packed.shape[1])
            r["packed"] = packed
        hist: List[Dict[str, torch.Tensor]] = []
        samples = self.mc.level_samples()
        for li, S in enumerate(samples):
            h: Dict[str, torch.Tensor] = {"depth": new(n)}
            if want_history:
                h.update(sdist=new(n, S + 1), tdist=new(n, S + 1), weights=new(n, S), density=new(n, S))
                if li < len(samples) - 1:
                    h.update(r_rgb=new(n, 3), r_acc=new(n))
                    if compute_extras:
                        for k in ("distance_mean", "distance_median", "distance_percentile_5", "distance_percentile_95"):
                            h["r_" + k] = new(n)
                if li == len(samples) - 1:
                    if not lidar_only:
                        h["rgb"] = new(3, n, S)
                    if K:
                        h["semantic"] = new(K, n, S)
                    if self.config.use_intensity:
                        h["intensity"] = new(n, S)
            for k, t in h.items():
                setattr(out.history[li], k, t.data_ptr())
            hist.append(h)
        cfg = _lib.NlrRenderCfg()
        cfg.train_frac = float(train_frac)
        cfg.compute_extras = int(compute_extras)
        cfg.sample_n, cfg.sample_m = sample_n, sample_m
        cfg.scale_factor = float(scale_factor)
        cfg.shuffled_rays = int(bool(getattr(self, "shuffled_rays", False)))
        for li in range(len(samples)):
            if rand_jitter is not None:
                t = rand_jitter[li].reshape(n).contiguous().float()
                keep.append(t)
                cfg.rand_jitter[li] = t.data_ptr()
            if rand_deg is not None:
                t = rand_deg[li].reshape(n, samples[li], sample_n).contiguous().float()
                keep.append(t)
                cfg.rand_deg[li] = t.data_ptr()
        with torch.cuda.device(dev):
            self._render_call(rays, n, cfg, out, lidar_only)
        if want_history:
            last = hist[-1]
            if "rgb" in last:
                last["rgb"] = last["rgb"].permute(1, 2, 0)
            if "semantic" in last:
                last["semantic"] = last["semantic"].permute(1, 2, 0)
        return r, hist

    def forward(self, rand, batch, train_frac, compute_extras, zero_glo=True, sample_n=7, sample_m=3, step=0,
                max_step=25000, curr_track=None):
        n = batch["origins"].shape[0]
        samples = self.mc.level_samples()
        rj = rd = None
        if rand:
            gen = rand if isinstance(rand, torch.Generator) else None
            rj = [torch.rand(n, 1, device=self.device, generator=gen) for _ in samples]
            rd = [torch.rand(n, S, sample_n, device=self.device, generator=gen) for S in samples]
        r, hist = self.render_rays(batch, train_frac, compute_extras, sample_n, sample_m, want_history=True,
                                   rand_jitter=rj, rand_deg=rd)
        renderings = []
        for li, h in enumerate(hist):
            last = li == len(hist) - 1
            rend = dict(r) if last else dict(depth=h["depth"], **{k[2:]: v for k, v in h.items() if k.startswith("r_")})
            if compute_extras:
                nv = self.config.vis_num_rays
                rend["ray_sdist"] = h["sdist"][:nv]
                rend["ray_weights"] = h["weights"][:nv]
                rend["ray_rgbs"] = hist[-1]["rgb"][:nv] if last else None
            renderings.append(rend)
        if compute_extras:
            final_rgb = torch.sum(renderings[-1]["ray_rgbs"] * renderings[-1]["ray_weights"][..., None], dim=-2)
            for li in range(len(hist) - 1):
                S = samples[li]
                renderings[li]["ray_rgbs"] = torch.broadcast_to(final_rgb[:, None, :], (final_rgb.shape[0], S, 3))
        ray_history = [{k: v for k, v in h.items() if k != "depth" and not k.startswith("r_")} for h in hist]
        return renderings, ray_history

    __call__ = forward


class CapturedRender:

    def __init__(self, model: "Model", batch: Dict[str, torch.Tensor], **kw):
        self.model, self.batch = model, batch
        side = torch.cuda.Stream(model.device)
        self.graph = torch.cuda.CUDAGraph()
        model._ws = None
        with torch.cuda.stream(side):
            model.render_rays(batch, **kw)
            side.synchronize()
            with torch.cuda.graph(self.graph, stream=side):
                self.out, self.hist = model.render_rays(batch, **kw)
        self._ws = model._ws
        model._ws = None
        torch.cuda.current_stream(model.device).wait_stream(side)

    def replay(self):
        self.graph.replay()
        return self.out


class _SingleProcess:
    process_index = 0
    num_processes = 1
    is_main_process = True

    def gather(self, t):
        return t


def _chunk_plan(total: int, chunk: int, world: int, rank: int):
    plan = []
    for first in range(0, total, chunk):
        count = min(chunk, total - first)
        share = -(-count // world)
        plan.append((first, count, rank * share, (rank + 1) * share))
    return plan


def _rows(flat: Dict[str, torch.Tensor], first: int, count: int, lo: int, hi: int) -> Dict[str, torch.Tensor]:
    real = max(min(hi, count) - lo, 0)
    out = {}
    for k, v in flat.items():
        part = v[first + lo:first + lo + real]
        if real < hi - lo:
            part = torch.cat([part, v.new_zeros((hi - lo - real,) + tuple(v.shape[1:]))])
        out[k] = part
    return out


class _Assembler:

    def __init__(self, total: int):
        self.total = total
        self.buffers: Dict[str, object] = {}

    def put(self, key: str, first: int, value):
        if isinstance(value, list):
            slot = self.buffers.setdefault(key, [[] for _ in value])
            for parts, v in zip(slot, value):
                parts.append(v)
            return
        buf = self.buffers.get(key)
        if buf is None:
            buf = self.buffers[key] = value.new_empty((self.total,) + tuple(value.shape[1:]))
        buf[first:first + value.shape[0]] = value


def _gather_packed(acc, tensors: List[torch.Tensor], world: int) -> List[torch.Tensor]:
    flat = torch.cat([t.reshape(-1).to(torch.float32) for t in tensors])
    got = acc.gather(flat[None])
    out, off = [], 0
    for t in tensors:
        n = t.numel()
        out.append(got[:, off:off + n].reshape((world * t.shape[0],) + tuple(t.shape[1:])).to(t.dtype))
        off += n
    return out


@torch.no_grad()
def render_image(model: Model, accelerator, batch, rand, config, train_frac=1, verbose=True, return_weights=False,
                 image=True, render_instance=False, instance_id=None, packed_gather=True):
    if render_instance:
        raise NotImplementedError("render_instance: the reference's Model.obj_rendering stops in a pdb.set_trace() and then reads an unassigned "
                                  "variable (ZI/obj_utils.py:216-217, reached from ZI/models.py:662); there is no behaviour to reproduce")
    acc = accelerator or _SingleProcess()
    world, rank = acc.num_processes, acc.process_index
    lead = tuple(batch["origins"].shape[:2]) if image else (batch["origins"].shape[0],)
    total = int(np.prod(lead))
    flat = {k: v.reshape(total, -1) for k, v in batch.items() if v is not None}
    model.eval()
    out = _Assembler(total)
    for first, count, lo, hi in _chunk_plan(total, config.render_chunk_size, world, rank):
        renderings, ray_history = model(rand, _rows(flat, first, count, lo, hi), train_frac=train_frac,
                                        compute_extras=True, zero_glo=True)

        items = []
        for key, val in renderings[-1].items():
# ... 37 lines not shown
```

Before: 5.384 million rays/s.

## Bake hash-grid levels into per-cell 8-corner records for single-load trilinear fetch

Adds a model-creation-time bake that, for each grid level whose size fits a 64 MiB budget, stores all 8 corner entries of every cell contiguously. The encode fast path then reads one 16/32-byte vector (or a scalar load when the wavefront is uniform) instead of 8 scattered gathers. This trades extra device memory (8x duplication per baked level) and a one-time bake kernel for fewer, coalesced memory transactions per sample. Baking is on by default in the Python Model, and set_table invalidates the records.

```diff
diff --git a/include/nerflidar_hip.h b/include/nerflidar_hip.h
--- a/include/nerflidar_hip.h
+++ b/include/nerflidar_hip.h
@@ -106,6 +106,11 @@
 int nlr_model_create(const NlrModelDesc *desc, NlrModel **out, void *stream);
 void nlr_model_destroy(NlrModel *m);
 int nlr_model_set_table(NlrModel *m, uint32_t level, const void *table_dev, int table_dtype);
+#define NLR_CELL_RECORD_BUDGET_MIB 64
+int nlr_model_bake_tables(NlrModel *m, void *stream);
+size_t nlr_model_baked_bytes(const NlrModel *m);
+size_t nlr_cell_records_host(const void *table_host, int table_dtype, const int32_t *offsets_host, uint32_t L, uint32_t C, float S,
+                             uint32_t H, uint32_t gridtype, uint32_t level, void *records_host, size_t records_bytes);
 
 typedef struct NlrRays {
     const float *origins, *directions, *viewdirs;
@@ -168,6 +173,7 @@
 #define NLR_DBG_TRAIN_ROUTE 8
 #define NLR_DBG_TRAIN_TRUNK_ROW0 9
 #define NLR_DBG_TRAIN_TRUNK_ROWS 10
+#define NLR_DBG_CELL_BUDGET_MIB 11
 int nlr_debug_set(uint32_t key, int value);
 int nlr_debug_get(uint32_t key);
 int nlr_grid_fast_path(const int32_t *offsets_host, uint32_t L, uint32_t C, float S, uint32_t H, int table_dtype, uint32_t gridtype,
diff --git a/nerf-lidar_amd/csrc/nlr_api.hip b/nerf-lidar_amd/csrc/nlr_api.hip
--- a/nerf-lidar_amd/csrc/nlr_api.hip
+++ b/nerf-lidar_amd/csrc/nlr_api.hip
@@ -64,6 +64,8 @@
     uint32_t bias_count = 0;
     float *u_det = nullptr, *u_rand = nullptr;
     float max_jitter = 0.0f;
+    void *rec[NLR_MAX_GRID_LEVELS] = {};
+    size_t rec_bytes[NLR_MAX_GRID_LEVELS] = {};
 };
 
 struct NlrModel {
@@ -426,8 +428,55 @@
     return NLR_OK;
 }
 
+static void drop_record(LevelModel &lv, uint32_t l) {
+    if (lv.rec[l]) (void)hipFree(lv.rec[l]);
+    lv.rec[l] = nullptr;
+    lv.rec_bytes[l] = 0;
+    lv.gp.rec[l] = nullptr;
+    lv.gp.rec_mask &= ~(1u << l);
+}
+
+extern "C" int nlr_model_bake_tables(NlrModel *m, void *stream) {
+    NLR_CHECK_ARG(m != nullptr, "model_bake_tables: NULL model");
+    const int dbg = nlr_debug_get(NLR_DBG_CELL_BUDGET_MIB);
+    const size_t budget = (size_t)(dbg > 0 ? dbg : NLR_CELL_RECORD_BUDGET_MIB) << 20;
+    hipStream_t st = (hipStream_t)stream;
+    for (uint32_t i = 0; i < m->num_levels; ++i) {
+        LevelModel &lv = m->lv[i];
+        const bool fast = nlr_grid_fast_ok(lv.gp);
+        for (uint32_t l = 0; l < lv.gp.L; ++l) {
+            const size_t bytes = fast ? nlr_cell_record_bytes(lv.gp, l) : 0;
+            if (!bytes || bytes > budget) {
+                drop_record(lv, l);
+                continue;
+            }
+            if (lv.rec_bytes[l] != bytes) {
+                drop_record(lv, l);
+                NLR_HIP(hipMalloc(&lv.rec[l], bytes));
+                lv.rec_bytes[l] = bytes;
+            }
+            lv.gp.rec_mask &= ~(1u << l);
+            if (int rc = nlr_launch_bake_level(lv.gp, l, lv.rec[l], st)) return rc;
+            lv.gp.rec[l] = lv.rec[l];
+            lv.gp.rec_mask |= 1u << l;
+        }
+    }
+    NLR_HIP(hipStreamSynchronize(st));
+    return NLR_OK;
+}
+
+extern "C" size_t nlr_model_baked_bytes(const NlrModel *m) {
+    size_t b = 0;
+    if (m)
+        for (uint32_t i = 0; i < m->num_levels; ++i)
+            for (uint32_t l = 0; l < NLR_MAX_GRID_LEVELS; ++l) b += m->lv[i].rec_bytes[l];
+    return b;
+}
+
 extern "C" void nlr_model_destroy(NlrModel *m) {
     if (!m) return;
+    for (uint32_t i = 0; i < NLR_MAX_LEVELS; ++i)
+        for (uint32_t l = 0; l < NLR_MAX_GRID_LEVELS; ++l) drop_record(m->lv[i], l);
     for (void *p : m->allocs) (void)hipFree(p);
     delete m;
 }
@@ -437,6 +486,7 @@
     NLR_CHECK_ARG(table_dtype == 0 || table_dtype == 1, "model_set_table: table_dtype must be 0 or 1");
     m->lv[level].gp.table = table_dev;
     m->lv[level].gp.table_dtype = table_dtype;
+    for (uint32_t l = 0; l < NLR_MAX_GRID_LEVELS; ++l) drop_record(m->lv[level], l);
     return NLR_OK;
 }
 
@@ -591,9 +641,10 @@
     if (N == 0) return NLR_OK;
     const LevelModel &lv = m->lv[level];
     hipStream_t st = (hipStream_t)stream;
+    const uint32_t groups = nlr_debug_get(NLR_DBG_RAY_GROUPS) == 1 ? 1u : 0u;
     if (lv.is_prop)
         return run_mlp_level(m, lv, rays, tdist, N, sample_n, sample_m, rand_deg, nullptr, nullptr, density, nullptr, nullptr,
-                             nullptr, features, st);
+                             nullptr, features, st, false, nullptr, nullptr, groups);
     Carve c(workspace, workspace_bytes);
     float *feat = features ? features : c.take((size_t)N * lv.S * lv.F + 256);
     float *rb = c.take((size_t)N * 32);
@@ -601,7 +652,7 @@
     if (c.off > workspace_bytes || (!workspace && c.off))
         NLR_FAIL(NLR_ERR_WORKSPACE, "mlp_level: workspace %zu B < needed %zu B", workspace_bytes, c.off);
     return run_mlp_level(m, lv, rays, tdist, N, sample_n, sample_m, rand_deg, feat, rb, density, rgb, sem, intensity, nullptr, st,
-                         features == nullptr);
+                         features == nullptr, nullptr, nullptr, groups);
 }
 
 struct DynScene {
diff --git a/nerf-lidar_amd/csrc/nlr_common.h b/nerf-lidar_amd/csrc/nlr_common.h
--- a/nerf-lidar_amd/csrc/nlr_common.h
+++ b/nerf-lidar_amd/csrc/nlr_common.h
@@ -47,14 +47,19 @@
     uint32_t dense[NLR_MAX_GRID_LEVELS];
     uint32_t mode[NLR_MAX_GRID_LEVELS];
     uint32_t step[NLR_MAX_GRID_LEVELS];
+    uint32_t rec_mask;
+    const void *rec[NLR_MAX_GRID_LEVELS];
 };
+
+size_t nlr_cell_record_bytes(const GridParams &gp, uint32_t level);
+int nlr_launch_bake_level(const GridParams &gp, uint32_t level, void *rec, hipStream_t st);
 
 int nlr_fill_grid_params(GridParams *gp, const void *table, int table_dtype, const int32_t *offsets_host,
                          uint32_t L, uint32_t C, float S, uint32_t H, uint32_t gridtype, int align_corners,
                          uint32_t interp);
 
 #ifdef __HIPCC__
-__device__ __forceinline__ uint32_t nlr_grid_index(uint32_t gridtype, uint32_t align_corners, uint32_t hsize,
+__host__ __device__ __forceinline__ uint32_t nlr_grid_index(uint32_t gridtype, uint32_t align_corners, uint32_t hsize,
                                                    uint32_t res, uint32_t x, uint32_t y, uint32_t z) {
     uint32_t stride = 1, index = 0;
     const uint32_t step = align_corners ? res : res + 1;
@@ -66,7 +71,7 @@
 }
 
 template <int MODE>
-__device__ __forceinline__ void nlr_corner_idx(const GridParams &gp, uint32_t level, const uint32_t (&pg)[3], uint32_t (&idx)[8]) {
+__host__ __device__ __forceinline__ void nlr_corner_idx(const GridParams &gp, uint32_t level, const uint32_t (&pg)[3], uint32_t (&idx)[8]) {
     if (MODE == 0) {
         const uint32_t s = gp.step[level];
         const uint32_t y0 = pg[1] * s, z0 = pg[2] * s * s;
diff --git a/nerf-lidar_amd/csrc/nlr_encode.hip b/nerf-lidar_amd/csrc/nlr_encode.hip
--- a/nerf-lidar_amd/csrc/nlr_encode.hip
+++ b/nerf-lidar_amd/csrc/nlr_encode.hip
@@ -339,8 +339,7 @@
     for (uint32_t l = NLR_DBG_LO; l < gp.L && l < (uint32_t)NLR_DBG_HI; ++l) {
         if (valid) {
             const float werf = re_weights ? nlr_erf_weight_fast(inv_s8, gp.inv_gsize[l]) : 1.0f;
-            if (gp.mode[l] == 0) nlr_level_fast<T, C, 0>(gp, l, g.x0, g.x1, g.x2, werf, r);
-            else nlr_level_fast<T, C, 1>(gp, l, g.x0, g.x1, g.x2, werf, r);
+            nlr_level_fast_any<T, C>(gp, l, g.x0, g.x1, g.x2, werf, r);
         }
         float a[C];
         nlr_group8_sum_to(r, a);
@@ -402,8 +401,7 @@
             if (l < (int)gp.L) {
                 const float werf = re_weights ? nlr_erf_weight_fast(inv_s8, gp.inv_gsize[l]) : 1.0f;
                 float a[C];
-                if (gp.mode[l] == 0) nlr_level_fast<T, C, 0>(gp, l, g.x0, g.x1, g.x2, werf, a);
-                else nlr_level_fast<T, C, 1>(gp, l, g.x0, g.x1, g.x2, werf, a);
+                nlr_level_fast_any<T, C>(gp, l, g.x0, g.x1, g.x2, werf, a);
 #pragma unroll
                 for (int c = 0; c < C; ++c) feat[l * C + c] = a[c];
             }
@@ -593,8 +591,8 @@
 }
 
 #include <atomic>
-#define NLR_DBG_KEYS 11
-static std::atomic<int> nlr_debug_switch[NLR_DBG_KEYS] = {{0}, {0}, {0}, {0}, {0}, {0}, {0}, {0}, {0}, {0}, {0}};
+#define NLR_DBG_KEYS 12
+static std::atomic<int> nlr_debug_switch[NLR_DBG_KEYS] = {{0}, {0}, {0}, {0}, {0}, {0}, {0}, {0}, {0}, {0}, {0}, {0}};
 extern "C" int nlr_debug_set(uint32_t key, int value) {
     NLR_CHECK_ARG(key < NLR_DBG_KEYS, "debug_set: unknown key %u", key);
     nlr_debug_switch[key].store(value);
@@ -602,6 +600,7 @@
 }
 extern "C" int nlr_debug_get(uint32_t key) { return key < NLR_DBG_KEYS ? nlr_debug_switch[key].load() : 0; }
 static bool nlr_force_generic() { return nlr_debug_switch[NLR_DBG_FORCE_GENERIC].load() != 0; }
+bool nlr_grid_fast_ok(const GridParams &gp) { return nlr_level_fast_ok(gp); }
 
 extern "C" int nlr_grid_fast_path(const int32_t *offsets_host, uint32_t L, uint32_t C, float S, uint32_t H, int table_dtype, uint32_t gridtype,
                                   int align_corners, uint32_t interp) {
diff --git a/nerf-lidar_amd/csrc/nlr_grid.hip b/nerf-lidar_amd/csrc/nlr_grid.hip
--- a/nerf-lidar_amd/csrc/nlr_grid.hip
+++ b/nerf-lidar_amd/csrc/nlr_grid.hip
@@ -207,12 +207,68 @@
     if (!no_cache && C <= 4 && gp.mode[level] <= 1 && gp.step[level] <= NLR_LDS_CACHE_MAX_STEP) return 2;
     return 0;
 }
-__device__ __forceinline__ void nlr_corner_idx_any(const GridParams &gp, uint32_t level, const uint32_t (&pg)[3], uint32_t (&idx)[8]) {
+__host__ __device__ __forceinline__ void nlr_corner_idx_any(const GridParams &gp, uint32_t level, const uint32_t (&pg)[3], uint32_t (&idx)[8]) {
     const uint32_t mode = gp.mode[level];
     if (mode == 0) nlr_corner_idx<0>(gp, level, pg, idx);
     else if (mode == 1) nlr_corner_idx<1>(gp, level, pg, idx);
     else nlr_corner_idx<2>(gp, level, pg, idx);
 }
+
+size_t nlr_cell_record_bytes(const GridParams &gp, uint32_t level) {
+    const size_t entry = (size_t)gp.C * (gp.table_dtype == 0 ? 4 : 2);
+    if (level >= gp.L || entry > 4 || gp.interp != 0 || gp.align_corners != 0 || gp.mode[level] > 1) return 0;
+    const uint64_t res = gp.res[level], bytes = res * res * res * 8u * entry;
+    return (res < 1024 && bytes <= (1ull << 32)) ? (size_t)bytes : 0;
+}
+
+template <typename U>
+__host__ __device__ __forceinline__ void nlr_bake_cell(const GridParams &gp, uint32_t level, uint32_t cell, const U *table, U *rec) {
+    const uint32_t res = gp.res[level];
+    const uint32_t z = cell / (res * res), rem = cell - z * res * res, y = rem / res;
+    const uint32_t pg[3] = {rem - y * res, y, z};
+    uint32_t idx[8];
+    nlr_corner_idx_any(gp, level, pg, idx);
+    const U *t = table + gp.offset[level];
+    U v[8];
+#pragma unroll
+    for (int c8 = 0; c8 < 8; ++c8) v[c8] = t[idx[c8]];
+#pragma unroll
+    for (int c8 = 0; c8 < 8; ++c8) rec[(size_t)cell * 8 + c8] = v[c8];
+}
+
+template <typename U>
+__global__ void __launch_bounds__(256) nlr_bake_cells_kernel(GridParams gp, uint32_t level, U *__restrict__ rec, uint32_t ncells) {
+    const uint32_t cell = blockIdx.x * 256u + threadIdx.x;
+    if (cell < ncells) nlr_bake_cell<U>(gp, level, cell, (const U *)gp.table, rec);
+}
+
+int nlr_launch_bake_level(const GridParams &gp, uint32_t level, void *rec, hipStream_t st) {
+    const size_t bytes = nlr_cell_record_bytes(gp, level);
+    NLR_CHECK_ARG(bytes && rec, "bake: level %u has no cell-record form", level);
+    const uint32_t res = gp.res[level], ncells = res * res * res;
+    const dim3 grid((ncells + 255) / 256), block(256);
+    if (gp.C * (gp.table_dtype == 0 ? 4u : 2u) == 4u)
+        hipLaunchKernelGGL((nlr_bake_cells_kernel<uint32_t>), grid, block, 0, st, gp, level, (uint32_t *)rec, ncells);
+    else
+        hipLaunchKernelGGL((nlr_bake_cells_kernel<uint16_t>), grid, block, 0, st, gp, level, (uint16_t *)rec, ncells);
+    NLR_LAUNCH_CHECK("nlr_bake_cells_kernel");
+    return NLR_OK;
+}
+
+extern "C" size_t nlr_cell_records_host(const void *table_host, int table_dtype, const int32_t *offsets_host, uint32_t L, uint32_t C, float S,
+                                        uint32_t H, uint32_t gridtype, uint32_t level, void *records_host, size_t records_bytes) {
+    GridParams gp;
+    if (!table_host || nlr_fill_grid_params(&gp, table_host, table_dtype, offsets_host, L, C, S, H, gridtype, 0, 0)) return 0;
+    const size_t bytes = nlr_cell_record_bytes(gp, level);
+    if (!bytes || !records_host || records_bytes < bytes) return bytes;
+    const uint32_t res = gp.res[level], ncells = res * res * res;
+    for (uint32_t cell = 0; cell < ncells; ++cell) {
+        if (C * (table_dtype == 0 ? 4u : 2u) == 4u) nlr_bake_cell<uint32_t>(gp, level, cell, (const uint32_t *)table_host, (uint32_t *)records_host);
+        else nlr_bake_cell<uint16_t>(gp, level, cell, (const uint16_t *)table_host, (uint16_t *)records_host);
+    }
+    return bytes;
+}
+
 template <int C>
 __global__ void __launch_bounds__(256) nlr_grid_bwd_kernel(const float *__restrict__ grad, const float *__restrict__ x,
                                                            GridParams gp, float *__restrict__ grad_table, uint32_t B,
diff --git a/nerf-lidar_amd/csrc/nlr_kernels.h b/nerf-lidar_amd/csrc/nlr_kernels.h
--- a/nerf-lidar_amd/csrc/nlr_kernels.h
+++ b/nerf-lidar_amd/csrc/nlr_kernels.h
@@ -73,6 +73,7 @@
 int nlr_fill_cast_params(CastParams *cp, const NlrRays *rays, const float *tdist, const float *rand_deg, uint32_t N,
                          uint32_t S, uint32_t n, uint32_t mloops, float std_scale);
 int nlr_launch_encode(const CastParams &cp, const GridParams &gp, int re_weights, float *feat, int piece_major, hipStream_t st);
+bool nlr_grid_fast_ok(const GridParams &gp);
 int nlr_launch_ray_vote(const float *tdist, uint32_t N, uint32_t S, uint32_t *votes, hipStream_t st);
 int nlr_launch_prop(const CastParams &cp, const GridParams &gp, const float *w1, const float *b1, const float *w2, float b2,
                     float density_bias, int re_weights, float *density, float *feat_out, hipStream_t st);
diff --git a/nerf-lidar_amd/csrc/nlr_level_fast.h b/nerf-lidar_amd/csrc/nlr_level_fast.h
--- a/nerf-lidar_amd/csrc/nlr_level_fast.h
+++ b/nerf-lidar_amd/csrc/nlr_level_fast.h
@@ -184,6 +184,42 @@
     }
 }
 
+template <typename T, int C>
+struct NlrCellRec {
+    static constexpr bool ok = C * sizeof(T) <= 4;
+    static constexpr int DW = ok ? 2 * (int)(C * sizeof(T)) : 1;
+    static constexpr int SH = 3 + (C * sizeof(T) == 2 ? 1 : 2);
+    static __device__ __forceinline__ float ch(const uint32_t (&q)[DW], int c8, int c) {
+        if constexpr (sizeof(T) == 4) return __builtin_bit_cast(float, q[c8]);
+        else {
+            const int h = c8 * C + c;
+            const __half2 p = __builtin_bit_cast(__half2, q[h >> 1]);
+            return (h & 1) ? __high2float(p) : __low2float(p);
+        }
+    }
+    static __device__ __forceinline__ void ld(const char *rec, uint32_t off, uint32_t (&q)[DW]) {
+        const uint4 a = *(const uint4 *)(rec + off);
+        q[0] = a.x, q[1] = a.y, q[2] = a.z, q[3] = a.w;
+        if constexpr (DW == 8) {
+            const uint4 b = *(const uint4 *)(rec + off + 16);
+            q[4] = b.x, q[5] = b.y, q[6] = b.z, q[7] = b.w;
+        }
+    }
+    static __device__ __forceinline__ void sld(const char *rec, uint32_t off, uint32_t (&q)[DW]) {
+        if constexpr (DW == 8) {
+            nlr_u8 t;
+            asm volatile("s_load_dwordx8 %0, %1, %2\ns_waitcnt lgkmcnt(0)" : "=&s"(t) : "s"(rec), "s"(off) : "memory");
+#pragma unroll
+            for (int i = 0; i < 8; ++i) q[i] = t[i];
+        } else {
+            nlr_u4 t;
+            asm volatile("s_load_dwordx4 %0, %1, %2\ns_waitcnt lgkmcnt(0)" : "=&s"(t) : "s"(rec), "s"(off) : "memory");
+#pragma unroll
+            for (int i = 0; i < 4; ++i) q[i] = t[i];
+        }
+    }
+};
+
 __device__ __forceinline__ uint32_t nlr_add_su(uint32_t v, uint32_t s) {
     uint32_t r;
     asm("v_add_u32 %0, %1, %2" : "=v"(r) : "s"(s), "v"(v));
@@ -195,7 +231,7 @@
     constexpr int E = NlrEntry<T, C>::E;
     constexpr int DW = (1 << E) / 4;
     const float scale = gp.scale[level];
-    const char *base = (const char *)gp.table + ((size_t)gp.offset[level] << E);
+    const char *base = MODE == 2 ? (const char *)gp.rec[level] : (const char *)gp.table + ((size_t)gp.offset[level] << E);
     const float p0 = fmaf(x0, scale, 0.5f), p1 = fmaf(x1, scale, 0.5f), p2 = fmaf(x2, scale, 0.5f);
     const uint32_t g0 = (uint32_t)p0, g1 = (uint32_t)p1, g2 = (uint32_t)p2;
     const float f0 = __builtin_amdgcn_fractf(p0), f1 = __builtin_amdgcn_fractf(p1), f2 = __builtin_amdgcn_fractf(p2);
@@ -211,14 +247,35 @@
     const uint32_t mask = hm << E;
     bool uniform = false;
     uint32_t u0 = 0, u1 = 0, u2 = 0;
-    if constexpr (DW >= 1) {
+    if constexpr (DW >= 1 || MODE == 2) {
         u0 = __builtin_amdgcn_readfirstlane(g0), u1 = __builtin_amdgcn_readfirstlane(g1), u2 = __builtin_amdgcn_readfirstlane(g2);
         uniform = __builtin_amdgcn_ballot_w64((g0 != u0) | (g1 != u1) | (g2 != u2)) == 0ull;
 #ifdef NLR_DBG_ENV
         if (nlr_dbg[3]) uniform = false;
 #endif
     }
-    if (uniform) {
+    if constexpr (MODE == 2) {
+        typedef NlrCellRec<T, C> Rec;
+        const uint32_t res = gp.res[level], ry = res << Rec::SH, rz = (res * res) << Rec::SH;
+        uint32_t q[Rec::DW];
+        if (uniform) {
+            Rec::sld(base, (u0 << Rec::SH) + u1 * ry + u2 * rz, q);
+#pragma unroll
+            for (int c8 = 0; c8 < 8; ++c8) {
+                const float w = (c8 & 1) ? w2[c8 >> 1].y : w2[c8 >> 1].x;
+#pragma unroll
+                for (int c = 0; c < C; ++c) r[c] = fmaf(w, Rec::ch(q, c8, c), r[c]);
+            }
+        } else {
+            Rec::ld(base, (g0 << Rec::SH) + g1 * ry + g2 * rz, q);
+#pragma unroll
+            for (int c8 = 0; c8 < 8; ++c8) {
+                const float w = (c8 & 1) ? w2[c8 >> 1].y : w2[c8 >> 1].x;
+#pragma unroll
+                for (int c = 0; c < C; ++c) r[c] = fmaf(w, Rec::ch(q, c8, c), r[c]);
+            }
+        }
+    } else if (uniform) {
         if constexpr (DW >= 1) {
             uint32_t so[8];
             if (MODE == 0) {
@@ -286,6 +343,18 @@
     }
 #pragma unroll
     for (int c = 0; c < C; ++c) a[c] = r[c] * werf;
+}
+
+template <typename T, int C>
+__device__ __forceinline__ void nlr_level_fast_any(const GridParams &gp, uint32_t level, float x0, float x1, float x2, float werf, float (&a)[C]) {
+    if constexpr (NlrCellRec<T, C>::ok) {
+        if ((gp.rec_mask >> level) & 1u) {
+            nlr_level_fast<T, C, 2>(gp, level, x0, x1, x2, werf, a);
+            return;
+        }
+    }
+    if (gp.mode[level] == 0) nlr_level_fast<T, C, 0>(gp, level, x0, x1, x2, werf, a);
+    else nlr_level_fast<T, C, 1>(gp, level, x0, x1, x2, werf, a);
 }
 
 #define NLR_DPP_ADD(R, CTRL) "v_add_f32_dpp " R ", " R ", " R " " CTRL " row_mask:0xf bank_mask:0xf\n"
diff --git a/nerf-lidar_amd/nerflidar_hip/_lib.py b/nerf-lidar_amd/nerflidar_hip/_lib.py
--- a/nerf-lidar_amd/nerflidar_hip/_lib.py
+++ b/nerf-lidar_amd/nerflidar_hip/_lib.py
@@ -74,7 +74,8 @@
 _lib = None
 
 EXPORTS = ["nlr_last_error", "nlr_version", "nlr_build_sha", "nlr_debug_set", "nlr_debug_get", "nlr_grid_fast_path", "nlr_grid_encode_forward", "nlr_grid_encode_backward", "nlr_grad_total_variation", "nlr_level_scale",
-           "nlr_sample_u", "nlr_model_create", "nlr_model_destroy", "nlr_model_set_table", "nlr_workspace_bytes",
+           "nlr_sample_u", "nlr_model_create", "nlr_model_destroy", "nlr_model_set_table", "nlr_model_bake_tables", "nlr_model_baked_bytes",
+           "nlr_cell_records_host", "nlr_workspace_bytes",
            "nlr_render_rays", "nlr_kernel_names", "nlr_resample_level", "nlr_mlp_level", "nlr_composite_level",
            "nlr_profile_begin", "nlr_profile_begin_kinds", "nlr_profile_end", "nlr_range_workspace_bytes", "nlr_range_project",
            "nlr_composite_backward", "nlr_hash_decay_forward", "nlr_hash_decay_backward", "nlr_box_winner", "nlr_cast_contract",
@@ -92,6 +93,8 @@
 ROUTE_FULL, ROUTE_FULL_FUSED, ROUTE_LIDAR, ROUTE_LIDAR_FUSED = 1, 2, 3, 4
 DBG_TRAIN_ROUTE, DBG_TRAIN_TRUNK_ROW0, DBG_TRAIN_TRUNK_ROWS = 8, 9, 10
 TRAIN_FULL, TRAIN_TRUNK, TRAIN_BWD = 1, 2, 4
+DBG_CELL_BUDGET_MIB = 11
+CELL_RECORD_BUDGET_MIB = 64
 
 
 def lib():
@@ -111,6 +114,12 @@
         L.nlr_model_destroy.argtypes = [c_fp]
         L.nlr_model_create.argtypes = [C.POINTER(NlrModelDesc), C.POINTER(c_fp), c_fp]
         L.nlr_model_set_table.argtypes = [c_fp, C.c_uint32, c_fp, C.c_int]
+        L.nlr_model_bake_tables.argtypes = [c_fp, c_fp]
+        L.nlr_model_baked_bytes.restype = C.c_size_t
+        L.nlr_model_baked_bytes.argtypes = [c_fp]
+        L.nlr_cell_records_host.restype = C.c_size_t
+        L.nlr_cell_records_host.argtypes = [c_fp, C.c_int, c_fp, C.c_uint32, C.c_uint32, C.c_float, C.c_uint32, C.c_uint32, C.c_uint32, c_fp,
+                                            C.c_size_t]
         L.nlr_level_scale.restype = None
         L.nlr_level_scale.argtypes = [C.c_uint32, C.c_float, C.c_uint32, c_fp, c_fp]
         L.nlr_sample_u.restype = None
diff --git a/nerf-lidar_amd/nerflidar_hip/models.py b/nerf-lidar_amd/nerflidar_hip/models.py
--- a/nerf-lidar_amd/nerflidar_hip/models.py
+++ b/nerf-lidar_amd/nerflidar_hip/models.py
@@ -20,7 +20,7 @@
 class Model:
 
     def __init__(self, mc: ModelConfig, state_dict: Dict[str, object], device="cuda:0",
-                 precision: int = _lib.PREC_FAST, table_dtype=torch.float32):
+                 precision: int = _lib.PREC_FAST, table_dtype=torch.float32, bake_tables: bool = True):
         if mc.config.instance_obj:
             raise NotImplementedError("instance_obj=True (dynamic-object branch, ZI/models.py:306-315,401-477) "
                                       "is outside the fused path (SURVEY section 8f-1)")
@@ -61,6 +61,16 @@
             rc = _lib.lib().nlr_model_create(C.byref(desc), C.byref(self._handle), _lib.current_stream())
         _lib.check(rc, "nlr_model_create")
         self._keep.clear()
+        self.baked_bytes = 0
+        if bake_tables:
+            self.bake_tables()
+
+    def bake_tables(self) -> int:
+        with torch.cuda.device(self.device):
+            rc = _lib.lib().nlr_model_bake_tables(self._handle, _lib.current_stream())
+        _lib.check(rc, "nlr_model_bake_tables")
+        self.baked_bytes = int(_lib.lib().nlr_model_baked_bytes(self._handle))
+        return self.baked_bytes
 
     def _linear(self, sd, name) -> _lib.NlrLinear:
         w, b = _f32c(sd[name + ".weight"]), _f32c(sd[name + ".bias"])
```

After: 5.359 million rays/s. No clear change (-0.5%).
